# araju6/parameter-server-distributed

Measured on AMD Instinct MI355X. Metric: samples/sec (whole node) ResNet-50 async-SGD, higher is better.
Workload: dtype bf16

## Files before the change

### parameter_server_distributed_amd/csrc/bindings.cpp

```cpp
#include <torch/extension.h>

#include "async_hyper.h"
#include "async_ps.h"
#include "checkpoint.h"
#include "comm.h"
#include "kernels/launchers.h"
#include "kernels/launchers_gemm.h"
#include "ops.h"
#include "ps_core.h"
#include "registry.h"
#include "staleness.h"

namespace py = pybind11;
using namespace psd;

PYBIND11_MODULE(_C, m) {
  m.doc() = "MI355X-native parameter-server runtime: gfx950 HIP kernels, RCCL comm, PS/coordinator cores";

  m.def("fused_apply_", &fused_apply_, py::arg("master"), py::arg("grads"), py::arg("state1"), py::arg("state2"),
        py::arg("shadow"), py::arg("dyn"), py::arg("kind"), py::arg("momentum") = 0.0, py::arg("dampening") = 0.0,
        py::arg("nesterov") = false, py::arg("weight_decay") = 0.0, py::arg("beta1") = 0.9, py::arg("beta2") = 0.999,
        py::arg("eps") = 1e-8, py::arg("maximize") = false,
        py::arg("grid_cap") = 0, py::arg("scales") = ScaleList{}, py::arg("mx_scales") = MxScaleList{});
  m.def("fused_apply_lw_", &fused_apply_lw_, py::arg("master"), py::arg("grads"), py::arg("state1"),
        py::arg("state2"), py::arg("shadow"), py::arg("dyn"), py::arg("kind"), py::arg("momentum") = 0.0,
        py::arg("dampening") = 0.0, py::arg("nesterov") = false, py::arg("weight_decay") = 0.0, py::arg("beta1") = 0.9,
        py::arg("beta2") = 0.999, py::arg("eps") = 1e-8, py::arg("maximize") = false, py::arg("trust_coef") = 0.001,
        py::arg("layers") = std::vector<at::Tensor>{}, py::arg("grid_cap") = 0, py::arg("scales") = ScaleList{},
        py::arg("mx_scales") = MxScaleList{});
  m.def(
      "lw_table_build",
      [](const std::vector<int64_t>& offsets, const std::vector<int64_t>& numels, const std::vector<int64_t>& ndims,
         int64_t n, bool exclude_1d, int64_t align, const std::string& device) {
        return lw_table_build(offsets, numels, ndims, n, exclude_1d, align, at::Device(device));
      },
      py::arg("offsets"), py::arg("numels"), py::arg("ndims"), py::arg("n"), py::arg("exclude_1d"),
      py::arg("align") = 64, py::arg("device") = "cpu");
  m.def(
      "async_hyper",
      [](int kind, int workers, double momentum, double beta1, double beta2, double weight_decay) {
        const AsyncHyper h = async_hyper(kind, workers, momentum, beta1, beta2, weight_decay);
        py::dict d;
        d["lr_factor"] = h.lr_factor;
        d["grad_scale"] = h.grad_scale;
        d["momentum"] = h.momentum;
        d["beta1"] = h.beta1;
        d["beta2"] = h.beta2;
        d["weight_decay"] = h.weight_decay;
        return d;
      },
      py::arg("kind"), py::arg("workers"), py::arg("momentum"), py::arg("beta1"), py::arg("beta2"),
      py::arg("weight_decay"), "per-push optimizer hyperparameters of an apply-on-arrival PS (async_hyper.h)");
  m.def("optim_advance_", &optim_advance_, py::arg("dyn"), py::arg("beta1") = 0.9, py::arg("beta2") = 0.999);
  m.def("multi_reduce_", &multi_reduce_, py::arg("out"), py::arg("srcs"), py::arg("scale") = 1.0,
        py::arg("scales") = ScaleList{}, py::arg("mx_scales") = MxScaleList{});
  m.def("push_quant_mx_", &push_quant_mx_, py::arg("x"), py::arg("q"), py::arg("scales"),
        py::arg("blocks_per_seg") = 0, py::arg("residual") = py::none());
  m.def("grad_clip_coef_", &grad_clip_coef_, py::arg("flat"), py::arg("clip_norm"), py::arg("out"), py::arg("partials"),
        py::arg("grid_cap") = 0);
  m.def("pack_cast_", &pack_cast_, py::arg("srcs"), py::arg("dsts"));
  m.def("xfer_", &xfer_, py::arg("srcs"), py::arg("dsts"), py::arg("blocks_per_seg"), py::arg("nt_store") = false);
  m.def("amax_", &amax_);
  m.def("quant_fp8_", &quant_fp8_);
  m.def("dequant_fp8_", &dequant_fp8_);
  m.def("quant_mx_", &quant_mx_, py::arg("x"), py::arg("out"), py::arg("scales"));
  m.def("dequant_mx_", &dequant_mx_, py::arg("q"), py::arg("scales"), py::arg("out"));
  m.def("quant_mx_t_", &quant_mx_t_, py::arg("x"), py::arg("out"), py::arg("scales"));
  m.def("quant_mx_dual_", &quant_mx_dual_, py::arg("x"), py::arg("q_row"), py::arg("s_row"), py::arg("q_t"),
        py::arg("s_t"));
  m.def("quant_fp8_jit_", &quant_fp8_jit_, py::arg("x"), py::arg("out"), py::arg("scale_inv"));
  m.def("quant_fp8_delayed_", &quant_fp8_delayed_, py::arg("x"), py::arg("out"), py::arg("scale_inv"),
        py::arg("hist"), py::arg("margin") = 1.0);
  m.def("embed_bwd_", &embed_bwd_, py::arg("sorted"), py::arg("perm"), py::arg("dy"), py::arg("out"));
  m.def("xent_fwd", &xent_fwd, py::arg("x"), py::arg("labels"));
  m.def("xent_bwd", &xent_bwd, py::arg("x"), py::arg("labels"), py::arg("lse"), py::arg("scale"),
        py::arg("lse_lo") = py::none());
  m.def("bn_fwd", &bn_fwd, py::arg("x"), py::arg("gamma"), py::arg("beta"), py::arg("running_mean"),
        py::arg("running_var"), py::arg("residual"), py::arg("relu"), py::arg("training"), py::arg("momentum"),
        py::arg("eps"), py::arg("counter"), py::arg("ss_eval"), py::arg("mask_out") = false,
        py::arg("residual_ss") = py::none(), py::arg("stats_only") = false, py::arg("q8_out") = py::none(),
        py::arg("part_in") = py::none(), py::arg("part_rows") = 0, py::arg("q8_mx") = py::none());
  m.def("bn_reduce_", &bn_reduce_, py::arg("x"), py::arg("shift"));
  m.def("bn_bwd_reduce_", &bn_bwd_reduce_, py::arg("dy"), py::arg("x"), py::arg("save_mean"),
        py::arg("ss") = py::none(), py::arg("dy2") = py::none(), py::arg("mbits") = py::none());
  m.def("bn_bwd_dual", &bn_bwd_dual, py::arg("dy"), py::arg("x"), py::arg("gamma"), py::arg("save_mean"),
        py::arg("save_invstd"), py::arg("mbits"), py::arg("dy2"), py::arg("xd"), py::arg("gamma_d"), py::arg("mean_d"),
        py::arg("invstd_d"), py::arg("dgamma_out") = py::none(), py::arg("dbeta_out") = py::none(),
        py::arg("dgamma_d_out") = py::none(), py::arg("dbeta_d_out") = py::none(), py::arg("fold") = false);
  m.def("bn_bwd_coef", &bn_bwd_coef, py::arg("dy"), py::arg("x"), py::arg("gamma"), py::arg("save_mean"),
        py::arg("save_invstd"), py::arg("mbits") = py::none(), py::arg("dy2") = py::none(), py::arg("part") = py::none(),
        py::arg("rows") = 0, py::arg("dgamma_out") = py::none(), py::arg("dbeta_out") = py::none());
  m.def("bn_bwd", &bn_bwd, py::arg("dy"), py::arg("x"), py::arg("y"), py::arg("gamma"), py::arg("save_mean"),
        py::arg("save_invstd"), py::arg("relu"), py::arg("need_dr"), py::arg("dgamma_out"), py::arg("dbeta_out"),
        py::arg("dy2") = py::none(), py::arg("ss") = py::none(), py::arg("mbits") = py::none(),
        py::arg("dq") = py::none(), py::arg("dqmx") = py::none());
  m.def("gemm_", &gemm_, py::arg("A"), py::arg("B"), py::arg("a_kmajor"), py::arg("b_kmajor"), py::arg("out"),
        py::arg("bias") = py::none(), py::arg("act") = 0, py::arg("aux") = py::none(), py::arg("part") = py::none(),
        py::arg("shift") = py::none());
  m.def("gemm_stats_rows", &gemm_stats_rows_, py::arg("M"));
  m.def("gemm_set_bcontig", &gemm_set_bcontig, py::arg("on"));
  m.def("gemm_ct_", &gemm_ct_, py::arg("A"), py::arg("B"), py::arg("out"), py::arg("bias") = py::none(),
        py::arg("act") = 0, py::arg("aux") = py::none());
  m.def("gemm_gelu_bwd_", &gemm_gelu_bwd_, py::arg("A"), py::arg("B"), py::arg("a_kmajor"), py::arg("b_kmajor"),
        py::arg("pre"), py::arg("out"), py::arg("db"), py::arg("accumulate") = false);
  m.def("gemm_splitk_", &gemm_splitk_, py::arg("A"), py::arg("B"), py::arg("a_kmajor"), py::arg("b_kmajor"),
        py::arg("out"), py::arg("accumulate") = false, py::arg("scale") = 1.0, py::arg("splits") = 0);
  m.def("gemm_fp8_", &gemm_fp8_, py::arg("A"), py::arg("B"), py::arg("a_scale"), py::arg("b_scale"), py::arg("out"),
        py::arg("bias") = py::none(), py::arg("act") = 0, py::arg("aux") = py::none(), py::arg("part") = py::none(),
        py::arg("shift") = py::none());
  m.def("gemm_fp8_splitk_", &gemm_fp8_splitk_, py::arg("A"), py::arg("B"), py::arg("a_scale"), py::arg("b_scale"),
        py::arg("out"), py::arg("accumulate") = false, py::arg("scale") = 1.0, py::arg("splits") = 0);
  m.def("gemm_fp8_splits", &gemm_fp8_splits, py::arg("M"), py::arg("N"), py::arg("K"));
  m.def("convn_", &convn_, py::arg("x"), py::arg("w2"), py::arg("out"), py::arg("R"), py::arg("S"), py::arg("stride"),
        py::arg("pad"), py::arg("part") = py::none(), py::arg("shift") = py::none(), py::arg("variant") = -1,
        py::arg("x2") = py::none(), py::arg("bias") = py::none(), py::arg("no_store") = false,
        py::arg("apply_ss") = py::none(), py::arg("apply_res") = py::none(), py::arg("apply_mask") = py::none());
  m.def("convn_stats_rows", &convn_stats_rows_, py::arg("M"));
  m.def("convn_part_rows", &convn_part_rows_, py::arg("M"), py::arg("N"), py::arg("variant"), py::arg("Ho"),
        py::arg("Wo"), py::arg("R"));
  m.def("convn_variant_ok", &convn_variant_ok_, py::arg("N"), py::arg("variant"), py::arg("R"), py::arg("S"),
        py::arg("stride"), py::arg("pad"), py::arg("Wo"), py::arg("has_x2") = false);
  m.def("convn_dgrad_s2_", &convn_dgrad_s2_, py::arg("dy"), py::arg("wph"), py::arg("out"), py::arg("variant"),
        py::arg("part") = py::none(), py::arg("bx") = py::none(), py::arg("bmean") = py::none(),
        py::arg("bss") = py::none());
  m.def("convn_dgrad_s2_rows", &convn_dgrad_s2_rows, py::arg("Nb"), py::arg("Ho"), py::arg("Wo"), py::arg("Ci"),
        py::arg("variant"));
  m.def("convn_bwd_", &convn_bwd_, py::arg("dy"), py::arg("w2"), py::arg("out"), py::arg("R"), py::arg("S"),
        py::arg("stride"), py::arg("pad"), py::arg("part"), py::arg("variant"), py::arg("mode"), py::arg("bx"),
        py::arg("bmean"), py::arg("bss") = py::none(), py::arg("bdr") = py::none(), py::arg("bmbits") = py::none(),
        py::arg("x2") = py::none(), py::arg("bias") = py::none(), py::arg("bxd") = py::none(),
        py::arg("bmean_d") = py::none(), py::arg("part_d") = py::none());
  m.def("bn_bwd_pre", &bn_bwd_pre, py::arg("g"), py::arg("x"), py::arg("gamma"), py::arg("save_mean"),
        py::arg("save_invstd"), py::arg("part"), py::arg("rows"), py::arg("dgamma_out") = py::none(),
        py::arg("dbeta_out") = py::none(), py::arg("dq") = py::none(), py::arg("dqmx") = py::none());
  m.def("convn_variants", &convn_variants_, py::arg("N"));
  m.def("convn_variant_kind", &convn_variant_kind_, py::arg("N"), py::arg("variant"));
  m.def("conv_fwd_", &conv_fwd_, py::arg("x"), py::arg("w2"), py::arg("out"), py::arg("R"), py::arg("S"),
        py::arg("stride"), py::arg("pad"), py::arg("part") = py::none(), py::arg("shift") = py::none());
  m.def("conv_wgrad_", &conv_wgrad_, py::arg("dy"), py::arg("x"), py::arg("out"), py::arg("R"), py::arg("S"),
        py::arg("stride"), py::arg("pad"), py::arg("splits") = 0);
  m.def("convw_", &convw_, py::arg("dy"), py::arg("x"), py::arg("out"), py::arg("R"), py::arg("S"), py::arg("stride"),
        py::arg("pad"), py::arg("variant") = -1, py::arg("accumulate") = false, py::arg("fold") = false);
  m.def("bn_bwd_dual_pre", &bn_bwd_dual_pre, py::arg("g"), py::arg("x"), py::arg("gamma"), py::arg("save_mean"),
        py::arg("save_invstd"), py::arg("part"), py::arg("part_d"), py::arg("rows"), py::arg("xd"), py::arg("gamma_d"),
        py::arg("mean_d"), py::arg("invstd_d"), py::arg("dgamma_out") = py::none(), py::arg("dbeta_out") = py::none(),
        py::arg("dgamma_d_out") = py::none(), py::arg("dbeta_d_out") = py::none(), py::arg("fold") = false,
        py::arg("fold_d") = false, py::arg("derive_d") = false);
  m.def("bn_elemt_coef", &bn_elemt_coef, py::arg("g"), py::arg("x"), py::arg("coef"));
  m.def("convw_fold_rows", &convw_fold_rows, py::arg("Cout"), py::arg("Cin"));
  m.def("convw_gram_rows", &convw_gram_rows_, py::arg("C"));
  m.def("convw_gram_", &convw_gram_, py::arg("x"), py::arg("out"), py::arg("variant") = 0);
  m.def("bnfold_dgrad_weights", &bnfold_dgrad_weights, py::arg("w"), py::arg("coef"));
  m.def("bnfold_rowdot", &bnfold_rowdot, py::arg("P"), py::arg("w"), py::arg("row"));
  m.def("bnfold_gram_stats", &bnfold_gram_stats, py::arg("P"), py::arg("w"), py::arg("shift"), py::arg("M"),
        py::arg("row"));
  m.def("bnfold_dual_weights", &bnfold_dual_weights, py::arg("w3"), py::arg("wd"), py::arg("ss3"), py::arg("ssd"));
  m.def("bn_finalize", &bn_finalize, py::arg("part"), py::arg("rows"), py::arg("M"), py::arg("gamma"),
        py::arg("beta"), py::arg("running_mean"), py::arg("running_var"), py::arg("momentum"), py::arg("eps"),
        py::arg("counter") = py::none());
  m.def("bnfold_combine", &bnfold_combine, py::arg("P"), py::arg("w"), py::arg("coef"), py::arg("out"),
        py::arg("accumulate") = false);
  m.def("convw_variants", &convw_variants_, py::arg("Cout"), py::arg("KK"));
  m.def("conv_fwd_fp8_", &conv_fwd_fp8_, py::arg("x"), py::arg("w2"), py::arg("x_scale"), py::arg("w_scale"),
        py::arg("out"), py::arg("R"), py::arg("S"), py::arg("stride"), py::arg("pad"), py::arg("part") = py::none(),
        py::arg("shift") = py::none());
  m.def("gelu_bwd_colsum_", &gelu_bwd_colsum_, py::arg("dy"), py::arg("pre"), py::arg("dx"), py::arg("out"),
        py::arg("accumulate") = false);
  m.def("colsum_", &colsum_, py::arg("x"), py::arg("out"), py::arg("accumulate") = false);
  m.def("maxpool3s2_fwd", &maxpool3s2_fwd);
  m.def("maxpool3s2_bwd", &maxpool3s2_bwd, py::arg("dy"), py::arg("arg"), py::arg("H"), py::arg("W"),
        py::arg("dy2") = py::none());
  m.def("gap_fwd", &gap_fwd);
  m.def("bn_pool_fwd", &bn_pool_fwd, py::arg("x"), py::arg("gamma"), py::arg("beta"), py::arg("running_mean"),
        py::arg("running_var"), py::arg("momentum"), py::arg("eps"), py::arg("counter") = py::none());
  m.def("stem_fwd", &stem_fwd, py::arg("x"), py::arg("w"), py::arg("gamma"), py::arg("beta"), py::arg("running_mean"),
        py::arg("running_var"), py::arg("momentum"), py::arg("eps"), py::arg("counter") = py::none());
  m.def("stem_wgrad", &stem_wgrad);
  m.def("attn_fwd", &attn_fwd, py::arg("qkv"), py::arg("heads"), py::arg("p"), py::arg("seed"),
        py::arg("step") = py::none(), py::arg("lens") = py::none(), py::arg("grid_cap") = 0, py::arg("causal") = false,
        py::arg("doc_start") = py::none(), py::arg("window") = 0);
  m.def("attn_bwd", &attn_bwd, py::arg("dout"), py::arg("qkv"), py::arg("o"), py::arg("lse"), py::arg("heads"),
        py::arg("p"), py::arg("seed"), py::arg("step") = py::none(), py::arg("bias_out") = py::none(),
        py::arg("lens") = py::none(), py::arg("grid_cap") = 0, py::arg("causal") = false,
        py::arg("doc_start") = py::none(), py::arg("window") = 0);
  m.def("rope_", &rope_, py::arg("qkv"), py::arg("heads"), py::arg("cos"), py::arg("sin"), py::arg("lens") = py::none(),
        py::arg("doc_start") = py::none(), py::arg("inverse") = false, py::arg("blocks") = 0);
  m.def("rms_fwd", &rms_fwd, py::arg("r"), py::arg("h") = py::none(), py::arg("gamma"), py::arg("eps"), py::arg("p"),
        py::arg("seed"), py::arg("step") = py::none());
  m.def("rms_bwd", &rms_bwd, py::arg("dy"), py::arg("dr_new") = py::none(), py::arg("r_new"), py::arg("rstd"),
        py::arg("gamma"), py::arg("p"), py::arg("seed"), py::arg("step") = py::none(), py::arg("had_h"),
        py::arg("dgamma_out") = py::none());
  m.def("swiglu_fwd", &swiglu_fwd, py::arg("gu"), py::arg("blocks") = 0);
  m.def("swiglu_bwd", &swiglu_bwd, py::arg("da"), py::arg("gu"), py::arg("blocks") = 0);
  m.def("ln_fwd", &ln_fwd, py::arg("x"), py::arg("h"), py::arg("gamma"), py::arg("beta"), py::arg("eps"), py::arg("p"),
        py::arg("seed"), py::arg("step") = py::none(), py::arg("q8_out") = py::none(),
        py::arg("sc8_out") = py::none());
  m.def("ln_bwd", &ln_bwd, py::arg("dy"), py::arg("s"), py::arg("mean"), py::arg("rstd"), py::arg("gamma"), py::arg("p"),
        py::arg("seed"), py::arg("step") = py::none(), py::arg("dgamma_out") = py::none(),
        py::arg("dbeta_out") = py::none(), py::arg("dhsum_out") = py::none());
  m.def("emb_ln_fwd", &emb_ln_fwd, py::arg("ids"), py::arg("types"), py::arg("W"), py::arg("P"), py::arg("T"),
        py::arg("gamma"), py::arg("beta"), py::arg("S"), py::arg("eps"), py::arg("p"), py::arg("seed"),
        py::arg("step") = py::none(), py::arg("pos_ids") = py::none());
  m.def("emb_ln_bwd", &emb_ln_bwd, py::arg("dy"), py::arg("ids"), py::arg("types"), py::arg("W"), py::arg("P"),
        py::arg("T"), py::arg("gamma"), py::arg("mean"), py::arg("rstd"), py::arg("S"), py::arg("p"), py::arg("seed"),
        py::arg("step") = py::none(), py::arg("dgamma") = py::none(), py::arg("dbeta") = py::none(),
        py::arg("dT") = py::none(), py::arg("pos_ids") = py::none());
  m.def("bn_pool_bwd", &bn_pool_bwd, py::arg("gpool"), py::arg("gpool2"), py::arg("arg"), py::arg("x"), py::arg("gamma"),
        py::arg("save_mean"), py::arg("save_invstd"), py::arg("ss"), py::arg("dgamma_out") = py::none(),
        py::arg("dbeta_out") = py::none());
  m.def("gap_bwd", &gap_bwd);
  m.def("subsample2", &subsample2, py::arg("x"));
  m.def("wprep_table", &wprep_table, py::arg("srcs"), py::arg("dsts"), py::arg("geo"));
  m.def("wprep_run", &wprep_run, py::arg("table"), py::arg("tiles"));
  m.attr("OPT_SGD") = (int)OPT_SGD;
  m.attr("OPT_MOMENTUM") = (int)OPT_MOMENTUM;
  m.attr("OPT_ADAM") = (int)OPT_ADAM;
  m.attr("OPT_ADAMW") = (int)OPT_ADAMW;
  m.attr("OPT_LARS") = (int)OPT_LARS;
  m.attr("OPT_LAMB") = (int)OPT_LAMB;

  m.def("save_reference_ckpt", &save_reference_ckpt, py::call_guard<py::gil_scoped_release>());
  m.def("load_reference_ckpt", &load_reference_ckpt, py::call_guard<py::gil_scoped_release>());
  m.def("save_native_ckpt", &save_native_ckpt, py::call_guard<py::gil_scoped_release>());
  m.def("load_native_ckpt", &load_native_ckpt, py::call_guard<py::gil_scoped_release>());
  m.def("crc32", [](py::bytes b) {
    std::string s = b;
    return crc32(s.data(), s.size());
  });

  py::class_<WorkerEntry>(m, "WorkerEntry")
      .def_readonly("worker_id", &WorkerEntry::worker_id)
      .def_readonly("address", &WorkerEntry::address)
      .def_readonly("port", &WorkerEntry::port)
      .def_readonly("hostname", &WorkerEntry::hostname)
      .def_readonly("status", &WorkerEntry::status)
      .def_readonly("last_heartbeat", &WorkerEntry::last_heartbeat)
      .def_readonly("join_epoch", &WorkerEntry::join_epoch);
  py::class_<RegisterResult>(m, "RegisterResult")
      .def_readonly("success", &RegisterResult::success)
      .def_readonly("message", &RegisterResult::message)
      .def_readonly("ps_address", &RegisterResult::ps_address)
      .def_readonly("total_workers", &RegisterResult::total_workers)
      .def_readonly("membership_epoch", &RegisterResult::membership_epoch);
  py::class_<ShardInfo>(m, "ShardInfo")
      .def_readonly("shard_id", &ShardInfo::shard_id)
      .def_readonly("address", &ShardInfo::address)
      .def_readonly("rank", &ShardInfo::rank);
  py::class_<Registry>(m, "Registry")
      .def(py::init<std::string, int32_t>())
      .def("register_worker", &Registry::register_worker)
      .def("heartbeat", &Registry::heartbeat)
      .def("deregister", &Registry::deregister)
      .def("list_workers", &Registry::list_workers)
      .def("live_ids", &Registry::live_ids)
      .def("ps_address", &Registry::ps_address)
      .def("set_ps_address", &Registry::set_ps_address)
      .def("remove_stale", &Registry::remove_stale)
      .def("membership_epoch", &Registry::membership_epoch)
      .def("wait_epoch_change", &Registry::wait_epoch_change, py::call_guard<py::gil_scoped_release>())
      .def("set_shard", &Registry::set_shard)
      .def("shards", &Registry::shards)
      .def("kv_set", [](Registry& r, const std::string& k, py::bytes v) { r.kv_set(k, std::string(v)); })
      .def("kv_get",
           [](Registry& r, const std::string& k, double timeout) {
             std::tuple<bool, std::string> res;
             {
               py::gil_scoped_release nogil;
               res = r.kv_get(k, timeout);
             }
             return py::make_tuple(std::get<0>(res), py::bytes(std::get<1>(res)));
           })
      .def("use_manual_clock", &Registry::use_manual_clock)
      .def("advance_clock", &Registry::advance_clock)
      .def("now", &Registry::now);

  py::class_<PSConfig>(m, "PSConfig")
      .def(py::init<>())
      .def_readwrite("total_workers", &PSConfig::total_workers)
      .def_readwrite("async_mode", &PSConfig::async_mode)
      .def_readwrite("staleness_bound", &PSConfig::staleness_bound)
      .def_readwrite("window", &PSConfig::window)
      .def_readwrite("opt_kind", &PSConfig::opt_kind)
      .def_readwrite("lr", &PSConfig::lr)
      .def_readwrite("momentum", &PSConfig::momentum)
// ... 128 lines not shown
```

### parameter_server_distributed_amd/csrc/conv_ops.cpp

```cpp
#include <ATen/ATen.h>
#include <c10/core/DeviceGuard.h>

#include <algorithm>

#include "glue.h"
#include "kernels/launchers_convn.h"
#include "kernels/launchers_convw.h"
#include "kernels/launchers_gemm.h"
#include "ops.h"

namespace psd {

namespace {

struct ConvGeo {
  int64_t Nb, C, H, W, R, S, stride, pad, Ho, Wo, M, bytes;
  int logC;
  bool pow2_c() const { return (C & (C - 1)) == 0; }
};

ConvGeo conv_geo(const at::Tensor& x, int64_t R, int64_t S, int64_t stride, int64_t pad) {
  ConvGeo g{};
  g.Nb = x.size(0), g.C = x.size(1), g.H = x.size(2), g.W = x.size(3);
  g.R = R, g.S = S, g.stride = stride, g.pad = pad;
// ... 55 lines not shown
  a.Wo = (int)g.Wo;
  a.S = (int)g.S;
  a.stride = (int)g.stride;
  a.pad = (int)g.pad;
}

int64_t part_rows_bound(int64_t M, int64_t N, int64_t variant, int64_t Ho, int64_t Wo, int64_t R) {
  return std::max(convn_stats_rows((int)M), convn_part_rows_geo((int)M, (int)N, (int)std::max<int64_t>(variant, 0),
                                                                (int)Ho, (int)Wo, (int)R));
}

}

static int64_t conv_fwd_impl(const at::Tensor& x, const at::Tensor& w2, at::Tensor out, int64_t R, int64_t S,
                             int64_t stride, int64_t pad, const at::Tensor* xs, const at::Tensor* ws,
                             const c10::optional<at::Tensor>& part, const c10::optional<at::Tensor>& shift) {
  const bool f8 = xs != nullptr;
  const auto dt = f8 ? at::kFloat8_e4m3fn : at::kBFloat16;
  const bool x_e5 = f8 && x.scalar_type() == at::kFloat8_e5m2;
  const int esz = f8 ? 1 : 2;
  TORCH_CHECK(is_nhwc_dev(x, x_e5 ? at::kFloat8_e5m2 : dt), "psd conv_fwd: x must be a channels_last ",
              f8 ? "e4m3fn / e5m2" : "bf16", " device tensor");
  TORCH_CHECK(w2.is_cuda() && w2.dim() == 2 && w2.scalar_type() == dt && w2.stride(1) == 1 &&
                  (w2.stride(0) * esz) % 16 == 0 && aligned16(w2),
              "psd conv_fwd: w2 must be a 2-D device tensor like x, unit inner stride, 16-B aligned rows");
  TORCH_CHECK(out.dim() == 2 && out.stride(1) == 1 && out.scalar_type() == at::kBFloat16, "psd conv_fwd: out");
  const bool mx = f8 && xs->scalar_type() == at::kByte;
  if (mx) {
    TORCH_CHECK(ws->scalar_type() == at::kByte && xs->is_cuda() && ws->is_cuda() && xs->is_contiguous() &&
                    ws->is_contiguous() && xs->numel() == x.numel() / 32 && ws->numel() == w2.numel() / 32 &&
                    w2.stride(0) == w2.size(1),
                "psd conv_fwd_fp8: MX scales must be uint8 [pixels, C/32] / [Cout, K/32] (contiguous w2)");
  } else if (f8) {
    TORCH_CHECK(xs->scalar_type() == at::kFloat && ws->scalar_type() == at::kFloat && xs->is_cuda() && ws->is_cuda() &&
                    xs->numel() >= 1 && ws->numel() >= 1,
                "psd conv_fwd_fp8: scales must be fp32 device scalars (or MX uint8 block scales)");
  }
  const ConvGeo g = conv_geo(x, R, S, stride, pad);
  const int64_t M = g.M, Cout = w2.size(0), K = R * S * g.C;
  TORCH_CHECK(w2.size(1) == K, "psd conv_fwd: w2 must be [Cout, R*S*C]");
  TORCH_CHECK(out.size(0) == M && out.size(1) == Cout, "psd conv_fwd: out must be [Nb*Ho*Wo, Cout]");
  if (!g.pow2_c() || g.C < (f8 ? 128 : 64) || g.bytes >= ((int64_t)1 << 32) || M >= ((int64_t)1 << 31)) return 0;
  const c10::DeviceGuard dg(x.device());
  GemmArgs a{};
  a.A = x.data_ptr();
  a.B = w2.data_ptr();
  a.C = out.data_ptr();
  a.M = (int)M;
  a.N = (int)Cout;
  a.K = (int)K;
  a.lda = (int)K;
  a.ldb = (int)w2.stride(0);
  a.ldc = (int)out.stride(0);
  a.a_kmajor = a.b_kmajor = 1;
  set_geo(a, g);
  if (mx) {
    a.a_mx = xs->data_ptr<uint8_t>();
    a.b_mx = ws->data_ptr<uint8_t>();
  } else if (f8) {
    a.a_scale = xs->data_ptr<float>();
    a.b_scale = ws->data_ptr<float>();
  }
  a.f8a = x_e5 ? 1 : 0;
  int rows = 0;
  set_stats(a, part, shift, out, &rows);
  hipError_t e = f8 ? launch_conv_fwd_fp8(a, stream_of(x)) : launch_conv_fwd(a, stream_of(x));
  if (e == hipErrorNotSupported) return 0;
  check_hip(e, "psd conv_fwd");
  return a.part ? rows : 1;
}

int64_t conv_fwd_(const at::Tensor& x, const at::Tensor& w2, at::Tensor out, int64_t R, int64_t S, int64_t stride,
                  int64_t pad, c10::optional<at::Tensor> part, c10::optional<at::Tensor> shift) {
  return conv_fwd_impl(x, w2, out, R, S, stride, pad, nullptr, nullptr, part, shift);
}

int64_t conv_fwd_fp8_(const at::Tensor& x, const at::Tensor& w2, const at::Tensor& x_scale, const at::Tensor& w_scale,
                      at::Tensor out, int64_t R, int64_t S, int64_t stride, int64_t pad, c10::optional<at::Tensor> part,
                      c10::optional<at::Tensor> shift) {
  return conv_fwd_impl(x, w2, out, R, S, stride, pad, &x_scale, &w_scale, part, shift);
}

bool conv_wgrad_(const at::Tensor& dy, const at::Tensor& x, at::Tensor out, int64_t R, int64_t S, int64_t stride,
                 int64_t pad, int64_t splits) {
  TORCH_CHECK(is_nhwc_dev(dy, at::kBFloat16) && is_nhwc_dev(x, at::kBFloat16),
              "psd conv_wgrad: dy and x must be channels_last bf16 device tensors");
  const ConvGeo g = conv_geo(x, R, S, stride, pad);
  const int64_t Cout = dy.size(1);
  TORCH_CHECK(dy_matches(dy, g), "psd conv_wgrad: dy shape does not match the convolution");
  const int64_t N = R * S * g.C, K = g.M;
  TORCH_CHECK(out.dim() == 2 && out.size(0) == Cout && out.size(1) == N && out.is_contiguous() &&
                  out.scalar_type() == at::kBFloat16,
              "psd conv_wgrad: out must be a contiguous bf16 [Cout, R*S*C]");
  if (!g.pow2_c() || g.C < 8 || g.bytes >= ((int64_t)1 << 32) || K >= ((int64_t)1 << 31) || K < 128) return false;
  const c10::DeviceGuard dg(x.device());
  const int64_t tiles = ((Cout + 255) / 256) * ((N + 255) / 256);
  int64_t s = splits > 0 ? splits : std::max<int64_t>(1, 256 / tiles);
  s = std::min<int64_t>(s, std::max<int64_t>(1, K / 128));
  at::Tensor slab = at::empty({s * Cout * N}, x.options().dtype(at::kFloat));
  GemmArgs a{};
  a.A = dy.data_ptr();
  a.B = x.data_ptr();
  a.M = (int)Cout;
  a.N = (int)N;
  a.K = (int)K;
  a.lda = (int)Cout;
  a.ldb = (int)N;
  a.ldc = (int)N;
  a.a_kmajor = a.b_kmajor = 0;
  set_geo(a, g);
  hipError_t e = launch_conv_wgrad(a, slab.data_ptr<float>(), (int)s, out.data_ptr(), stream_of(x));
  if (e == hipErrorNotSupported) return false;
  check_hip(e, "psd conv_wgrad");
  return true;
}

int64_t convn_stats_rows_(int64_t M) { return convn_stats_rows((int)M); }
int64_t convn_part_rows_(int64_t M, int64_t N, int64_t v, int64_t Ho, int64_t Wo, int64_t R) {
  return convn_part_rows_geo((int)M, (int)N, (int)v, (int)Ho, (int)Wo, (int)R);
}
bool convn_variant_ok_(int64_t N, int64_t v, int64_t R, int64_t S, int64_t stride, int64_t pad, int64_t Wo,
                       bool has_x2) {
  return convn_variant_ok((int)N, (int)v, (int)R, (int)S, (int)stride, (int)pad, (int)Wo, has_x2);
}
int64_t convn_variants_(int64_t N) { return convn_variants((int)N); }
int64_t convn_variant_kind_(int64_t N, int64_t v) { return convn_variant_kind((int)N, (int)v); }

namespace {
int64_t convn_x2(ConvnArgs& a, const at::Tensor& x, c10::optional<at::Tensor> x2, c10::optional<at::Tensor> bias,
                 int64_t N) {
  if (given(bias)) {
    TORCH_CHECK(bias->scalar_type() == at::kFloat && bias->numel() == N && bias->is_contiguous() &&
                    bias->device() == x.device(),
                "psd convn: bias must be fp32 [N] on the input's device");
    a.bias = bias->data_ptr<float>();
  }
  if (!given(x2)) return 0;
  TORCH_CHECK(is_nhwc_dev(*x2, at::kBFloat16) && x2->device() == x.device() && x2->size(0) == x.size(0) &&
                  x2->size(2) == x.size(2) && x2->size(3) == x.size(3),
              "psd convn: x2 must be a channels_last bf16 tensor with the input's N, H, W");
  const int64_t C2 = x2->size(1), bytes = x2->numel() * 2;
  if (C2 < 64 || (C2 & (C2 - 1)) != 0 || bytes > 0xFFFFFF00ll) return -1;
  a.x2 = x2->data_ptr();
  a.x2bytes = (uint32_t)bytes;
  a.logC2 = log2_exact(C2);
  return C2;
}
}

int64_t convn_(const at::Tensor& x, const at::Tensor& w2, at::Tensor out, int64_t R, int64_t S, int64_t stride,
               int64_t pad, c10::optional<at::Tensor> part, c10::optional<at::Tensor> shift, int64_t variant,
               c10::optional<at::Tensor> x2, c10::optional<at::Tensor> bias, bool no_store,
               c10::optional<at::Tensor> apply_ss, c10::optional<at::Tensor> apply_res,
               c10::optional<at::Tensor> apply_mask) {
  TORCH_CHECK(is_nhwc_dev(x, at::kBFloat16), "psd convn: x must be a channels_last bf16 device tensor");
  TORCH_CHECK(w2.is_cuda() && w2.dim() == 2 && w2.scalar_type() == at::kBFloat16 && w2.is_contiguous(),
              "psd convn: w2 must be a contiguous bf16 [Cout, R*S*C] device tensor");
  TORCH_CHECK(no_store || (out.is_cuda() && out.dim() == 2 && out.stride(1) == 1 &&
                           out.scalar_type() == at::kBFloat16 && aligned16(out)),
              "psd convn: out must be a bf16 [M, Cout] device tensor, 16-B aligned");
  const bool apply = given(apply_ss);
  const ConvGeo g = conv_geo(x, R, S, stride, pad);
  const int64_t M = g.M, Cout = w2.size(0), Ho = g.Ho, Wo = g.Wo;
  ConvnArgs a{};
  const int64_t C2 = convn_x2(a, x, x2, bias, Cout);
  if (C2 < 0) return 0;
  const int64_t K = R * S * g.C + C2;
  TORCH_CHECK(w2.size(1) == K, "psd convn: w2 must be [Cout, R*S*C (+ C2)]");
  TORCH_CHECK(no_store || (out.size(0) == M && out.size(1) == Cout), "psd convn: out must be [Nb*Ho*Wo, Cout]");
  const bool stats = given(part);
  TORCH_CHECK(!no_store || (stats && !apply), "psd convn: no_store is a statistics-only pass");
  if (apply) {
    TORCH_CHECK(!stats && apply_ss->scalar_type() == at::kFloat && apply_ss->numel() == 2 * Cout &&
                    apply_ss->is_contiguous() && apply_ss->device() == x.device(),
                "psd convn: apply_ss must be fp32 [2 Cout] (no statistics in an apply pass)");
    TORCH_CHECK(!given(apply_res) ||
                    (apply_res->scalar_type() == at::kBFloat16 && apply_res->numel() == M * Cout &&
                     apply_res->device() == x.device() && nhwc_laid(*apply_res)),
                "psd convn: apply_res must be a bf16 [M, Cout] (or channels_last) residual, or None");
    TORCH_CHECK(given(apply_mask) && apply_mask->scalar_type() == at::kByte && apply_mask->numel() == M * Cout / 8 &&
                    apply_mask->is_contiguous(),
                "psd convn: apply_mask must be uint8 [M * Cout / 8]");
    TORCH_CHECK(out.stride(0) == Cout, "psd convn: the apply pass writes a dense [M, Cout] output");
  }
  if (stats) {
    TORCH_CHECK(given(shift) && shift->numel() == Cout && shift->scalar_type() == at::kFloat &&
                    shift->is_contiguous() && shift->device() == x.device(),
                "psd convn: statistics need an fp32 [Cout] shift on x's device");
    TORCH_CHECK(part->scalar_type() == at::kFloat && part->is_contiguous() && part->device() == x.device() &&
                    part->numel() >= part_rows_bound(M, Cout, variant, Ho, Wo, R) * 2 * Cout,
                "psd convn: part must be fp32 [convn_part_rows(...), 2, Cout]");
  }
  const int64_t wbytes = w2.numel() * 2;
  if (!g.pow2_c() || g.C < 64 || g.bytes > 0xFFFFFF00ll || wbytes >= ((int64_t)1 << 32) ||
      M >= ((int64_t)1 << 31) - 256 || convn_tile_n((int)Cout) == 0 || (!no_store && out.stride(0) % 8 != 0) ||
      Ho <= 0 || Wo <= 0 || variant >= convn_variants((int)Cout))
    return 0;
  const c10::DeviceGuard dg(x.device());
  a.x = x.data_ptr();
  a.w = w2.data_ptr();
  a.y = no_store ? nullptr : out.data_ptr();
  a.part = stats ? part->data_ptr<float>() : nullptr;
  a.shift = stats ? shift->data_ptr<float>() : nullptr;
  if (apply) {
    a.bwd = 8;
    a.bss = apply_ss->data_ptr<float>();
    a.ares = opt_ptr<const uint16_t>(apply_res);
    a.amask = apply_mask->data_ptr<uint8_t>();
  }
  set_geo(a, g, wbytes, Cout, K, no_store ? Cout : out.stride(0), variant);
  const hipError_t e = launch_convn(a, stream_of(x));
  if (e == hipErrorNotSupported) return 0;
  check_hip(e, "psd convn");
  return stats ? convn_part_rows_geo((int)M, (int)Cout, (int)std::max<int64_t>(variant, 0), (int)Ho, (int)Wo, (int)R)
               : 1;
}

int64_t convn_dgrad_s2_(const at::Tensor& dy, const std::vector<at::Tensor>& wph, at::Tensor out, int64_t variant,
                        c10::optional<at::Tensor> part, c10::optional<at::Tensor> bx, c10::optional<at::Tensor> bmean,
                        c10::optional<at::Tensor> bss) {
  TORCH_CHECK(is_nhwc_dev(dy, at::kBFloat16), "psd convn_dgrad_s2: dy must be a channels_last bf16 device tensor");
  TORCH_CHECK(wph.size() == 4, "psd convn_dgrad_s2: four phase weights");
  ConvGeo g = conv_geo(dy, 1, 1, 1, 0);
  const int64_t Co = g.C, Ho = g.Ho, Wo = g.Wo, M = g.M;
  const int64_t Ci = wph[0].size(0);
  for (int k = 0; k < 4; ++k) {
    const int64_t taps = (1 + (k >> 1)) * (1 + (k & 1));
    TORCH_CHECK(wph[k].is_cuda() && wph[k].dim() == 2 && wph[k].scalar_type() == at::kBFloat16 &&
                    wph[k].is_contiguous() && wph[k].size(0) == Ci && wph[k].size(1) == taps * Co &&
                    wph[k].device() == dy.device(),
                "psd convn_dgrad_s2: wph[k] must be a contiguous bf16 [Ci, taps * Co] tensor");
  }
  TORCH_CHECK(out.dim() == 2 && out.is_contiguous() && out.scalar_type() == at::kBFloat16 && out.size(0) == 4 * M &&
                  out.size(1) == Ci && out.device() == dy.device(),
              "psd convn_dgrad_s2: out must be a contiguous bf16 [Nb * 2Ho * 2Wo, Ci] tensor");
  const bool fused = given(part);
  if (fused) {
    TORCH_CHECK(given(bx) && bx->scalar_type() == at::kBFloat16 && bx->numel() == 4 * M * Ci &&
                    bx->device() == dy.device() && nhwc_laid(*bx),
                "psd convn_dgrad_s2: bx must be the BN input, bf16 like dX");
    TORCH_CHECK(given(bmean) && bmean->scalar_type() == at::kFloat && bmean->numel() == Ci && bmean->is_contiguous() &&
                    given(bss) && bss->scalar_type() == at::kFloat && bss->numel() == 2 * Ci && bss->is_contiguous(),
                "psd convn_dgrad_s2: mode 1 needs the BN's fp32 mean [Ci] and scale/shift [2 Ci]");
    TORCH_CHECK(part->scalar_type() == at::kFloat && part->is_contiguous() && part->device() == dy.device() &&
                    part->numel() >= 4 * part_rows_bound(M, Ci, variant, Ho, Wo, 2) * 2 * Ci,
                "psd convn_dgrad_s2: part must be fp32 [4 * convn_dgrad_s2_rows(...), 2, Ci]");
  }
  if (!g.pow2_c() || Co < 64 || g.bytes > 0xFFFFFF00ll || convn_tile_n((int)Ci) == 0 || Ci % 8 != 0 || variant < 0 ||
      variant >= convn_variants((int)Ci) || convn_variant_kind((int)Ci, (int)variant) != 0 || M >= (1 << 24))
    return 0;
  const c10::DeviceGuard dg(dy.device());
  const hipStream_t st = stream_of(dy);
  int64_t rows = 0;
  for (int k = 0; k < 4; ++k) {
    g.R = 1 + (k >> 1), g.S = 1 + (k & 1);
    ConvnArgs a{};
    a.x = dy.data_ptr();
    a.w = wph[k].data_ptr();
    a.y = out.data_ptr();
    set_geo(a, g, wph[k].numel() * 2, Ci, g.R * g.S * Co, Ci, variant);
    a.ophase = 1 + k;
    if (fused) {
      a.bwd = 1;
      a.part = part->data_ptr<float>() + rows * 2 * Ci;
      a.bx = reinterpret_cast<const uint16_t*>(bx->data_ptr());
      a.bmean = bmean->data_ptr<float>();
      a.bss = bss->data_ptr<float>();
    }
    const hipError_t e = launch_convn(a, st);
    if (e == hipErrorNotSupported) {
      TORCH_CHECK(k == 0, "psd convn_dgrad_s2: phase ", k, " declined after phase 0 ran");
      return 0;
    }
    check_hip(e, "psd convn_dgrad_s2");
    if (fused) rows += convn_part_rows_geo((int)M, (int)Ci, (int)variant, (int)Ho, (int)Wo, (int)g.R);
  }
  return fused ? rows : 1;
}

int64_t convn_dgrad_s2_rows(int64_t Nb, int64_t Ho, int64_t Wo, int64_t Ci, int64_t variant) {
  return 4 * part_rows_bound((int)(Nb * Ho * Wo), Ci, variant, Ho, Wo, 2);
}

int64_t convn_bwd_(const at::Tensor& dy, const at::Tensor& w2, at::Tensor out, int64_t R, int64_t S, int64_t stride,
                   int64_t pad, at::Tensor part, int64_t variant, int64_t mode, c10::optional<at::Tensor> bx,
                   const at::Tensor& bmean, c10::optional<at::Tensor> bss, c10::optional<at::Tensor> bdr,
                   c10::optional<at::Tensor> bmbits, c10::optional<at::Tensor> x2, c10::optional<at::Tensor> bias,
                   c10::optional<at::Tensor> bxd, c10::optional<at::Tensor> bmean_d, c10::optional<at::Tensor> part_d) {
  TORCH_CHECK(is_nhwc_dev(dy, at::kBFloat16), "psd convn_bwd: dy must be a channels_last bf16 device tensor");
  TORCH_CHECK(w2.is_cuda() && w2.dim() == 2 && w2.scalar_type() == at::kBFloat16 && w2.is_contiguous(),
              "psd convn_bwd: w2 must be a contiguous bf16 [N, R*S*C] tensor");
  TORCH_CHECK(out.dim() == 2 && out.is_contiguous() && out.scalar_type() == at::kBFloat16, "psd convn_bwd: out");
  TORCH_CHECK(mode == 1 || mode == 2 || mode == 3 || mode == 5,
              "psd convn_bwd: mode 1 (mask from x, ss), 2 (bit-mask + dr), 3 (2 + the dual tail's second BN) or 5 "
              "(2 with dr on the stride-2 quarter grid)");
  const ConvGeo g = conv_geo(dy, R, S, stride, pad);
  const int64_t Nb = g.Nb, Ho = g.Ho, Wo = g.Wo, M = g.M, N = w2.size(0);
  ConvnArgs a{};
  const int64_t C2 = convn_x2(a, dy, x2, bias, N);
  if (C2 < 0) return 0;
  const int64_t K = R * S * g.C + C2;
  TORCH_CHECK(w2.size(1) == K && out.size(0) == M && out.size(1) == N, "psd convn_bwd: shapes");
  auto like_out = [&](const at::Tensor& t, const char* what) {
    TORCH_CHECK(t.scalar_type() == at::kBFloat16 && t.numel() == M * N && t.device() == dy.device() && nhwc_laid(t),
                "psd convn_bwd: ", what, " must be a contiguous bf16 [M, N] (or channels_last) tensor");
  };
  const bool has_bx = given(bx);
  TORCH_CHECK(has_bx || mode == 2 || mode == 5, "psd convn_bwd: only modes 2 and 5 run without the BN input bx");
  if (has_bx) like_out(*bx, "bx");
  TORCH_CHECK(bmean.scalar_type() == at::kFloat && bmean.numel() == N && bmean.is_contiguous(), "psd convn_bwd: bmean");
  TORCH_CHECK(part.scalar_type() == at::kFloat && part.is_contiguous() &&
                  part.numel() >= part_rows_bound(M, N, variant, Ho, Wo, R) * 2 * N,
              "psd convn_bwd: part must be fp32 [convn_part_rows(...), 2, N]");
  if (mode == 1) {
    TORCH_CHECK(given(bss) && bss->numel() == 2 * N && bss->scalar_type() == at::kFloat && bss->is_contiguous(),
                "psd convn_bwd: mode 1 needs ss fp32 [2N]");
  } else {
    if (mode == 3) {
      TORCH_CHECK(given(bxd) && given(bmean_d) && given(part_d), "psd convn_bwd: mode 3 needs bxd, bmean_d and part_d");
      like_out(*bxd, "bxd");
      TORCH_CHECK(bmean_d->scalar_type() == at::kFloat && bmean_d->numel() == N && bmean_d->is_contiguous(),
                  "psd convn_bwd: bmean_d");
      TORCH_CHECK(part_d->scalar_type() == at::kFloat && part_d->is_contiguous() && part_d->numel() >= part.numel(),
                  "psd convn_bwd: part_d like part");
    }
    TORCH_CHECK(given(bdr), "psd convn_bwd: mode 2 needs dr");
    if (mode == 5) {
      TORCH_CHECK(bdr->scalar_type() == at::kBFloat16 && bdr->dim() == 4 && bdr->size(0) == Nb && bdr->size(1) == N &&
                      bdr->size(2) * 2 == Ho && bdr->size(3) * 2 == Wo &&
                      bdr->is_contiguous(at::MemoryFormat::ChannelsLast) && bdr->device() == dy.device(),
                  "psd convn_bwd: mode 5 dr must be channels_last bf16 [Nb, N, Ho/2, Wo/2]");
    } else {
      like_out(*bdr, "dr");
    }
    TORCH_CHECK(given(bmbits) && bmbits->scalar_type() == at::kByte && bmbits->numel() == M * N / 8 &&
                    bmbits->is_contiguous(),
                "psd convn_bwd: mode 2 needs the uint8 [M*N/8] bit-mask");
  }
  const int64_t wbytes = w2.numel() * 2;
  if (!g.pow2_c() || g.C < 64 || g.bytes > 0xFFFFFF00ll || wbytes >= ((int64_t)1 << 32) ||
      M >= ((int64_t)1 << 31) - 256 || convn_tile_n((int)N) == 0 || variant >= convn_variants((int)N) || N % 8 != 0)
    return 0;
  const c10::DeviceGuard dg(dy.device());
  a.x = dy.data_ptr();
  a.w = w2.data_ptr();
  a.y = out.data_ptr();
  a.part = part.data_ptr<float>();
  set_geo(a, g, wbytes, N, K, N, variant);
  a.bwd = (int)mode;
  a.bx = opt_ptr<const uint16_t>(bx);
  a.bmean = bmean.data_ptr<float>();
  a.bss = mode == 1 ? bss->data_ptr<float>() : nullptr;
  a.bdr = mode >= 2 ? reinterpret_cast<const uint16_t*>(bdr->data_ptr()) : nullptr;
  a.bmbits = mode >= 2 ? bmbits->data_ptr<uint8_t>() : nullptr;
  if (mode == 3) {
    a.bxd = reinterpret_cast<const uint16_t*>(bxd->data_ptr());
    a.bmean_d = bmean_d->data_ptr<float>();
    a.part_d = part_d->data_ptr<float>();
  }
  const hipError_t e = launch_convn(a, stream_of(dy));
  if (e == hipErrorNotSupported) return 0;
  check_hip(e, "psd convn_bwd");
  return convn_part_rows_geo((int)M, (int)N, (int)std::max<int64_t>(variant, 0), (int)Ho, (int)Wo, (int)R);
}

int64_t convw_variants_(int64_t Cout, int64_t KK) { return convw_variants((int)Cout, (int)KK); }

int64_t convw_fold_rows(int64_t Cout, int64_t Cin) {
  const int64_t rows = (Cout + Cin + 16 + 127) / 128 * 128;
  return convw_fold_ok((int)Cout, (int)Cin, (int)rows) ? rows : 0;
}

namespace {
bool run_convw(ConvwArgs& a, const at::Tensor& x, const char* op) {
  const ConvwPlan p = convw_plan(a);
  if (p.splits <= 0) return false;
  at::Tensor slab = at::empty({p.slab_floats}, x.options().dtype(at::kFloat));
  a.slab = slab.data_ptr<float>();
  const hipError_t e = launch_convw(a, stream_of(x));
  if (e == hipErrorNotSupported) return false;
  check_hip(e, op);
  return true;
}
}

bool convw_(const at::Tensor& dy, const at::Tensor& x, at::Tensor out, int64_t R, int64_t S, int64_t stride,
            int64_t pad, int64_t variant, bool accumulate, bool fold) {
  TORCH_CHECK(is_nhwc_dev(dy, at::kBFloat16) && is_nhwc_dev(x, at::kBFloat16) && dy.device() == x.device(),
              "psd convw: dy and x must be channels_last bf16 tensors on one device");
  const ConvGeo g = conv_geo(x, R, S, stride, pad);
  const int64_t Cout = dy.size(1);
  TORCH_CHECK(dy_matches(dy, g), "psd convw: dy shape does not match the convolution");
  const int64_t KK = R * S * g.C, M = g.M;
  const int64_t rows = fold ? convw_fold_rows(Cout, KK) : Cout;
  TORCH_CHECK(out.is_cuda() && out.device() == x.device() && out.dim() == 2 && out.size(0) == rows &&
                  out.size(1) == KK && out.is_contiguous() &&
                  out.scalar_type() == (fold ? at::kFloat : at::kBFloat16) && aligned16(out),
              "psd convw: out must be a contiguous [Cout, R*S*C] bf16 tensor (fold: fp32 [convw_fold_rows, C]) "
              "on x's device");
  if (fold && (R != 1 || S != 1 || stride != 1 || pad != 0 || accumulate)) return false;
  const int64_t dybytes = dy.numel() * 2;
  if (!g.pow2_c() || g.C < 64 || g.bytes > 0xFFFFFF00ll || dybytes > 0xFFFFFF00ll || M >= ((int64_t)1 << 31) ||
      (!fold && variant >= convw_variants((int)Cout, (int)KK)) || g.H >= 32768 || g.W >= 32768)
    return false;
  const c10::DeviceGuard dg(x.device());
  ConvwArgs a{};
  a.dy = dy.data_ptr();
  a.x = x.data_ptr();
  a.out = out.data_ptr();
  a.dybytes = (uint32_t)dybytes;
  set_geo(a, g);
  a.Cout = (int)Cout;
  a.KK = (int)KK;
  a.variant = (int)variant;
  a.accumulate = accumulate ? 1 : 0;
  a.fold = fold ? 1 : 0;
  a.Arows = (int)rows;
  return run_convw(a, x, "psd convw");
}

int64_t convw_gram_rows_(int64_t C) { return convw_gram_rows((int)C); }

bool convw_gram_(const at::Tensor& x, at::Tensor out, int64_t variant) {
  TORCH_CHECK(is_nhwc_dev(x, at::kBFloat16), "psd convw_gram: x must be a channels_last bf16 tensor");
  const ConvGeo g = conv_geo(x, 1, 1, 1, 0);
  const int64_t C = g.C, M = g.M;
  const int64_t rows = convw_gram_rows((int)C);
  TORCH_CHECK(out.is_cuda() && out.device() == x.device() && out.dim() == 2 && out.size(0) == rows &&
                  out.size(1) == C && out.is_contiguous() && out.scalar_type() == at::kFloat && aligned16(out),
              "psd convw_gram: out must be a contiguous fp32 [convw_gram_rows(C), C] tensor on x's device");
  if (rows == 0 || g.bytes > 0xFFFFFF00ll || M >= ((int64_t)1 << 31) || M == 0) return false;
  const c10::DeviceGuard dg(x.device());
  ConvwArgs a{};
  a.dy = x.data_ptr();
  a.x = x.data_ptr();
  a.out = out.data_ptr();
  a.dybytes = (uint32_t)g.bytes;
  set_geo(a, g);
  a.Cout = 0;
  a.KK = (int)C;
  a.fold = 2;
  a.variant = (int)variant;
  a.Arows = (int)rows;
  return run_convw(a, x, "psd convw_gram");
}

}
```

### parameter_server_distributed_amd/csrc/kernels/convn.hip

```cpp
#include "mfma_common.h"
#include "cu_count.h"
#include "launchers_convn.h"

namespace psd {

namespace {

constexpr int kBM = 128;
constexpr int kBK = 64;

__device__ __forceinline__ bf16x8 frag(const uint8_t* lds, int rb, int ks, int lane) {
  const int row = rb * 16 + (lane & 15);
  return __builtin_bit_cast(bf16x8, *reinterpret_cast<const u32x4*>(lds + kmaj_off(row, ks * 4 + (lane >> 4))));
}

template <int DPSK, int A>
__device__ __forceinline__ void wait_ahead(int ahead) {
  if constexpr (A <= 0) {
    wait_vm<0>();
  } else {
    if (ahead >= A) wait_vm<A * DPSK>();
    else wait_ahead<DPSK, A - 1>(ahead);
  }
}

template <int N>
__device__ __forceinline__ float ror_row(float x) {
  return __builtin_bit_cast(float, __builtin_amdgcn_mov_dpp(__builtin_bit_cast(int, x), 0x120 + N, 0xF, 0xF, true));
}

__device__ __forceinline__ int fdiv(int x, int d, float inv) {
  int q = (int)((float)x * inv);
  const int r = x - q * d;
  q += (r >= d ? 1 : 0) - (r < 0 ? 1 : 0);
  return q;
}

template <int BM, int BN, int WNT, int NSLOT>
struct Geo {
  static constexpr int WM = BM / 64;
  static constexpr int NWC = BN / WNT;
  static constexpr int NW = WM * NWC;
  static constexpr int NT = 64 * NW;
  static constexpr int JN = WNT / 16;
  static constexpr int APW = (BM / 8) / NW;
  static constexpr int BPW = (BN / 8) / NW;
  static constexpr int DPS = APW + BPW;
  static constexpr int AB = BM * 128;
  static constexpr int SLOT = AB + BN * 128;
  static constexpr int STG = 2048;
  static_assert((BM / 8) % NW == 0 && (BN / 8) % NW == 0 && APW >= 1 && BPW >= 1, "DMA pieces per wave");
  static_assert(DPS * (NSLOT - 2) < 64, "vmcnt is 6 bits");
  static_assert(WNT == 32 || WNT == 64, "wave tile width");
};


}

template <int JN>
struct EpiSums {
  float s1[JN], s2[JN];
  float ga[8], gb[8], gd[8];
  __device__ __forceinline__ void zero() {
#pragma unroll
    for (int j = 0; j < JN; ++j) s1[j] = s2[j] = 0.f;
#pragma unroll
    for (int e = 0; e < 8; ++e) ga[e] = gb[e] = gd[e] = 0.f;
  }
};

template <int WNT, bool STATS, int BWD>
__device__ __forceinline__ void convn_flush(const ConvnArgs& a, EpiSums<WNT / 16>& es, int64_t prow, int wc, int lane,
                                            int n0) {
  constexpr int JN = WNT / 16;
  const int cl = lane & 15;
  if constexpr (STATS) {
#pragma unroll
    for (int j = 0; j < JN; ++j) {
      float s1 = es.s1[j], s2 = es.s2[j];
      s1 += xor16(s1, lane);
      s2 += xor16(s2, lane);
      s1 += xor32(s1, lane);
      s2 += xor32(s2, lane);
      if (lane < 16) {
        float* pr = a.part + prow * 2 * a.N;
        const int col = n0 + wc * WNT + j * 16 + cl;
        pr[col] = s1;
        pr[a.N + col] = s2;
      }
    }
  }
  if constexpr (BWD >= 1 && BWD <= 5) {
    constexpr int CPR = WNT * 2 / 16;
    const int my_col = n0 + wc * WNT + (lane % CPR) * 8;
#pragma unroll
    for (int e = 0; e < 8; ++e) {
      if constexpr (CPR == 4) {
        es.ga[e] += ror_row<4>(es.ga[e]);
        es.gb[e] += ror_row<4>(es.gb[e]);
      }
      es.ga[e] += ror_row<8>(es.ga[e]);
      es.gb[e] += ror_row<8>(es.gb[e]);
      es.ga[e] += xor16(es.ga[e], lane);
      es.gb[e] += xor16(es.gb[e], lane);
      es.ga[e] += xor32(es.ga[e], lane);
      es.gb[e] += xor32(es.gb[e], lane);
      if constexpr (BWD == 3) {
        if constexpr (CPR == 4) es.gd[e] += ror_row<4>(es.gd[e]);
        es.gd[e] += ror_row<8>(es.gd[e]);
        es.gd[e] += xor16(es.gd[e], lane);
        es.gd[e] += xor32(es.gd[e], lane);
      }
    }
    if (lane < CPR) {
      float* pr = a.part + prow * 2 * a.N;
      store8_f32(pr + my_col, es.ga);
      store8_f32(pr + a.N + my_col, es.gb);
      if constexpr (BWD == 3) {
        float* pd = a.part_d + prow * 2 * a.N;
        store8_f32(pd + my_col, es.ga);
        store8_f32(pd + a.N + my_col, es.gd);
      }
    }
  }
}

template <int WNT>
struct EpiOps {
  static constexpr int CPR = WNT * 2 / 16;
  static constexpr int PASSES = 16 * CPR / 64;
  int mm[4][PASSES];
  u32x4 exr[4][PASSES], rv4[4][PASSES], dv4[4][PASSES];
  uint32_t bt[4][PASSES];
};

template <int WNT, int BWD, typename Pix>
__device__ __forceinline__ void epi_load(const ConvnArgs& a, int wr, int wc, int lane, Pix pix, int n0, EpiOps<WNT>& o) {
  constexpr bool BRED = BWD >= 1 && BWD <= 5;
  constexpr bool APPLY = BWD == 8;
  constexpr int CPR = EpiOps<WNT>::CPR, PASSES = EpiOps<WNT>::PASSES;
  const int my_col = n0 + wc * WNT + (lane % CPR) * 8;
  const bool has_bx = !BRED || a.bx != nullptr;
  const bool fast_div = a.M < (1 << 24);
  float inv_hw = 0.f, inv_wo = 0.f;
  if constexpr (BWD == 5) {
    inv_hw = 1.f / (float)(a.Ho * a.Wo);
    inv_wo = 1.f / (float)a.Wo;
  }
#pragma unroll
  for (int i = 0; i < 4; ++i)
#pragma unroll
    for (int ps = 0; ps < PASSES; ++ps) {
      const int c = ps * 64 + lane;
      const int rr = c / CPR;
      const int m = pix(wr * 64 + i * 16 + rr);
      o.mm[i][ps] = m;
      if constexpr (APPLY) {
        o.rv4[i][ps] = u32x4{0u, 0u, 0u, 0u};
        if (m >= 0 && a.ares) o.rv4[i][ps] = *reinterpret_cast<const u32x4*>(a.ares + (int64_t)m * a.N + my_col);
      }
      if constexpr (BRED) {
        o.exr[i][ps] = o.rv4[i][ps] = o.dv4[i][ps] = u32x4{0u, 0u, 0u, 0u};
        o.bt[i][ps] = 0u;
        if (m >= 0) {
          if (has_bx) o.exr[i][ps] = *reinterpret_cast<const u32x4*>(a.bx + (int64_t)m * a.N + my_col);
          if constexpr (BWD >= 2) {
            if constexpr (BWD == 5) {
              const int hw = a.Ho * a.Wo;
              const int n = fast_div ? fdiv(m, hw, inv_hw) : m / hw, rem = m - n * hw;
              const int h = fast_div ? fdiv(rem, a.Wo, inv_wo) : rem / a.Wo, w = rem - h * a.Wo;
              if (((h | w) & 1) == 0) {
                const int64_t q = ((int64_t)n * (a.Ho >> 1) + (h >> 1)) * (a.Wo >> 1) + (w >> 1);
                o.rv4[i][ps] = *reinterpret_cast<const u32x4*>(a.bdr + q * a.N + my_col);
              }
            } else {
              o.rv4[i][ps] = *reinterpret_cast<const u32x4*>(a.bdr + (int64_t)m * a.N + my_col);
            }
            o.bt[i][ps] = a.bmbits[((int64_t)m * a.N + my_col) >> 3];
          }
          if constexpr (BWD == 3) o.dv4[i][ps] = *reinterpret_cast<const u32x4*>(a.bxd + (int64_t)m * a.N + my_col);
        }
      }
    }
}

template <int BM, int BN, int WNT, bool STATS, int BWD, bool DEFER = false, bool PRE = false, typename Pix>
__device__ __forceinline__ void convn_epilogue(const ConvnArgs& a, f32x4 (&acc)[4][WNT / 16],
                                               const float (&kshift)[WNT / 16], int tm, int wr, int wc, int lane,
                                               uint8_t* stg, Pix pix, int n0, EpiSums<WNT / 16>& es,
                                               const EpiOps<WNT>* pre = nullptr) {
  constexpr int JN = WNT / 16;
  constexpr int WM = BM / 64;
  const int cl = lane & 15, rq = (lane >> 4) * 4;
  if (a.bias) {
#pragma unroll
    for (int j = 0; j < JN; ++j) {
      const float bv = a.bias[n0 + wc * WNT + j * 16 + cl];
#pragma unroll
      for (int i = 0; i < 4; ++i) acc[i][j] += f32x4{bv, bv, bv, bv};
    }
  }
  if constexpr (STATS) {
    typedef float f32x2 __attribute__((ext_vector_type(2)));
    const bool rnd = a.y != nullptr;
#pragma unroll
    for (int i = 0; i < 4; ++i) {
      const bool full = pix(wr * 64 + i * 16 + 15) >= 0;
#pragma unroll
      for (int j = 0; j < JN; ++j) {
        const f32x2 k2 = {kshift[j], kshift[j]};
        f32x2 s1 = {0.f, 0.f}, s2 = {0.f, 0.f};
#pragma unroll
        for (int r = 0; r < 4; r += 2) {
          f32x2 d;
          if (rnd) {
            const uint32_t pk = pack_bf16x2_rne(acc[i][j][r], acc[i][j][r + 1]);
            d = f32x2{__uint_as_float(pk << 16), __uint_as_float(pk & 0xFFFF0000u)} - k2;
          } else {
            d = f32x2{acc[i][j][r], acc[i][j][r + 1]} - k2;
          }
          if (!full) {
            d[0] = pix(wr * 64 + i * 16 + rq + r) >= 0 ? d[0] : 0.f;
            d[1] = pix(wr * 64 + i * 16 + rq + r + 1) >= 0 ? d[1] : 0.f;
          }
          s1 += d;
          s2 = __builtin_elementwise_fma(d, d, s2);
        }
        es.s1[j] += s1[0] + s1[1];
        es.s2[j] += s2[0] + s2[1];
      }
    }
  }
  constexpr bool BRED = BWD >= 1 && BWD <= 5;
  constexpr bool APPLY = BWD == 8;
  if constexpr (STATS && !BRED && !APPLY) {
    if (a.y == nullptr) {
      if constexpr (!DEFER) convn_flush<WNT, STATS, BWD>(a, es, (int64_t)tm * WM + wr, wc, lane, n0);
      return;
    }
  }
  if constexpr (APPLY) {
#pragma unroll
    for (int j = 0; j < JN; ++j) {
      const int col = n0 + wc * WNT + j * 16 + cl;
      const float sc = a.bss[col], sh = a.bss[a.N + col];
#pragma unroll
      for (int i = 0; i < 4; ++i)
#pragma unroll
        for (int r = 0; r < 4; ++r) acc[i][j][r] = fmaf(acc[i][j][r], sc, sh);
    }
  }
  const int L = cl & 3;
  constexpr int RB = WNT * 2;
  constexpr int CPR = RB / 16;
  constexpr int PASSES = 16 * CPR / 64;
  uint16_t* y = reinterpret_cast<uint16_t*>(a.y);
  const int my_c16 = lane % CPR;
  const int my_col = n0 + wc * WNT + my_c16 * 8;
  float bmu[8], bsc[8], bsh[8], bmd[8];
  if constexpr (BWD == 3) load8_f32(a.bmean_d + my_col, bmd);
  if constexpr (BRED) load8_f32(a.bmean + my_col, bmu);
  if constexpr (BWD == 1) {
    load8_f32(a.bss + my_col, bsc);
    load8_f32(a.bss + a.N + my_col, bsh);
  }
  EpiOps<WNT> own;
  if constexpr (!PRE) epi_load<WNT, BWD>(a, wr, wc, lane, pix, n0, own);
  const EpiOps<WNT>& ops = PRE ? *pre : own;
  const auto& mm = ops.mm;
  const auto& exr = ops.exr;
  const auto& rv4 = ops.rv4;
  const auto& dv4 = ops.dv4;
  const auto& bt = ops.bt;
#pragma unroll
  for (int i = 0; i < 4; ++i) {
    const int r = rq + L;
#pragma unroll
    for (int j = 0; j < JN; ++j) {
      float w[4];
      quad_t4(acc[i][j], L, w);
      const int c8 = (j * 16 + (cl & ~3)) >> 2;
      const int off = r * RB + ((c8 ^ ((r & 7) << 1)) & (RB / 8 - 1)) * 8;
      const uint32_t lo = pack_bf16x2_rne(w[0], w[1]), hi = pack_bf16x2_rne(w[2], w[3]);
      *reinterpret_cast<uint64_t*>(stg + off) = (uint64_t)lo | ((uint64_t)hi << 32);
    }
#pragma unroll
    for (int ps = 0; ps < PASSES; ++ps) {
      const int c = ps * 64 + lane;
      const int rr = c / CPR, c16 = c % CPR;
      const int off = rr * RB + (((2 * c16) ^ ((rr & 7) << 1)) & (RB / 8 - 1)) * 8;
      u32x4 v = *reinterpret_cast<const u32x4*>(stg + off);
      const int m = mm[i][ps];
      if (m >= 0) {
        const int64_t go = (int64_t)m * a.ldc + n0 + wc * WNT + c16 * 8;
        if constexpr (APPLY) {
          float d[8], rv[8];
          load8_bf16(reinterpret_cast<const uint16_t*>(&v), d);
          load8_bf16(reinterpret_cast<const uint16_t*>(&rv4[i][ps]), rv);
          uint32_t bits = 0;
#pragma unroll
          for (int e = 0; e < 8; ++e) {
            const float o = relu_nan(d[e] + rv[e]);
            d[e] = o;
            bits |= (o > 0.f ? 1u : 0u) << e;
          }
          uint32_t pk[4];
#pragma unroll
          for (int e = 0; e < 4; ++e) pk[e] = pack_bf16x2_rne(d[2 * e], d[2 * e + 1]);
          v = u32x4{pk[0], pk[1], pk[2], pk[3]};
          a.amask[((int64_t)m * a.N + my_col) >> 3] = (uint8_t)bits;
        }
        if constexpr (BRED) {
          float d[8], xv[8];
          load8_bf16(reinterpret_cast<const uint16_t*>(&v), d);
          load8_bf16(reinterpret_cast<const uint16_t*>(&exr[i][ps]), xv);
          if constexpr (BWD >= 2) {
            float rv[8];
            load8_bf16(reinterpret_cast<const uint16_t*>(&rv4[i][ps]), rv);
            const uint32_t bits = bt[i][ps];
#pragma unroll
            for (int e = 0; e < 8; ++e) d[e] = ((bits >> e) & 1u) ? d[e] + rv[e] : 0.f;
          } else {
#pragma unroll
            for (int e = 0; e < 8; ++e) d[e] = fmaf(xv[e], bsc[e], bsh[e]) > 0.f ? d[e] : 0.f;
          }
          uint32_t pk[4];
#pragma unroll
          for (int e = 0; e < 4; ++e) pk[e] = pack_bf16x2_rne(d[2 * e], d[2 * e + 1]);
          v = u32x4{pk[0], pk[1], pk[2], pk[3]};
          float gq[8];
          load8_bf16(reinterpret_cast<const uint16_t*>(&v), gq);
#pragma unroll
          for (int e = 0; e < 8; ++e) {
            es.ga[e] += gq[e];
            es.gb[e] = fmaf(gq[e], xv[e] - bmu[e], es.gb[e]);
          }
          if constexpr (BWD == 3) {
            float dv[8];
            load8_bf16(reinterpret_cast<const uint16_t*>(&dv4[i][ps]), dv);
#pragma unroll
            for (int e = 0; e < 8; ++e) es.gd[e] = fmaf(gq[e], dv[e] - bmd[e], es.gd[e]);
          }
        }
        *reinterpret_cast<u32x4*>(y + go) = v;
      }
    }
  }
  if constexpr (!DEFER) convn_flush<WNT, STATS, BWD>(a, es, (int64_t)tm * WM + wr, wc, lane, n0);
}

template <int BM, int BN, int WNT, int NSLOT, bool STATS, int BWD = 0>
__global__ __launch_bounds__(512) void convn_kernel(ConvnArgs a) {
  using G = Geo<BM, BN, WNT, NSLOT>;
  extern __shared__ __attribute__((aligned(16))) uint8_t smem[];
  const int tiles_m = gridDim.x;
  const int tm = xcd_remap(blockIdx.x, tiles_m);
  const int m0 = tm * BM, n0 = blockIdx.y * BN;
  constexpr int SLOTB = G::SLOT;
  const int oph = (a.ophase - 1) >> 1, opw = (a.ophase - 1) & 1;
  const float inv_ohw = 1.f / (float)(a.Ho * a.Wo), inv_owo = 1.f / (float)a.Wo;
  auto pix = [&](int p) -> int {
    const int m = m0 + p;
    if (m >= a.M) return -1;
    if (a.ophase == 0) return m;
    const int hw = a.Ho * a.Wo;
    const int n = fdiv(m, hw, inv_ohw), rem = m - n * hw;
    const int i = fdiv(rem, a.Wo, inv_owo), j = rem - i * a.Wo;
    return ((n * 2 * a.Ho + 2 * i + oph) * 2 * a.Wo) + 2 * j + opw;
  };
  const int lane = threadIdx.x & 63;
  const int wid = __builtin_amdgcn_readfirstlane(threadIdx.x >> 6);
  const int wr = wid / G::NWC, wc = wid % G::NWC;
  const int cl = lane & 15, rq = (lane >> 4) * 4;

  float kshift[G::JN];
#pragma unroll
  for (int j = 0; j < G::JN; ++j) kshift[j] = 0.f;
  if constexpr (STATS) {
#pragma unroll
    for (int j = 0; j < G::JN; ++j) kshift[j] = a.shift[n0 + wc * WNT + j * 16 + cl];
  }

  int p0[G::APW], hw[G::APW];
  {
    const int howo = a.Ho * a.Wo;
#pragma unroll
    for (int i = 0; i < G::APW; ++i) {
      const int row = (i * G::NW + wid) * 8 + (lane >> 3);
      const int m = m0 + row;
      const int n = m / howo, rem = m - n * howo;
      const int ho = rem / a.Wo, wo = rem - ho * a.Wo;
      const int h0 = ho * a.stride - a.pad, w0 = wo * a.stride - a.pad;
      p0[i] = (n * a.H + h0) * a.W + w0;
      hw[i] = m < a.M ? (int)(((uint32_t)h0 << 16) | ((uint32_t)w0 & 0xffffu)) : (int)0x80000000u;
    }
  }
  const rsrc_t xr = make_rsrc(a.x, a.xbytes);
  const rsrc_t x2r = make_rsrc(a.x2 ? a.x2 : a.x, a.x2 ? a.x2bytes : 0u);
  const rsrc_t wrs = make_rsrc(a.w, a.wbytes);
  const int cmask = (1 << a.logC) - 1;
  const int nslot = a.nslot;

  auto stage = [&](int t) {
    uint8_t* slot = smem + (t % nslot) * SLOTB;
    const int k0 = t * kBK;
    if (k0 >= a.K1) {
      const int c0 = k0 - a.K1;
#pragma unroll
      for (int i = 0; i < G::APW; ++i) {
        const int piece = i * G::NW + wid;
        const int row = piece * 8 + (lane >> 3);
        const int kc = (lane & 7) ^ ((row >> 1) & 7);
        const bool ok = hw[i] != (int)0x80000000u;
        const uint32_t off = ok ? ((((uint32_t)p0[i]) << a.logC2) + (uint32_t)(c0 + kc * 8)) * 2u : kOOB;
        __builtin_amdgcn_raw_ptr_buffer_load_lds(x2r, (__attribute__((address_space(3))) void*)(slot + piece * 1024),
                                                 16, off, 0, 0, 0);
      }
    } else {
    const int rs = k0 >> a.logC, ci0 = k0 & cmask;
    const int r = rs / a.S, s = rs - r * a.S;
#pragma unroll
    for (int i = 0; i < G::APW; ++i) {
      const int piece = i * G::NW + wid;
      const int row = piece * 8 + (lane >> 3);
      const int kc = (lane & 7) ^ ((row >> 1) & 7);
      const int hh = (hw[i] >> 16) + r, ww = ((int)((uint32_t)hw[i] << 16) >> 16) + s;
      const bool ok = (unsigned)hh < (unsigned)a.H && (unsigned)ww < (unsigned)a.W;
      const uint32_t off = ok ? ((((uint32_t)(p0[i] + r * a.W + s)) << a.logC) + (uint32_t)(ci0 + kc * 8)) * 2u : kOOB;
      __builtin_amdgcn_raw_ptr_buffer_load_lds(xr, (__attribute__((address_space(3))) void*)(slot + piece * 1024), 16,
                                               off, 0, 0, 0);
    }
    }
#pragma unroll
    for (int i = 0; i < G::BPW; ++i) {
      const int piece = i * G::NW + wid;
      const int row = piece * 8 + (lane >> 3);
      const int kc = (lane & 7) ^ ((row >> 1) & 7);
      const uint32_t off = ((uint32_t)(n0 + row) * (uint32_t)a.K + (uint32_t)(k0 + kc * 8)) * 2u;
      __builtin_amdgcn_raw_ptr_buffer_load_lds(wrs,
                                               (__attribute__((address_space(3))) void*)(slot + (SLOTB - BN * 128) +
                                                                                        piece * 1024),
                                               16, off, 0, 0, 0);
    }
  };

  f32x4 acc[4][G::JN];
#pragma unroll
  for (int i = 0; i < 4; ++i)
#pragma unroll
    for (int j = 0; j < G::JN; ++j) acc[i][j] = f32x4{0.f, 0.f, 0.f, 0.f};

  const int nt = a.K / kBK;
  const int D = nslot - 1 > 0 ? nslot - 1 : 1;
  for (int p = 0; p < D && p < nt; ++p) stage(p);
  constexpr int DPSK = G::DPS;
  for (int t = 0; t < nt; ++t) {
    wait_ahead<DPSK, NSLOT - 2>(min(nt - 1 - t, D - 1));
    __builtin_amdgcn_s_barrier();
    __builtin_amdgcn_sched_barrier(0);
    if (t + D < nt) stage(t + D);
    const uint8_t* As = smem + (t % nslot) * SLOTB;
    const uint8_t* Bs = As + (SLOTB - BN * 128);
    bf16x8 af[2][4], bf[2][G::JN];
#pragma unroll
    for (int ks = 0; ks < 2; ++ks) {
#pragma unroll
      for (int j = 0; j < G::JN; ++j) bf[ks][j] = frag(Bs, wc * G::JN + j, ks, lane);
#pragma unroll
      for (int i = 0; i < 4; ++i) af[ks][i] = frag(As, wr * 4 + i, ks, lane);
    }
#pragma unroll
    for (int ks = 0; ks < 2; ++ks)
#pragma unroll
      for (int i = 0; i < 4; ++i)
#pragma unroll
        for (int j = 0; j < G::JN; ++j)
          acc[i][j] = __builtin_amdgcn_mfma_f32_16x16x32_bf16(af[ks][i], bf[ks][j], acc[i][j], 0, 0, 0);
    __builtin_amdgcn_sched_barrier(0);
  }

  EpiSums<G::JN> es;
  es.zero();
  convn_epilogue<BM, BN, WNT, STATS, BWD>(a, acc, kshift, tm, wr, wc, lane,
                                          smem + a.nslot * SLOTB + wid * G::STG, pix,
                                          n0, es);
}


template <int BN, int WNT, int NSLOT, bool STATS, int BWD>
__global__ __launch_bounds__(512) void convp_kernel(ConvnArgs a, int tiles_m) {
  constexpr int BM = 128;
  using G = Geo<BM, BN, WNT, NSLOT>;
  constexpr int SLOTB = G::SLOT;
  extern __shared__ __attribute__((aligned(16))) uint8_t smem[];
  const int n0 = blockIdx.y * BN;
  const int gx = gridDim.x;
  const int bq = xcd_remap(blockIdx.x, gx);
  const int t_begin = (int)(((int64_t)bq * tiles_m) / gx);
  const int t_end = (int)(((int64_t)(bq + 1) * tiles_m) / gx);
  const int lane = threadIdx.x & 63;
  const int wid = __builtin_amdgcn_readfirstlane(threadIdx.x >> 6);
  const int wr = wid / G::NWC, wc = wid % G::NWC;
  const int cl = lane & 15;
  float kshift[G::JN];
#pragma unroll
  for (int j = 0; j < G::JN; ++j) kshift[j] = 0.f;
  if constexpr (STATS) {
#pragma unroll
    for (int j = 0; j < G::JN; ++j) kshift[j] = a.shift[n0 + wc * WNT + j * 16 + cl];
  }
  const rsrc_t xr = make_rsrc(a.x, a.xbytes);
  const rsrc_t x2r = make_rsrc(a.x2 ? a.x2 : a.x, a.x2 ? a.x2bytes : 0u);
  const rsrc_t wrs = make_rsrc(a.w, a.wbytes);
  const int nslot = a.nslot;
  const int nt = a.K / kBK;
  const int total = (t_end - t_begin) * nt;
  auto stage = [&](int T) {
    uint8_t* slot = smem + (T % nslot) * SLOTB;
    const int tile = t_begin + T / nt;
    const int k0 = (T % nt) * kBK;
    const int m0 = tile * BM;
    const bool second = k0 >= a.K1;
    const int c0 = second ? k0 - a.K1 : k0;
    const int lc = second ? a.logC2 : a.logC;
#pragma unroll
    for (int i = 0; i < G::APW; ++i) {
      const int piece = i * G::NW + wid;
      const int row = piece * 8 + (lane >> 3);
      const int kc = (lane & 7) ^ ((row >> 1) & 7);
      const int m = m0 + row;
      const uint32_t off = m < a.M ? ((((uint32_t)m) << lc) + (uint32_t)(c0 + kc * 8)) * 2u : kOOB;
      __builtin_amdgcn_raw_ptr_buffer_load_lds(second ? x2r : xr,
                                               (__attribute__((address_space(3))) void*)(slot + piece * 1024), 16, off,
                                               0, 0, 0);
    }
#pragma unroll
    for (int i = 0; i < G::BPW; ++i) {
      const int piece = i * G::NW + wid;
      const int row = piece * 8 + (lane >> 3);
      const int kc = (lane & 7) ^ ((row >> 1) & 7);
      const uint32_t off = ((uint32_t)(n0 + row) * (uint32_t)a.K + (uint32_t)(k0 + kc * 8)) * 2u;
      __builtin_amdgcn_raw_ptr_buffer_load_lds(
          wrs, (__attribute__((address_space(3))) void*)(slot + (SLOTB - BN * 128) + piece * 1024), 16, off, 0, 0, 0);
    }
  };
  f32x4 acc[4][G::JN];
#pragma unroll
  for (int i = 0; i < 4; ++i)
#pragma unroll
    for (int j = 0; j < G::JN; ++j) acc[i][j] = f32x4{0.f, 0.f, 0.f, 0.f};
  EpiSums<G::JN> es;
  es.zero();
  uint8_t* stg = smem + nslot * SLOTB + wid * G::STG;
  const int D = nslot - 1;
  for (int p = 0; p < D && p < total; ++p) stage(p);
  for (int T = 0; T < total; ++T) {
    wait_ahead<G::DPS, NSLOT - 2>(min(total - 1 - T, D - 1));
    __builtin_amdgcn_s_barrier();
    __builtin_amdgcn_sched_barrier(0);
    if (T + D < total) stage(T + D);
    const uint8_t* As = smem + (T % nslot) * SLOTB;
    const uint8_t* Bs = As + (SLOTB - BN * 128);
    bf16x8 af[2][4], bf[2][G::JN];
#pragma unroll
    for (int ks = 0; ks < 2; ++ks) {
#pragma unroll
      for (int j = 0; j < G::JN; ++j) bf[ks][j] = frag(Bs, wc * G::JN + j, ks, lane);
#pragma unroll
      for (int i = 0; i < 4; ++i) af[ks][i] = frag(As, wr * 4 + i, ks, lane);
    }
#pragma unroll
    for (int ks = 0; ks < 2; ++ks)
#pragma unroll
      for (int i = 0; i < 4; ++i)
#pragma unroll
        for (int j = 0; j < G::JN; ++j)
          acc[i][j] = __builtin_amdgcn_mfma_f32_16x16x32_bf16(af[ks][i], bf[ks][j], acc[i][j], 0, 0, 0);
    __builtin_amdgcn_sched_barrier(0);
    if (T % nt == nt - 1) {
      const int tile = t_begin + T / nt;
      const int m0 = tile * BM;
      auto pix = [&](int p) -> int { return m0 + p < a.M ? m0 + p : -1; };
      convn_epilogue<BM, BN, WNT, STATS, BWD, true>(a, acc, kshift, tile, wr, wc, lane, stg, pix, n0, es);
#pragma unroll
      for (int i = 0; i < 4; ++i)
#pragma unroll
        for (int j = 0; j < G::JN; ++j) acc[i][j] = f32x4{0.f, 0.f, 0.f, 0.f};
    }
  }
  convn_flush<WNT, STATS, BWD>(a, es, (int64_t)blockIdx.x * G::WM + wr, wc, lane, n0);
}

constexpr int kPrMaxSlots = 6;
template <int BN, int WNT, bool STATS, int BWD>
__global__ __launch_bounds__(512) void convpr_kernel(ConvnArgs a, int tiles_m) {
  constexpr int BM = 128;
  using G = Geo<BM, BN, WNT, 3>;
  constexpr int AB = BM * 128;
  extern __shared__ __attribute__((aligned(16))) uint8_t smem[];
  const int n0 = blockIdx.y * BN;
  const int gx = gridDim.x;
  const int bq = xcd_remap(blockIdx.x, gx);
  const int t_begin = (int)(((int64_t)bq * tiles_m) / gx);
  const int t_end = (int)(((int64_t)(bq + 1) * tiles_m) / gx);
  const int lane = threadIdx.x & 63;
  const int wid = __builtin_amdgcn_readfirstlane(threadIdx.x >> 6);
  const int wr = wid / G::NWC, wc = wid % G::NWC;
  const int cl = lane & 15;
  float kshift[G::JN];
#pragma unroll
  for (int j = 0; j < G::JN; ++j) kshift[j] = 0.f;
  if constexpr (STATS) {
#pragma unroll
    for (int j = 0; j < G::JN; ++j) kshift[j] = a.shift[n0 + wc * WNT + j * 16 + cl];
  }
  const rsrc_t xr = make_rsrc(a.x, a.xbytes);
  const rsrc_t x2r = make_rsrc(a.x2 ? a.x2 : a.x, a.x2 ? a.x2bytes : 0u);
  const rsrc_t wrs = make_rsrc(a.w, a.wbytes);
  const int nslot = a.nslot;
  const int nt = a.K / kBK;
  uint8_t* bres = smem;
  uint8_t* ring = smem + nt * BN * 128;
  uint8_t* stg = ring + nslot * AB + wid * G::STG;
  for (int pc = wid; pc < nt * (BN / 8); pc += G::NW) {
    const int kt = pc / (BN / 8), rp = pc - kt * (BN / 8);
    const int row = rp * 8 + (lane >> 3);
    const int kc = (lane & 7) ^ ((row >> 1) & 7);
    const uint32_t off = ((uint32_t)(n0 + row) * (uint32_t)a.K + (uint32_t)(kt * kBK + kc * 8)) * 2u;
    __builtin_amdgcn_raw_ptr_buffer_load_lds(wrs, (__attribute__((address_space(3))) void*)(bres + pc * 1024), 16, off, 0,
                                             0, 0);
  }
  wait_vm<0>();
  const int total = (t_end - t_begin) * nt;
  auto stage = [&](int T) {
    uint8_t* slot = ring + (T % nslot) * AB;
    const int tile = t_begin + T / nt;
    const int k0 = (T % nt) * kBK;
    const int m0 = tile * BM;
    const bool second = k0 >= a.K1;
    const int c0 = second ? k0 - a.K1 : k0;
    const int lc = second ? a.logC2 : a.logC;
#pragma unroll
    for (int i = 0; i < G::APW; ++i) {
      const int piece = i * G::NW + wid;
      const int row = piece * 8 + (lane >> 3);
      const int kc = (lane & 7) ^ ((row >> 1) & 7);
      const int m = m0 + row;
      const uint32_t off = m < a.M ? ((((uint32_t)m) << lc) + (uint32_t)(c0 + kc * 8)) * 2u : kOOB;
      __builtin_amdgcn_raw_ptr_buffer_load_lds(second ? x2r : xr,
                                               (__attribute__((address_space(3))) void*)(slot + piece * 1024), 16, off,
                                               0, 0, 0);
    }
  };
  f32x4 acc[4][G::JN];
#pragma unroll
  for (int i = 0; i < 4; ++i)
#pragma unroll
    for (int j = 0; j < G::JN; ++j) acc[i][j] = f32x4{0.f, 0.f, 0.f, 0.f};
  EpiSums<G::JN> es;
  es.zero();
  const int D = nslot - 1;
  for (int p = 0; p < D && p < total; ++p) stage(p);
  for (int T = 0; T < total; ++T) {
    wait_ahead<G::APW, kPrMaxSlots - 2>(min(total - 1 - T, D - 1));
    __builtin_amdgcn_s_barrier();
    __builtin_amdgcn_sched_barrier(0);
    if (T + D < total) stage(T + D);
    const uint8_t* As = ring + (T % nslot) * AB;
    const uint8_t* Bs = bres + (T % nt) * BN * 128;
    bf16x8 af[2][4], bf[2][G::JN];
#pragma unroll
    for (int ks = 0; ks < 2; ++ks) {
#pragma unroll
      for (int j = 0; j < G::JN; ++j) bf[ks][j] = frag(Bs, wc * G::JN + j, ks, lane);
#pragma unroll
      for (int i = 0; i < 4; ++i) af[ks][i] = frag(As, wr * 4 + i, ks, lane);
    }
#pragma unroll
    for (int ks = 0; ks < 2; ++ks)
#pragma unroll
      for (int i = 0; i < 4; ++i)
#pragma unroll
        for (int j = 0; j < G::JN; ++j)
          acc[i][j] = __builtin_amdgcn_mfma_f32_16x16x32_bf16(af[ks][i], bf[ks][j], acc[i][j], 0, 0, 0);
    __builtin_amdgcn_sched_barrier(0);
    if (T % nt == nt - 1) {
      const int tile = t_begin + T / nt;
      const int m0 = tile * BM;
      auto pix = [&](int p) -> int { return m0 + p < a.M ? m0 + p : -1; };
      convn_epilogue<BM, BN, WNT, STATS, BWD, true>(a, acc, kshift, tile, wr, wc, lane, stg, pix, n0, es);
#pragma unroll
      for (int i = 0; i < 4; ++i)
#pragma unroll
        for (int j = 0; j < G::JN; ++j) acc[i][j] = f32x4{0.f, 0.f, 0.f, 0.f};
    }
  }
  convn_flush<WNT, STATS, BWD>(a, es, (int64_t)blockIdx.x * G::WM + wr, wc, lane, n0);
}

__device__ __forceinline__ int hx_swz(int row) { return ((row >> 1) & 3) << 1; }
__device__ __forceinline__ int hx_off(int row, int kc) { return row * 128 + ((kc ^ hx_swz(row)) << 4); }

constexpr int kHxWin = 4 * 64 * 128;
constexpr int kHxW = 9 * 64 * 128;
constexpr int kHxLds = kHxW + 2 * kHxWin + 4 * 2048 + 512;

template <bool STATS, int BWD>
__global__ __launch_bounds__(256) void convh_kernel(ConvnArgs a, int ntiles) {
  extern __shared__ __attribute__((aligned(16))) uint8_t smem[];
  uint8_t* wlds = smem;
  auto winb = [&](int b) { return smem + kHxW + b * kHxWin; };
  const int lane = threadIdx.x & 63;
  const int wid = __builtin_amdgcn_readfirstlane(threadIdx.x >> 6);
  const int wr = wid >> 1, wc = wid & 1;
  const int cl = lane & 15;
  const int tpi = (a.Ho + 1) >> 1;
  const int t_begin = (int)(((int64_t)blockIdx.x * ntiles) / gridDim.x);
  const int t_end = (int)(((int64_t)(blockIdx.x + 1) * ntiles) / gridDim.x);
  if (t_begin >= t_end) return;
  float kshift[2] = {0.f, 0.f};
  if constexpr (STATS) {
#pragma unroll
    for (int j = 0; j < 2; ++j) kshift[j] = a.shift[wc * 32 + j * 16 + cl];
  }
  const rsrc_t xr = make_rsrc(a.x, a.xbytes);
  const rsrc_t wrs = make_rsrc(a.w, a.wbytes);
  for (int pc = wid; pc < 72; pc += 4) {
    const int t = pc >> 3, row = (pc & 7) * 8 + (lane >> 3);
    const int kc = (lane & 7) ^ hx_swz(row);
    const uint32_t off = ((uint32_t)row * (uint32_t)a.K + (uint32_t)(t * 64 + kc * 8)) * 2u;
    __builtin_amdgcn_raw_ptr_buffer_load_lds(wrs, (__attribute__((address_space(3))) void*)(wlds + pc * 1024), 16, off,
                                             0, 0, 0);
  }
  auto stage = [&](int tile, int b) {
    const int n = tile / tpi, ho0 = (tile - n * tpi) * 2;
#pragma unroll
    for (int i = 0; i < 8; ++i) {
      const int pc = i * 4 + wid;
      const int row = pc * 8 + (lane >> 3);
      const int jj = row >> 6, ws = row & 63;
      const int hi = ho0 - 1 + jj, wi = ws - 1;
      const int kc = (lane & 7) ^ hx_swz(row);
      const bool ok = (unsigned)hi < (unsigned)a.H && (unsigned)wi < (unsigned)a.W;
      const uint32_t off = ok ? ((((uint32_t)((n * a.H + hi) * a.W + wi)) << 6) + (uint32_t)(kc * 8)) * 2u : kOOB;
      __builtin_amdgcn_raw_ptr_buffer_load_lds(xr, (__attribute__((address_space(3))) void*)(winb(b) + pc * 1024), 16,
                                               off, 0, 0, 0);
    }
  };
  stage(t_begin, 0);
  wait_vm<0>();
  __syncthreads();
  uint8_t* stg = smem + kHxW + 2 * kHxWin + wid * 2048;
  EpiSums<2> es;
  es.zero();
  auto pix_of = [&](int tl) {
    const int n = tl / tpi, ho0 = (tl - n * tpi) * 2;
    return [=](int p) -> int {
      const int j = p >> 6, wo = p & 63;
      return ((wo < a.Wo) & (ho0 + j < a.Ho)) ? (n * a.Ho + ho0 + j) * a.Wo + wo : -1;
    };
  };
  for (int tile = t_begin, it = 0; tile < t_end; ++tile, ++it) {
    const int b = it & 1;
    if (tile + 1 < t_end) stage(tile + 1, b ^ 1);
    const uint8_t* win = winb(b);
    f32x4 acc[4][2];
#pragma unroll
    for (int i = 0; i < 4; ++i)
#pragma unroll
      for (int j = 0; j < 2; ++j) acc[i][j] = f32x4{0.f, 0.f, 0.f, 0.f};
    auto load_tap = [&](int tap, bf16x8 (&af)[2][4], bf16x8 (&bf)[2][2]) {
      const int tr = tap / 3, ts = tap - tr * 3;
      const uint8_t* Bs = wlds + tap * 8192;
#pragma unroll
      for (int ks = 0; ks < 2; ++ks) {
#pragma unroll
        for (int j = 0; j < 2; ++j)
          bf[ks][j] = __builtin_bit_cast(
              bf16x8, *reinterpret_cast<const u32x4*>(Bs + hx_off((wc * 2 + j) * 16 + (lane & 15), ks * 4 + (lane >> 4))));
#pragma unroll
        for (int i = 0; i < 4; ++i) {
          const int row = (wr + tr) * 64 + i * 16 + (lane & 15) + ts;
          af[ks][i] = __builtin_bit_cast(bf16x8, *reinterpret_cast<const u32x4*>(win + hx_off(row, ks * 4 + (lane >> 4))));
        }
      }
    };
    bf16x8 fa[2][2][4], fb[2][2][2];
    load_tap(0, fa[0], fb[0]);
#pragma unroll
    for (int tap = 0; tap < 9; ++tap) {
      const int cb = tap & 1;
      if (tap + 1 < 9) load_tap(tap + 1, fa[cb ^ 1], fb[cb ^ 1]);
      __builtin_amdgcn_sched_barrier(0);
#pragma unroll
      for (int ks = 0; ks < 2; ++ks)
#pragma unroll
        for (int i = 0; i < 4; ++i)
#pragma unroll
          for (int j = 0; j < 2; ++j)
            acc[i][j] = __builtin_amdgcn_mfma_f32_16x16x32_bf16(fa[cb][ks][i], fb[cb][ks][j], acc[i][j], 0, 0, 0);
      __builtin_amdgcn_sched_barrier(0);
    }
    wait_vm<0>();
    convn_epilogue<128, 64, 32, STATS, BWD, true>(a, acc, kshift, tile, wr, wc, lane, stg, pix_of(tile), 0, es);
    __syncthreads();
  }
  convn_flush<32, STATS, BWD>(a, es, (int64_t)blockIdx.x * 2 + wr, wc, lane, 0);
}

static bool convh_ok(const ConvnArgs& a) {
  return a.N == 64 && a.logC == 6 && a.R == 3 && a.S == 3 && a.stride == 1 && a.pad == 1 && a.H == a.Ho &&
         a.W == a.Wo && a.Wo + 2 <= 64 && !a.x2 && a.K == 576 && a.ldc == 64;
}

static int convh_grid(int ntiles) { return ntiles < cu_count() ? ntiles : cu_count(); }

template <bool STATS, int BWD>
static hipError_t convh_launch_t(const ConvnArgs& a, hipStream_t st) {
  static bool attr = false;
  if (!attr) {
    const hipError_t e =
        hipFuncSetAttribute((const void*)convh_kernel<STATS, BWD>, hipFuncAttributeMaxDynamicSharedMemorySize, kHxLds);
    if (e != hipSuccess) return e;
    attr = true;
  }
  const int ntiles = (a.M / (a.Ho * a.Wo)) * ((a.Ho + 1) / 2);
  hipLaunchKernelGGL((convh_kernel<STATS, BWD>), dim3(convh_grid(ntiles)), dim3(256), kHxLds, st, a, ntiles);
  return hipGetLastError();
}

static hipError_t convh_launch(const ConvnArgs& a, hipStream_t st) {
  if (a.bwd == 1) return convh_launch_t<false, 1>(a, st);
  if (a.bwd == 2) return convh_launch_t<false, 2>(a, st);
  if (a.bwd == 3) return convh_launch_t<false, 3>(a, st);
  if (a.bwd == 5) return convh_launch_t<false, 5>(a, st);
  return a.part ? convh_launch_t<true, 0>(a, st) : convh_launch_t<false, 0>(a, st);
}

template <int BN>
struct P1Cfg;
template <>
struct P1Cfg<256> {
  static constexpr int WNT = 64;
};
template <>
struct P1Cfg<128> {
  static constexpr int WNT = 32;
};
template <>
struct P1Cfg<64> {
  static constexpr int WNT = 32;
};
constexpr int kP1Slots = 3;
template <int BN>
constexpr int p1_lds() {
  using G = Geo<128, BN, P1Cfg<BN>::WNT, kP1Slots>;
  return kP1Slots * G::SLOT + G::NW * G::STG;
}

static int convp_grid_x(int tiles_m, int tiles_n) {
  int g = cu_count() / (tiles_n > 0 ? tiles_n : 1);
  if (g < 1) g = 1;
  return g < tiles_m ? g : tiles_m;
}

template <int BN, bool STATS, int BWD>
static hipError_t convp_launch_t(const ConvnArgs& a0, hipStream_t st, int grid_mul = 1) {
  constexpr int WNT = P1Cfg<BN>::WNT;
  using G = Geo<128, BN, WNT, kP1Slots>;
  constexpr int LDS = p1_lds<BN>();
  static_assert(LDS <= 160 * 1024, "LDS");
  static bool attr = false;
  if (!attr) {
    const hipError_t e = hipFuncSetAttribute((const void*)convp_kernel<BN, WNT, kP1Slots, STATS, BWD>,
                                             hipFuncAttributeMaxDynamicSharedMemorySize, LDS);
    if (e != hipSuccess) return e;
    attr = true;
  }
  ConvnArgs a = a0;
  a.nslot = kP1Slots;
  const int tiles_m = (a.M + 127) / 128, tiles_n = a.N / BN;
  int gx = convp_grid_x(tiles_m, tiles_n) * grid_mul;
  if (gx > tiles_m) gx = tiles_m;
  hipLaunchKernelGGL((convp_kernel<BN, WNT, kP1Slots, STATS, BWD>), dim3(gx, tiles_n), dim3(G::NT), LDS, st, a,
                     tiles_m);
  return hipGetLastError();
}

template <int BN>
static int pr_slots(int K) {
  using G = Geo<128, BN, P1Cfg<BN>::WNT, 3>;
  const int fixed = (K / kBK) * BN * 128 + G::NW * G::STG;
  int ns = (160 * 1024 - fixed) / (128 * 128);
  if (ns > kPrMaxSlots) ns = kPrMaxSlots;
  return ns >= 3 ? ns : 0;
}

template <int BN, bool STATS, int BWD>
static hipError_t convpr_launch_t(const ConvnArgs& a0, int ns, hipStream_t st, int grid_mul = 1) {
  constexpr int WNT = P1Cfg<BN>::WNT;
  using G = Geo<128, BN, WNT, 3>;
  static bool attr = false;
  if (!attr) {
    const hipError_t e = hipFuncSetAttribute((const void*)convpr_kernel<BN, WNT, STATS, BWD>,
                                             hipFuncAttributeMaxDynamicSharedMemorySize, 160 * 1024);
    if (e != hipSuccess) return e;
    attr = true;
  }
  ConvnArgs a = a0;
  a.nslot = ns;
  const int lds = (a.K / kBK) * BN * 128 + ns * 128 * 128 + G::NW * G::STG;
  const int tiles_m = (a.M + 127) / 128, tiles_n = a.N / BN;
  int gx = convp_grid_x(tiles_m, tiles_n) * grid_mul;
  if (gx > tiles_m) gx = tiles_m;
  hipLaunchKernelGGL((convpr_kernel<BN, WNT, STATS, BWD>), dim3(gx, tiles_n), dim3(G::NT), lds, st, a, tiles_m);
  return hipGetLastError();
}

template <int BN>
static hipError_t convpr_launch_s(const ConvnArgs& a, int ns, hipStream_t st, int gm = 1) {
  if (a.bwd == 1) return convpr_launch_t<BN, false, 1>(a, ns, st, gm);
  if (a.bwd == 2) return convpr_launch_t<BN, false, 2>(a, ns, st, gm);
  if (a.bwd == 3) return convpr_launch_t<BN, false, 3>(a, ns, st, gm);
  if (a.bwd == 5) return convpr_launch_t<BN, false, 5>(a, ns, st, gm);
  if (a.bwd == 8) return convpr_launch_t<BN, false, 8>(a, ns, st, gm);
  return a.part ? convpr_launch_t<BN, true, 0>(a, ns, st, gm) : convpr_launch_t<BN, false, 0>(a, ns, st, gm);
}

template <int BN>
static hipError_t convp_launch_s(const ConvnArgs& a, hipStream_t st, int gm = 1) {
  if (const int ns = pr_slots<BN>(a.K)) return convpr_launch_s<BN>(a, ns, st, gm);
  if (a.bwd == 1) return convp_launch_t<BN, false, 1>(a, st, gm);
  if (a.bwd == 2) return convp_launch_t<BN, false, 2>(a, st, gm);
  if (a.bwd == 3) return convp_launch_t<BN, false, 3>(a, st, gm);
  if (a.bwd == 5) return convp_launch_t<BN, false, 5>(a, st, gm);
  if (a.bwd == 8) return convp_launch_t<BN, false, 8>(a, st, gm);
  return a.part ? convp_launch_t<BN, true, 0>(a, st, gm) : convp_launch_t<BN, false, 0>(a, st, gm);
}

template <int BN>
static hipError_t convp2_launch_s(const ConvnArgs& a, hipStream_t st) {
  using G = Geo<128, BN, P1Cfg<BN>::WNT, 3>;
  const int lds2 = (a.K / kBK) * BN * 128 + 2 * 128 * 128 + G::NW * G::STG;
  if (lds2 <= 80 * 1024) return convpr_launch_s<BN>(a, 2, st, 2);
  return convp_launch_s<BN>(a, st, 2);
}

static hipError_t convp2_launch(const ConvnArgs& a, int bn, hipStream_t st) {
  if (a.R != 1 || a.S != 1 || a.stride != 1 || a.pad != 0 || a.Ho != a.H || a.Wo != a.W) return hipErrorNotSupported;
  if (bn == 256) return convp2_launch_s<256>(a, st);
  if (bn == 128) return convp2_launch_s<128>(a, st);
  return convp2_launch_s<64>(a, st);
}

static hipError_t convp_launch(const ConvnArgs& a, int bn, hipStream_t st) {
  if (a.R != 1 || a.S != 1 || a.stride != 1 || a.pad != 0 || a.Ho != a.H || a.Wo != a.W) return hipErrorNotSupported;
  if (bn == 256) return convp_launch_s<256>(a, st);
  if (bn == 128) return convp_launch_s<128>(a, st);
  return convp_launch_s<64>(a, st);
}

template <int BM, int BN, int WNT, int NSLOT, bool STATS, int BWD>
static hipError_t convn_launch_t(const ConvnArgs& a0, hipStream_t st) {
  using G = Geo<BM, BN, WNT, NSLOT>;
  constexpr int LDS_MAX = NSLOT * G::SLOT + G::NW * G::STG;
  static_assert(LDS_MAX <= 160 * 1024, "LDS");
  static bool attr = false;
  if (!attr) {
    const hipError_t e = hipFuncSetAttribute((const void*)convn_kernel<BM, BN, WNT, NSLOT, STATS, BWD>,
                                             hipFuncAttributeMaxDynamicSharedMemorySize, LDS_MAX);
    if (e != hipSuccess) return e;
    attr = true;
  }
  ConvnArgs a = a0;
  const int nt = a.K / kBK;
  a.nslot = nt < NSLOT ? (nt < 2 ? 1 : nt) : NSLOT;
  const int lds = a.nslot * G::SLOT + G::NW * G::STG;
  const int tiles_m = (a.M + BM - 1) / BM;
  hipLaunchKernelGGL((convn_kernel<BM, BN, WNT, NSLOT, STATS, BWD>), dim3(tiles_m, a.N / BN), dim3(G::NT), lds, st, a);
  return hipGetLastError();
}

template <int BM, int BN, int WNT, int NSLOT>
static hipError_t convn_launch_s(const ConvnArgs& a, hipStream_t st) {
  if (a.bwd == 1) return convn_launch_t<BM, BN, WNT, NSLOT, false, 1>(a, st);
  if (a.bwd == 2) return convn_launch_t<BM, BN, WNT, NSLOT, false, 2>(a, st);
  if (a.bwd == 3) return convn_launch_t<BM, BN, WNT, NSLOT, false, 3>(a, st);
  if (a.bwd == 5) return convn_launch_t<BM, BN, WNT, NSLOT, false, 5>(a, st);
  if (a.bwd == 8) return convn_launch_t<BM, BN, WNT, NSLOT, false, 8>(a, st);
  return a.part ? convn_launch_t<BM, BN, WNT, NSLOT, true, 0>(a, st)
                : convn_launch_t<BM, BN, WNT, NSLOT, false, 0>(a, st);
}

int convn_tile_n(int N) {
  if (N == 64) return 64;
  if (N == 128) return 128;
  if (N % 256 == 0) return 256;
  return 0;
}

static int plain_count(int bn) { return bn == 256 ? 3 : 4; }
static int persist_count(int bn) { return bn == 64 ? 1 : 0; }
static int p1_count(int bn) { return bn ? 2 : 0; }
static int convn_variant_count(int bn) { return plain_count(bn) + persist_count(bn) + p1_count(bn); }
static bool is_persist(int bn, int v) { return v >= plain_count(bn) && v < plain_count(bn) + persist_count(bn); }
static bool is_p1(int bn, int v) { return v == plain_count(bn) + persist_count(bn); }
static bool is_p2(int bn, int v) { return v == plain_count(bn) + persist_count(bn) + 1; }

int convn_variant_kind(int N, int v) {
  const int bn = convn_tile_n(N);
  if (!bn || v < 0 || v >= convn_variant_count(bn)) return -1;
  return v < plain_count(bn) ? 0 : is_persist(bn, v) ? 2 : is_p1(bn, v) ? 3 : 4;
}

int convn_variants(int N) {
  const int bn = convn_tile_n(N);
  return bn ? convn_variant_count(bn) : 0;
}

static int default_variant(const ConvnArgs& a, int bn) {
  (void)a;
  (void)bn;
  return 0;
}

static int variant_bm(int bn, int v) {
  if (is_persist(bn, v) || is_p1(bn, v) || is_p2(bn, v)) return 128;
  if (bn == 64) return (v == 2 || v == 3) ? 256 : 128;
  if (bn == 128) return v == 2 ? 256 : 128;
  return 128;
}

bool convn_variant_ok(int N, int v, int R, int S, int stride, int pad, int Wo, bool has_x2) {
  const int bn = convn_tile_n(N);
  if (!bn || v < 0 || v >= convn_variant_count(bn)) return false;
  if (v < plain_count(bn)) return true;
  if (is_p1(bn, v) || is_p2(bn, v)) return R == 1 && S == 1 && stride == 1 && pad == 0;
  return !has_x2 && N == 64 && R == 3 && S == 3 && stride == 1 && pad == 1 && Wo + 2 <= 64;
}

int convn_stats_rows(int M) { return 4 * ((M + 255) / 256) + 4; }

int convn_part_rows_geo(int M, int N, int variant, int Ho, int Wo, int R) {
  const int bn = convn_tile_n(N);
  if (!bn) return 0;
  const int bm = variant_bm(bn, variant);
  if (is_persist(bn, variant)) {
    if (Ho <= 0 || Wo <= 0) return 0;
    return 2 * convh_grid((M / (Ho * Wo)) * ((Ho + 1) / 2));
  }
  if (is_p1(bn, variant)) return 2 * convp_grid_x((M + 127) / 128, N / bn);
  if (is_p2(bn, variant)) {
    const int t = (M + 127) / 128, g = 2 * convp_grid_x(t, N / bn);
    return 2 * (g < t ? g : t);
  }
  return (bm / 64) * ((M + bm - 1) / bm);
}

int convn_part_rows(int M, int N, int variant) { return convn_part_rows_geo(M, N, variant, 0, 0, 1); }

hipError_t launch_convn(const ConvnArgs& a_in, hipStream_t st) {
  if (a_in.M <= 0) return hipSuccess;
  ConvnArgs a = a_in;
  if (!a.x2) a.K1 = a.K;
  const int bn = convn_tile_n(a.N);
  const int C = 1 << a.logC;
  const bool two = a.x2 != nullptr;
  const int K1 = two ? a.K1 : a.K;
  const bool ok = bn > 0 && a.logC >= 6 && a.K % kBK == 0 && K1 == a.R * a.S * C && a.ldc % 8 == 0 &&
                  (!two || (a.R == 1 && a.S == 1 && a.stride == 1 && a.pad == 0 && a.logC2 >= 6 && K1 % kBK == 0 &&
                            a.K == K1 + (1 << a.logC2) && a.x2bytes > 0 && a.x2bytes <= 0xFFFFFF00u)) &&
                  a.ldc >= a.N && a.H < 32768 && a.W < 32768 && a.xbytes > 0 && a.xbytes <= 0xFFFFFF00u &&
                  a.wbytes > 0 && a.variant < convn_variant_count(bn) &&
                  (a.y || (a.bwd == 0 && a.part)) &&
                  (a.bwd == 0 ? (!a.part || a.shift)
                   : a.bwd == 8 ? (!a.part && a.bss && a.amask && a.ldc == a.N && a.N % 8 == 0)
                              : (a.part && (a.bx || a.bwd >= 2) && a.bmean && a.ldc == a.N &&
                                 (a.bwd == 1 ? a.bss != nullptr
                                             : ((a.bwd == 2 || a.bwd == 3 || a.bwd == 5) && a.bdr && a.bmbits &&
                                                (a.bwd != 3 || (a.bxd && a.bmean_d && a.part_d)) &&
                                                (a.bwd != 5 || (a.Ho % 2 == 0 && a.Wo % 2 == 0))))));
  if (!ok) return hipErrorNotSupported;
  if (a.ophase != 0 &&
      (a.ophase > 4 || a.variant < 0 || a.variant >= plain_count(bn) || two || a.stride != 1 || a.pad != 0 ||
// ... 30 lines not shown
```

### parameter_server_distributed_amd/csrc/kernels/launchers_convn.h

```cpp
#pragma once
#include <hip/hip_runtime_api.h>
#include <cstdint>

namespace psd {

struct ConvnArgs {
  const void* x;
  const void* w;
  void* y;
  float* part;
  const float* shift;
  uint32_t xbytes;
  uint32_t wbytes;
  int M, N, K;
  int H, W, logC, Ho, Wo, R, S, stride, pad;
  int ldc;
  int variant;
  int nslot;
  int bwd;
  const uint16_t* bx;
  const float* bmean;
  const float* bss;
  const uint16_t* bdr;
  const uint8_t* bmbits;
  const uint16_t* bxd;
  const float* bmean_d;
  float* part_d;
  const void* x2;
  uint32_t x2bytes;
  int K1, logC2;
  const float* bias;
  const uint16_t* ares;
  uint8_t* amask;
  int ophase;
};

int convn_tile_n(int N);
int convn_stats_rows(int M);
int convn_part_rows(int M, int N, int variant);
int convn_part_rows_geo(int M, int N, int variant, int Ho, int Wo, int R);
bool convn_variant_ok(int N, int v, int R, int S, int stride, int pad, int Wo, bool has_x2);
int convn_variants(int N);
int convn_variant_kind(int N, int v);
hipError_t launch_convn(const ConvnArgs& a, hipStream_t stream);

}
```

### parameter_server_distributed_amd/csrc/ops.h

```cpp
#pragma once
#include <ATen/ATen.h>
#include <tuple>
#include <vector>

namespace psd {

using ScaleList = std::vector<c10::optional<at::Tensor>>;
using MxScaleList = std::vector<at::Tensor>;

void fused_apply_(at::Tensor master, const std::vector<at::Tensor>& grads, c10::optional<at::Tensor> state1,
                  c10::optional<at::Tensor> state2, c10::optional<at::Tensor> shadow, at::Tensor dyn, int64_t kind,
                  double momentum, double dampening, bool nesterov, double weight_decay, double beta1, double beta2,
                  double eps, bool maximize, int64_t grid_cap = 0, const ScaleList& scales = {},
                  const MxScaleList& mx_scales = {});
std::vector<at::Tensor> lw_table_build(const std::vector<int64_t>& offsets, const std::vector<int64_t>& numels,
                                       const std::vector<int64_t>& ndims, int64_t n, bool exclude_1d, int64_t align,
                                       const at::Device& device);
void fused_apply_lw_(at::Tensor master, const std::vector<at::Tensor>& grads, c10::optional<at::Tensor> state1,
                     c10::optional<at::Tensor> state2, c10::optional<at::Tensor> shadow, at::Tensor dyn, int64_t kind,
                     double momentum, double dampening, bool nesterov, double weight_decay, double beta1, double beta2,
                     double eps, bool maximize, double trust_coef, const std::vector<at::Tensor>& layers,
                     int64_t grid_cap = 0, const ScaleList& scales = {}, const MxScaleList& mx_scales = {});
void optim_advance_(at::Tensor dyn, double beta1, double beta2);
void multi_reduce_(at::Tensor out, const std::vector<at::Tensor>& srcs, double scale, const ScaleList& scales = {},
                   const MxScaleList& mx_scales = {});
void push_quant_mx_(const at::Tensor& x, at::Tensor q, at::Tensor scales, int64_t blocks_per_seg = 0,
                    c10::optional<at::Tensor> residual = c10::nullopt);
void grad_clip_coef_(const at::Tensor& flat, double clip_norm, at::Tensor out, at::Tensor partials,
                     int64_t grid_cap = 0);
void pack_cast_(const std::vector<at::Tensor>& srcs, const std::vector<at::Tensor>& dsts);
void xfer_(const std::vector<at::Tensor>& srcs, const std::vector<at::Tensor>& dsts, int64_t blocks_per_seg,
           bool nt_store);
void amax_(const at::Tensor& x, at::Tensor amax_out);
void quant_fp8_(const at::Tensor& x, const at::Tensor& amax, double fp8_max, at::Tensor out, at::Tensor scale_inv);
void quant_fp8_jit_(const at::Tensor& x, at::Tensor out, at::Tensor scale_inv);
void quant_fp8_delayed_(const at::Tensor& x, at::Tensor out, at::Tensor scale_inv, at::Tensor hist, double margin);
void dequant_fp8_(const at::Tensor& x, const at::Tensor& scale_inv, at::Tensor out);
void quant_mx_(const at::Tensor& x, at::Tensor out, at::Tensor scales);
void dequant_mx_(const at::Tensor& q, const at::Tensor& scales, at::Tensor out);
void quant_mx_t_(const at::Tensor& x, at::Tensor out, at::Tensor scales);
void quant_mx_dual_(const at::Tensor& x, at::Tensor q_row, at::Tensor s_row, at::Tensor q_t, at::Tensor s_t);

std::vector<at::Tensor> bn_fwd(const at::Tensor& x, c10::optional<at::Tensor> gamma, c10::optional<at::Tensor> beta,
                               c10::optional<at::Tensor> running_mean, c10::optional<at::Tensor> running_var,
                               c10::optional<at::Tensor> residual, bool relu, bool training, double momentum, double eps,
                               c10::optional<at::Tensor> counter, c10::optional<at::Tensor> ss_eval,
                               bool mask_out, c10::optional<at::Tensor> residual_ss, bool stats_only,
                               c10::optional<at::Tensor> q8_out, c10::optional<at::Tensor> part_in,
                               int64_t part_rows, c10::optional<at::Tensor> q8_mx);
at::Tensor bn_reduce_(const at::Tensor& x, const at::Tensor& shift);
at::Tensor bn_bwd_reduce_(const at::Tensor& dy, const at::Tensor& x, const at::Tensor& save_mean,
                          c10::optional<at::Tensor> ss, c10::optional<at::Tensor> dy2,
                          c10::optional<at::Tensor> mbits);
std::vector<at::Tensor> bn_bwd_dual(const at::Tensor& dy, const at::Tensor& x, const at::Tensor& gamma,
                                    const at::Tensor& save_mean, const at::Tensor& save_invstd, const at::Tensor& mbits,
                                    c10::optional<at::Tensor> dy2, const at::Tensor& xd, const at::Tensor& gamma_d,
                                    const at::Tensor& mean_d, const at::Tensor& invstd_d,
                                    c10::optional<at::Tensor> dgamma_out, c10::optional<at::Tensor> dbeta_out,
                                    c10::optional<at::Tensor> dgamma_d_out, c10::optional<at::Tensor> dbeta_d_out, bool fold);
at::Tensor bn_elemt_coef(const at::Tensor& g, const at::Tensor& x, const at::Tensor& coef);
std::vector<at::Tensor> bn_bwd_dual_pre(const at::Tensor& g, const at::Tensor& x, const at::Tensor& gamma,
                                        const at::Tensor& save_mean, const at::Tensor& save_invstd,
                                        const at::Tensor& part, const at::Tensor& part_d, int64_t rows,
                                        const at::Tensor& xd, const at::Tensor& gamma_d, const at::Tensor& mean_d,
                                        const at::Tensor& invstd_d, c10::optional<at::Tensor> dgamma_out,
                                        c10::optional<at::Tensor> dbeta_out, c10::optional<at::Tensor> dgamma_d_out,
                                        c10::optional<at::Tensor> dbeta_d_out, bool fold, bool fold_d, bool derive_d);
std::vector<at::Tensor> bnfold_dgrad_weights(const at::Tensor& w, const at::Tensor& coef);
void bnfold_combine(const at::Tensor& P, const at::Tensor& w, const at::Tensor& coef, at::Tensor out, bool accumulate);
void bnfold_rowdot(const at::Tensor& P, const at::Tensor& w, at::Tensor row);
void bnfold_gram_stats(const at::Tensor& P, const at::Tensor& w, const at::Tensor& shift, int64_t M, at::Tensor row);
std::vector<at::Tensor> bnfold_dual_weights(const at::Tensor& w3, const at::Tensor& wd, const at::Tensor& ss3,
                                            const at::Tensor& ssd);
std::vector<at::Tensor> bn_finalize(const at::Tensor& part, int64_t rows, int64_t M, const at::Tensor& gamma,
                                    const at::Tensor& beta, at::Tensor running_mean, at::Tensor running_var,
                                    double momentum, double eps, c10::optional<at::Tensor> counter);
std::vector<at::Tensor> bn_bwd_coef(const at::Tensor& dy, const at::Tensor& x, const at::Tensor& gamma,
                                    const at::Tensor& save_mean, const at::Tensor& save_invstd,
                                    c10::optional<at::Tensor> mbits, c10::optional<at::Tensor> dy2,
                                    c10::optional<at::Tensor> part, int64_t rows, c10::optional<at::Tensor> dgamma_out,
                                    c10::optional<at::Tensor> dbeta_out);
std::vector<at::Tensor> bn_bwd(const at::Tensor& dy, const at::Tensor& x, c10::optional<at::Tensor> y,
                               c10::optional<at::Tensor> gamma, const at::Tensor& save_mean,
                               const at::Tensor& save_invstd, bool relu, bool need_dr,
                               c10::optional<at::Tensor> dgamma_out, c10::optional<at::Tensor> dbeta_out,
                               c10::optional<at::Tensor> dy2, c10::optional<at::Tensor> ss,
                               c10::optional<at::Tensor> mbits, c10::optional<at::Tensor> dq, c10::optional<at::Tensor> dqmx);

int64_t gemm_(const at::Tensor& A, const at::Tensor& B, bool a_kmajor, bool b_kmajor, at::Tensor out,
              c10::optional<at::Tensor> bias, int64_t act, c10::optional<at::Tensor> aux,
              c10::optional<at::Tensor> part, c10::optional<at::Tensor> shift);
int64_t gemm_stats_rows_(int64_t M);
struct GemmArgs;
void set_stats(GemmArgs& a, const c10::optional<at::Tensor>& part, const c10::optional<at::Tensor>& shift,
               const at::Tensor& out, int* rows);
bool gemm_ct_(const at::Tensor& A, const at::Tensor& B, at::Tensor out, c10::optional<at::Tensor> bias, int64_t act,
              c10::optional<at::Tensor> aux);
bool gemm_gelu_bwd_(const at::Tensor& A, const at::Tensor& B, bool a_kmajor, bool b_kmajor, const at::Tensor& pre,
                    at::Tensor out, at::Tensor db, bool accumulate);
void gemm_splitk_(const at::Tensor& A, const at::Tensor& B, bool a_kmajor, bool b_kmajor, at::Tensor out,
                  bool accumulate, double scale, int64_t splits);
void colsum_(const at::Tensor& x, at::Tensor out, bool accumulate);
void gelu_bwd_colsum_(const at::Tensor& dy, const at::Tensor& pre, at::Tensor dx, at::Tensor out, bool accumulate);
int64_t convn_part_rows_(int64_t M, int64_t N, int64_t v, int64_t Ho, int64_t Wo, int64_t R);
bool convn_variant_ok_(int64_t N, int64_t v, int64_t R, int64_t S, int64_t stride, int64_t pad, int64_t Wo, bool has_x2);
int64_t convn_(const at::Tensor& x, const at::Tensor& w2, at::Tensor out, int64_t R, int64_t S, int64_t stride,
               int64_t pad, c10::optional<at::Tensor> part, c10::optional<at::Tensor> shift, int64_t variant,
               c10::optional<at::Tensor> x2, c10::optional<at::Tensor> bias, bool no_store,
               c10::optional<at::Tensor> apply_ss, c10::optional<at::Tensor> apply_res,
               c10::optional<at::Tensor> apply_mask);
int64_t convn_stats_rows_(int64_t M);
int64_t convn_dgrad_s2_(const at::Tensor& dy, const std::vector<at::Tensor>& wph, at::Tensor out, int64_t variant,
                        c10::optional<at::Tensor> part, c10::optional<at::Tensor> bx, c10::optional<at::Tensor> bmean,
                        c10::optional<at::Tensor> bss);
int64_t convn_dgrad_s2_rows(int64_t Nb, int64_t Ho, int64_t Wo, int64_t Ci, int64_t variant);
int64_t convn_bwd_(const at::Tensor& dy, const at::Tensor& w2, at::Tensor out, int64_t R, int64_t S, int64_t stride,
                   int64_t pad, at::Tensor part, int64_t variant, int64_t mode, c10::optional<at::Tensor> bx,
                   const at::Tensor& bmean, c10::optional<at::Tensor> bss, c10::optional<at::Tensor> bdr,
                   c10::optional<at::Tensor> bmbits, c10::optional<at::Tensor> x2,
                   c10::optional<at::Tensor> bias, c10::optional<at::Tensor> bxd, c10::optional<at::Tensor> bmean_d,
                   c10::optional<at::Tensor> part_d);
std::vector<at::Tensor> bn_bwd_pre(const at::Tensor& g, const at::Tensor& x, c10::optional<at::Tensor> gamma,
                                   const at::Tensor& save_mean, const at::Tensor& save_invstd, const at::Tensor& part,
                                   int64_t rows, c10::optional<at::Tensor> dgamma_out,
                                   c10::optional<at::Tensor> dbeta_out, c10::optional<at::Tensor> dq,
                                   c10::optional<at::Tensor> dqmx);
int64_t convn_variants_(int64_t N);
int64_t convn_variant_kind_(int64_t N, int64_t v);
int64_t conv_fwd_(const at::Tensor& x, const at::Tensor& w2, at::Tensor out, int64_t R, int64_t S, int64_t stride,
                  int64_t pad, c10::optional<at::Tensor> part, c10::optional<at::Tensor> shift);
bool conv_wgrad_(const at::Tensor& dy, const at::Tensor& x, at::Tensor out, int64_t R, int64_t S, int64_t stride,
                 int64_t pad, int64_t splits);
bool convw_(const at::Tensor& dy, const at::Tensor& x, at::Tensor out, int64_t R, int64_t S, int64_t stride,
            int64_t pad, int64_t variant, bool accumulate, bool fold);
int64_t convw_fold_rows(int64_t Cout, int64_t Cin);
int64_t convw_gram_rows_(int64_t C);
bool convw_gram_(const at::Tensor& x, at::Tensor out, int64_t variant);
int64_t convw_variants_(int64_t Cout, int64_t KK);
int64_t conv_fwd_fp8_(const at::Tensor& x, const at::Tensor& w2, const at::Tensor& x_scale, const at::Tensor& w_scale,
                      at::Tensor out, int64_t R, int64_t S, int64_t stride, int64_t pad, c10::optional<at::Tensor> part,
                      c10::optional<at::Tensor> shift);
int64_t gemm_fp8_(const at::Tensor& A, const at::Tensor& B, const at::Tensor& a_scale, const at::Tensor& b_scale,
                  at::Tensor out, c10::optional<at::Tensor> bias, int64_t act, c10::optional<at::Tensor> aux,
                  c10::optional<at::Tensor> part, c10::optional<at::Tensor> shift);
void gemm_fp8_splitk_(const at::Tensor& A, const at::Tensor& B, const at::Tensor& a_scale, const at::Tensor& b_scale,
                      at::Tensor out, bool accumulate, double scale, int64_t splits);
std::vector<at::Tensor> maxpool3s2_fwd(const at::Tensor& x);
at::Tensor maxpool3s2_bwd(const at::Tensor& dy, const at::Tensor& arg, int64_t H, int64_t W,
                          const c10::optional<at::Tensor>& dy2);
at::Tensor gap_fwd(const at::Tensor& x);
std::vector<at::Tensor> bn_pool_fwd(const at::Tensor& x, const at::Tensor& gamma, const at::Tensor& beta,
                                    const at::Tensor& running_mean, const at::Tensor& running_var, double momentum,
                                    double eps, c10::optional<at::Tensor> counter);
std::vector<at::Tensor> stem_fwd(const at::Tensor& x, const at::Tensor& w, const at::Tensor& gamma, const at::Tensor& beta,
                                 const at::Tensor& running_mean, const at::Tensor& running_var, double momentum,
                                 double eps, c10::optional<at::Tensor> counter);
at::Tensor stem_wgrad(const at::Tensor& x, const at::Tensor& dy);
std::vector<at::Tensor> attn_fwd(const at::Tensor& qkv, int64_t heads, double p, int64_t seed,
                                 c10::optional<at::Tensor> step, c10::optional<at::Tensor> lens, int64_t grid_cap,
                                 bool causal, c10::optional<at::Tensor> doc_start = c10::nullopt, int64_t window = 0);
at::Tensor attn_bwd(const at::Tensor& dout, const at::Tensor& qkv, const at::Tensor& o, const at::Tensor& lse,
                    int64_t heads, double p, int64_t seed, c10::optional<at::Tensor> step,
                    c10::optional<at::Tensor> bias_out, c10::optional<at::Tensor> lens, int64_t grid_cap,
                    bool causal, c10::optional<at::Tensor> doc_start = c10::nullopt, int64_t window = 0);
at::Tensor rope_(at::Tensor qkv, int64_t heads, const at::Tensor& cos, const at::Tensor& sin,
                 c10::optional<at::Tensor> lens, c10::optional<at::Tensor> doc_start, bool inverse, int64_t blocks);
std::vector<at::Tensor> rms_fwd(const at::Tensor& r, c10::optional<at::Tensor> h, const at::Tensor& gamma, double eps,
                                double p, int64_t seed, c10::optional<at::Tensor> step);
std::vector<at::Tensor> rms_bwd(const at::Tensor& dy, c10::optional<at::Tensor> dr_new, const at::Tensor& r_new,
                                const at::Tensor& rstd, const at::Tensor& gamma, double p, int64_t seed,
                                c10::optional<at::Tensor> step, bool had_h, c10::optional<at::Tensor> dgamma_out);
at::Tensor swiglu_fwd(const at::Tensor& gu, int64_t blocks);
at::Tensor swiglu_bwd(const at::Tensor& da, const at::Tensor& gu, int64_t blocks);
std::vector<at::Tensor> ln_fwd(const at::Tensor& x, const at::Tensor& h, const at::Tensor& gamma, const at::Tensor& beta,
                               double eps, double p, int64_t seed, c10::optional<at::Tensor> step,
                               c10::optional<at::Tensor> q8_out = c10::nullopt,
                               c10::optional<at::Tensor> sc8_out = c10::nullopt);
std::vector<at::Tensor> ln_bwd(const at::Tensor& dy, const at::Tensor& s, const at::Tensor& mean, const at::Tensor& rstd,
                               const at::Tensor& gamma, double p, int64_t seed, c10::optional<at::Tensor> step,
                               c10::optional<at::Tensor> dgamma_out, c10::optional<at::Tensor> dbeta_out,
                               c10::optional<at::Tensor> dhsum_out);
std::vector<at::Tensor> emb_ln_fwd(const at::Tensor& ids, const at::Tensor& types, const at::Tensor& W,
                                   const at::Tensor& P, const at::Tensor& T, const at::Tensor& gamma,
                                   const at::Tensor& beta, int64_t S, double eps, double p, int64_t seed,
                                   c10::optional<at::Tensor> step, c10::optional<at::Tensor> pos_ids = c10::nullopt);
std::vector<at::Tensor> emb_ln_bwd(const at::Tensor& dy, const at::Tensor& ids, const at::Tensor& types,
                                   const at::Tensor& W, const at::Tensor& P, const at::Tensor& T,
                                   const at::Tensor& gamma, const at::Tensor& mean, const at::Tensor& rstd, int64_t S,
                                   double p, int64_t seed, c10::optional<at::Tensor> step,
                                   c10::optional<at::Tensor> dgamma_out, c10::optional<at::Tensor> dbeta_out,
                                   c10::optional<at::Tensor> dT_out, c10::optional<at::Tensor> pos_ids = c10::nullopt);
std::vector<at::Tensor> bn_pool_bwd(const at::Tensor& gpool, c10::optional<at::Tensor> gpool2, const at::Tensor& arg,
                                    const at::Tensor& x, const at::Tensor& gamma, const at::Tensor& save_mean,
                                    const at::Tensor& save_invstd, const at::Tensor& ss,
                                    c10::optional<at::Tensor> dgamma_out, c10::optional<at::Tensor> dbeta_out);
at::Tensor gap_bwd(const at::Tensor& dy, int64_t H, int64_t W);
at::Tensor subsample2(const at::Tensor& x);

std::tuple<at::Tensor, int64_t> wprep_table(const std::vector<at::Tensor>& srcs, const std::vector<at::Tensor>& dsts,
                                            const std::vector<int64_t>& geo);
void wprep_run(const at::Tensor& table, int64_t tiles);

void embed_bwd_(const at::Tensor& sorted, const at::Tensor& perm, const at::Tensor& dy, at::Tensor out);
std::vector<at::Tensor> xent_fwd(const at::Tensor& x, const at::Tensor& labels);
at::Tensor xent_bwd(const at::Tensor& x, const at::Tensor& labels, const at::Tensor& lse, const at::Tensor& scale,
                    c10::optional<at::Tensor> lse_lo);

}
```

### parameter_server_distributed_amd/ops/conv.py

```python
from __future__ import annotations


import functools

import torch
import torch.nn as nn
import torch.nn.functional as F

from ..utils.config import feature as _feat
from . import wprep as _wprep
from . import autotune as _at
from .handover import (BwdPre, StatsPending, StridedDr, bn_momentum, fold_v as _fold_v, pop_dr, same, sinks, take,
                       take_dr)


def _enabled() -> bool:
    return _feat("conv1x1")


def _choose(key: tuple, candidates: dict) -> str:
    return _at.choose(("conv1x1",) + key, candidates, "miopen")


def decisions() -> dict:
# ... 53 lines not shown
def _q_weight(mod, w2: torch.Tensor):
    if _mx_on():
        return mx_weight(mod, w2)
    return _q8(w2)


def _take_dq8(mod, dy: torch.Tensor):
    return take(mod, "_psd_dq8_pending", dy, strides=True)


def _take_q8(mod, x: torch.Tensor):
    return take(mod, "_psd_q8_pending", x, strides=True)




def _psdn_ok(cin: int, cout: int) -> bool:
    return cin >= 64 and (cin & (cin - 1)) == 0 and (cout in (64, 128) or cout % 256 == 0) and \
        _feat("convn")


def _bn_consumer(mod):
    bn = getattr(mod, "_psd_bn", None) if mod is not None else None
    if bn is None or not bn.training or bn.running_mean is None or not _feat("convn_stats"):
        return None
    return bn


class _Lazy:
    __slots__ = ("fn", "t", "shape")

    def __init__(self, fn, shape):
        self.fn, self.t, self.shape = fn, None, tuple(shape)

    def __call__(self) -> torch.Tensor:
        if self.t is None:
            self.t = self.fn()
        return self.t


def _wt(w2: torch.Tensor, mod=None, weight=None) -> _Lazy:
    def make():
        t = _wprep.get(mod, weight, "t") if weight is not None else None
        return t if t is not None else w2.t().contiguous()
    return _Lazy(make, (w2.shape[1], w2.shape[0]))


def _wflip(mod, weight: torch.Tensor) -> torch.Tensor:
    t = _wprep.get(mod, weight, "f")
    if t is not None:
        return t
    cout, cin, k, _ = weight.shape
    return weight.flip(2, 3).permute(1, 2, 3, 0).reshape(cin, k * k * cout).contiguous()


def _get(w):
    return w() if isinstance(w, _Lazy) else w


def _out_hw(h: int, w: int, k: int, stride: int, pad: int) -> tuple:
    return (h + 2 * pad - k) // stride + 1, (w + 2 * pad - k) // stride + 1


def _convn_variants(x, w2, k: int, stride: int, pad: int, bn=None) -> dict:
    C = _native()
    n, _, h, w = x.shape
    cout = w2.shape[0]
    ho, wo = _out_hw(h, w, k, stride, pad)
    M = n * ho * wo

    def make(v, stats):
        def fn():
            out = torch.empty(M, cout, device=x.device, dtype=x.dtype)
            part = None
            if stats:
                part = torch.empty(_part_rows(M, cout, v, ho, wo, k), 2, cout, device=x.device, dtype=torch.float32)
            rows = C.convn_(x, _get(w2), out, k, k, stride, pad, part=part,
                            shift=bn.running_mean if stats else None, variant=v)
            if rows == 0:
                raise RuntimeError("convn_ declined a shape _psdn_ok accepted")
            y = _from_2d(out, n, ho, wo)
            if stats:
                bn._psd_stats_pending = StatsPending(y, part, rows)
            return y
        return fn

    ok = [v for v in range(C.convn_variants(cout)) if _variant_ok(cout, v, k, stride, pad, wo, x.shape[1], h)]
    cands = {f"psdn{v}": make(v, bn is not None) for v in ok}
    if bn is not None:
        cands.update({f"psdu{v}": make(v, False) for v in ok})
    return cands


def _variant_ok(cout: int, v: int, k: int, stride: int, pad: int, wo: int, cin: int | None = None,
                h: int | None = None) -> bool:
    C = _native()
    if not C.convn_variant_ok(cout, v, k, k, stride, pad, wo):
        return False
    kind = C.convn_variant_kind(cout, v)
    if kind == 2:
        return _feat("convn_persist") and cin == 64 and (h is None or h == wo)
    if kind == 3:
        return _feat("convn_p1")
    if kind == 4:
        return _feat("convn_p1") and _feat("convn_p2")
    return kind == 0


def _part_rows(M: int, N: int, v: int, ho: int, wo: int, k: int) -> int:
    C = _native()
    return max(C.convn_stats_rows(M), C.convn_part_rows(M, N, v, ho, wo, k))


def _fwd_records(ctx, mod) -> None:
    ctx.bn_in = getattr(mod, "_psd_bn_in", None) if mod is not None else None
    ctx.strided_to = getattr(mod, "_psd_strided_to", None) if mod is not None else None


def _bn_bwd_fusion(bn, x: torch.Tensor):
    st = getattr(bn, "_psd_fwd", None) if bn is not None else None
    if st is None or not _feat("convn_bwd"):
        return None
    y, bx, mean, ss, mbits, xd, mean_d = st
    if not same(y, x, strides=True):
        return None
    if mbits is not None:
        if not bn._psd_pending_dr:
            return None
        if isinstance(bn._psd_pending_dr[-1], StridedDr):
            if xd is not None or x.shape[2] % 2 or x.shape[3] % 2 or not _feat("convn_bwd5"):
                return None
            return dict(mode=5, bn=bn, bx=bx, mean=mean, mbits=mbits)
        if xd is not None:
            if not _feat("convn_bwd3"):
                return None
            return dict(mode=3, bn=bn, bx=bx, mean=mean, mbits=mbits, bxd=xd, mean_d=mean_d)
        return dict(mode=2, bn=bn, bx=bx, mean=mean, mbits=mbits)
    return dict(mode=1, bn=bn, bx=bx, mean=mean, ss=ss)


def _take_dr_for(fu) -> None:
    if fu is not None:
        fu["dr"] = fu["bn"]._psd_pending_dr.pop() if fu["mode"] >= 2 else None


def _convn_bwd_launch(dy, w2, cout: int, k: int, pad: int, v: int, fu: dict, prows: int, declined: str,
                      x2=None, bias=None) -> torch.Tensor:
    n, _, h, w = dy.shape
    out = torch.empty(n * h * w, cout, device=dy.device, dtype=dy.dtype)
    part = torch.empty(prows, 2, cout, device=dy.device, dtype=torch.float32)
    part_d = torch.empty_like(part) if fu["mode"] == 3 else None
    rows = _native().convn_bwd_(dy, w2, out, k, k, 1, pad, part, v, fu["mode"], fu["bx"], fu["mean"],
                                bss=fu.get("ss"), bdr=_dr_arg(fu.get("dr")), bmbits=fu.get("mbits"), x2=x2,
                                bias=bias, bxd=fu.get("bxd"), bmean_d=fu.get("mean_d"), part_d=part_d)
    if rows == 0:
        raise RuntimeError(declined)
    g = _from_2d(out, n, h, w)
    fu["bn"]._psd_bwd_pre = BwdPre(g, part, rows, part_d)
    return g


def _convn_bwd_variants(dy, w2, k: int, pad: int, fu: dict) -> dict:
    C = _native()
    n, _, h, w = dy.shape
    cout = w2.shape[0]

    def make(v):
        return lambda: _convn_bwd_launch(dy, _get(w2), cout, k, pad, v, fu, _part_rows(n * h * w, cout, v, h, w, k) + 1,
                                         "convn_bwd_ declined a shape _psdn_ok accepted")

    return {f"psdnb{v}": make(v) for v in range(C.convn_variants(cout))
            if _variant_ok(cout, v, k, 1, pad, w, dy.shape[1], h)}


def _s2_phase_weights(weight: torch.Tensor) -> list:
    cin = weight.shape[1]
    sel = (lambda t, d: t.narrow(d, 1, 1), lambda t, d: t[(slice(None),) * d + (slice(None, None, 2),)].flip(d))
    out = []
    for ph in (0, 1):
        for pw in (0, 1):
            wsel = sel[pw](sel[ph](weight, 2), 3)
            out.append(wsel.permute(1, 2, 3, 0).reshape(cin, -1).contiguous())
    return out


def _dgrad_s2_phases(dy, weight, x, fu, mod=None) -> dict:
    C = _native()
    n, cin, h, w = x.shape
    ho, wo = dy.shape[2], dy.shape[3]
    def phases():
        got = _wprep.get(mod, weight, "p")
        return got if got is not None else _s2_phase_weights(weight)

    wph = _Lazy(phases, (4,))

    def make(v, fused):
        def fn():
            out = torch.empty(n * h * w, cin, device=dy.device, dtype=dy.dtype)
            if fused:
                part = torch.empty(C.convn_dgrad_s2_rows(n, ho, wo, cin, v) + 1, 2, cin, device=dy.device,
                                   dtype=torch.float32)
                rows = C.convn_dgrad_s2_(dy, wph(), out, v, part=part, bx=fu["bx"], bmean=fu["mean"], bss=fu["ss"])
            else:
                rows = C.convn_dgrad_s2_(dy, wph(), out, v)
            if rows == 0:
                raise RuntimeError("convn_dgrad_s2_ declined a shape it was offered for")
            g = _from_2d(out, n, h, w)
            if fused:
                fu["bn"]._psd_bwd_pre = BwdPre(g, part, rows)
            return g
        return fn

    cands = {}
    for v in range(C.convn_variants(cin)):
        if C.convn_variant_kind(cin, v) != 0 or not C.convn_variant_ok(cin, v, 2, 2, 1, 0, wo, False):
            continue
        cands[f"psdns{v}"] = make(v, False)
        if fu is not None:
            cands[f"psdnbs{v}"] = make(v, True)
    return cands


def _dgrad_route(key: tuple, cands: dict, default: str, fu, dy_like, timed=None, defer=None):
    timed = cands if timed is None else timed
    if fu is None:
        how = _at.choose(key, timed, default)
        return cands[how]() if how != defer else None
    if fu.get("bx") is None:
        cands = {name: fn for name, fn in cands.items() if name.startswith("psdnb")}
        if not cands:
            raise RuntimeError("psd: a BN without its stored input needs the fused bwd-data epilogue")
        key, default = key + ("nobx",), next(iter(cands))
    timed = {n: (timed[n] if n.startswith("psdnb") else _with_bn_bwd_reduce(timed[n], fu)) for n in cands}
    how = _at.choose(key + ("bnbwd",), timed, default, group=lambda n: n.startswith("psdnb"))
    out = cands[how]() if how != defer else None
    if not how.startswith("psdnb"):
        fu["bn"]._psd_bwd_pre = None
        if fu.get("dr") is not None:
            fu["bn"]._psd_pending_dr.append(fu["dr"])
    return out


def _with_bn_reduce(fn, bn):
    def g():
        y = fn()
        _native().bn_reduce_(y, bn.running_mean)
        return y
    return g


def _with_bn_bwd_reduce(fn, fu):
    def g():
        dx = fn()
        _native().bn_bwd_reduce_(dx, fu["bx"], fu["mean"], ss=fu.get("ss"), dy2=take_dr(fu.get("dr")),
                                 mbits=fu.get("mbits"))
        return dx
    return g


def _stats_part(bn, M: int, cout: int, device):
    if bn is None or not _feat("gemm_stats"):
        return None
    return torch.empty(_native().gemm_stats_rows(M), 2, cout, device=device, dtype=torch.float32)


def _hand_stats(bn, y, part, rows: int):
    if part is not None and rows > 0:
        bn._psd_stats_pending = StatsPending(y, part, rows)


def _dr_arg(dr):
    return dr.t4 if isinstance(dr, StridedDr) else dr


def _route(key: tuple, cands: dict, default: str, bn=None) -> str:
    if bn is None:
        return _at.choose(key, cands, default)
    timed = {name: (fn if name.startswith(("psdn", "psds")) else _with_bn_reduce(fn, bn))
             for name, fn in cands.items()}
    how = _at.choose(key + ("bnstats",), timed, default)
    bn._psd_stats_pending = None
    return how


def _convw_cands(dy, x, k: int, stride: int, pad: int) -> dict:
    if not _feat("convw"):
        return {}
    C = _native()
    cout, cin = dy.shape[1], x.shape[1]
    kk = k * k * cin
    if cin < 64 or (cin & (cin - 1)) or not (cout in (64, 128) or cout % 256 == 0):
        return {}

    def make(v):
        def fn(into=None):
            o = into if into is not None else torch.empty(cout, kk, device=dy.device, dtype=dy.dtype)
            if not C.convw_(dy, x, o, k, k, stride, pad, variant=v):
                raise _at.Declined(f"convw_ variant {v}")
            return o.view(cout, k, k, cin).permute(0, 3, 1, 2)
        return fn

    nv = C.convw_variants(cout, kk)
    persist = 1 if (cout == 64 and kk == 576) else 0
    shapes = (nv - persist) // 2
    vs = [v for v in range(nv) if (v < shapes or _feat("convw_twostage")) and (v < 2 * shapes or _feat("convw_persist"))]
    return {f"psdw{v}": make(v) for v in vs}

# ... 606 lines not shown
```

### parameter_server_distributed_amd/ops/tail.py

```python
from __future__ import annotations

import types

import torch

from ..utils.config import feature as _feat
from . import autotune as _at
from .conv import (Conv1x1, ConvNHWC, _fold_backward, _fold_v, _from_2d, _fwd_records, _native, _part_rows, _sink_view,
                   _write_dw, fold_ok)
from .bn import FusedBatchNorm2d
from .handover import (BnFwd, FoldPending, StridedDr, bn_momentum, dual_from_fold, pop_dr, route_res_grad, sinks,
                       take)

__all__ = ["tail_ok", "conv_bn_tail", "dual_tail_ok", "conv_bn_dual_tail", "TAIL_CALLS"]

TAIL_CALLS = {"fwd": 0, "bwd_fused": 0, "bwd_recompute": 0, "dual_fwd": 0, "dual_bwd_fused": 0,
              "dual_bwd_recompute": 0}


def tail_ok(conv, bn, a2: torch.Tensor, idt: torch.Tensor) -> bool:
    if not (_feat("tail_recompute") and _feat("convn")) or not isinstance(conv, Conv1x1):
        return False
    tail8 = conv.fp8 and _feat("tail_fp8") and getattr(bn, "_psd_fold_conv", None) is conv
    if conv.fp8 and not tail8:
        return False
    if not isinstance(bn, FusedBatchNorm2d) or not bn.relu or not bn.training or bn.weight is None:
        return False
    if not (a2.is_cuda and a2.dtype == torch.bfloat16 and idt.dtype == torch.bfloat16 and torch.is_grad_enabled()):
        return False
    if conv.weight.dtype != torch.bfloat16 or (getattr(bn, "_psd_q8_consumer", None) is not None and not tail8):
        return False
    cin, cout = conv.in_channels, conv.out_channels
    if idt.shape != (a2.shape[0], cout, a2.shape[2], a2.shape[3]):
        return False
    if not (a2.is_contiguous(memory_format=torch.channels_last) and idt.is_contiguous(memory_format=torch.channels_last)):
        return False
    C = _native()
    return fold_ok(cin, cout) and C.convn_variants(cout) > 0 and (a2.shape[0] * a2.shape[2] * a2.shape[3]) % 8 == 0


def _kind_ok(kind: int) -> bool:
    return kind in (0, 3) or (kind == 4 and _feat("convn_p2"))


def _variant(a2, w2, M: int, cin: int, cout: int, h: int, w: int, shift) -> int:
    C = _native()
    dev = a2.device
    scratch = []

    def make(v):
        def fn():
            if not scratch:
                scratch.extend((torch.zeros(M, cout, device=dev, dtype=torch.bfloat16),
                                torch.zeros(2 * cout, device=dev, dtype=torch.float32)))
            res, ss = scratch
            out = torch.empty(M, cout, device=dev, dtype=torch.bfloat16)
            mb = torch.empty(M * cout // 8, device=dev, dtype=torch.uint8)
            if C.convn_(a2, w2, out, 1, 1, 1, 0, variant=v, apply_ss=ss, apply_res=res, apply_mask=mb) == 0:
                raise _at.Declined("convn apply pass")
            return out
        return fn

    cands = {f"psdn{v}": make(v) for v in range(C.convn_variants(cout))
             if _kind_ok(C.convn_variant_kind(cout, v)) and C.convn_variant_ok(cout, v, 1, 1, 1, 0, w)}
    how = _at.choose(("tail", "apply", M, cin, cout), cands, next(iter(cands)))
    return int(how[4:])


def _stats_route(a2, w2, M: int, cin: int, cout: int, v: int, h: int, w: int, shift) -> str:
    C = _native()
    if not _feat("tail_gram") or C.convw_gram_rows(cin) <= 0 or cout % 4:
        return "pass"
    dev = a2.device

    def gram():
        P = torch.empty(C.convw_gram_rows(cin), cin, device=dev, dtype=torch.float32)
        if not C.convw_gram_(a2, P, variant=_fold_v()):
            raise _at.Declined("convw Gram launch")
        row = torch.empty(2, cout, device=dev, dtype=torch.float32)
        C.bnfold_gram_stats(P, w2, shift, M, row)
        return row

    def pas():
        part = torch.empty(_part_rows(M, cout, v, h, w, 1), 2, cout, device=dev, dtype=torch.float32)
        rows = C.convn_(a2, w2, part, 1, 1, 1, 0, part=part, shift=shift, variant=v, no_store=True)
        if rows == 0:
            raise _at.Declined("convn statistics-only pass")
        return part[:rows].sum(0)

    return _at.choose(("tail", "stats", M, cin, cout), {"gram": gram, "pass": pas}, "pass")


def _conv1x1_bwd(dy, x, weight, need_x: bool, need_w: bool):
    return torch.ops.aten.convolution_backward(dy, x, weight, None, [1, 1], [0, 0], [1, 1], False, [0, 0], 1,
                                               [need_x, need_w, False])


class _TailFn(torch.autograd.Function):
    @staticmethod
    def forward(ctx, a2, weight, gamma, beta, idt, conv, bn, resid_to):
        C = _native()
        n, cin, h, w = a2.shape
        cout = weight.shape[0]
        M = n * h * w
        w2 = weight.reshape(cout, cin)
        if not w2.is_contiguous():
            w2 = w2.contiguous()
        v = _variant(a2, w2, M, cin, cout, h, w, bn.running_mean)
        if _stats_route(a2, w2, M, cin, cout, v, h, w, bn.running_mean) == "gram":
            P = torch.empty(C.convw_gram_rows(cin), cin, device=a2.device, dtype=torch.float32)
            if not C.convw_gram_(a2, P, variant=_fold_v()):
                raise RuntimeError("psd tail: convw declined the Gram launch")
            part = torch.empty(1, 2, cout, device=a2.device, dtype=torch.float32)
            C.bnfold_gram_stats(P, w2, bn.running_mean, M, part[0])
            rows = 1
        else:
            part = torch.empty(_part_rows(M, cout, v, h, w, 1), 2, cout, device=a2.device, dtype=torch.float32)
            rows = C.convn_(a2, w2, part, 1, 1, 1, 0, part=part, shift=bn.running_mean, variant=v, no_store=True)
            if rows == 0:
                raise RuntimeError("psd tail: convn declined the statistics-only pass")
        mean, invstd, ss = C.bn_finalize(part, rows, M, gamma, beta, bn.running_mean, bn.running_var,
                                         bn_momentum(bn), bn.eps, bn.num_batches_tracked)
        out = torch.empty(M, cout, device=a2.device, dtype=torch.bfloat16)
        mbits = torch.empty(M * cout // 8, device=a2.device, dtype=torch.uint8)
        if C.convn_(a2, w2, out, 1, 1, 1, 0, variant=v, apply_ss=ss, apply_res=idt, apply_mask=mbits) == 0:
            raise RuntimeError("psd tail: convn declined the apply pass")
        y = _from_2d(out, n, h, w)
        bn._psd_fwd = BnFwd(y, None, mean, ss, mbits)
        ctx.mod = conv
        _fwd_records(ctx, conv)
        ctx.bn, ctx.resid_to, ctx.v = bn, resid_to, v
        ctx.save_for_backward(a2, weight, gamma, mean, invstd, mbits)
        TAIL_CALLS["fwd"] += 1
        return y

    @staticmethod
    def backward(ctx, dy):
        a2, weight, gamma, mean, invstd, mbits = ctx.saved_tensors
        C = _native()
        bn = ctx.bn
        bn._psd_fwd = None
        n, cin, h, w = a2.shape
        cout = weight.shape[0]
        M = n * h * w
        dgo, dbo = sinks(bn)
        pre = take(bn, "_psd_bwd_pre", dy, strides=False)
        need_x, need_w = ctx.needs_input_grad[0], ctx.needs_input_grad[1]
        if pre is not None and pre.part_d is None:
            g, part, rows = pre[:3]
            if part.shape[0] <= rows:
                raise RuntimeError("psd tail: the partials buffer has no row for sum g y")
            P = torch.empty(C.convw_fold_rows(cout, cin), cin, device=dy.device, dtype=torch.float32)
            if not C.convw_(g, a2, P, 1, 1, 1, 0, variant=_fold_v(), fold=True):
                raise RuntimeError("psd tail: convw_ declined the fold wgrad")
            C.bnfold_rowdot(P, weight, part[rows])
            g, coef, dg, db = C.bn_bwd_coef(g, g, gamma, mean, invstd, part=part, rows=rows + 1, dgamma_out=dgo,
                                            dbeta_out=dbo)
            y = None
            TAIL_CALLS["bwd_fused"] += 1
        else:
            P = None
            w2 = weight.reshape(cout, cin).contiguous()
            out = torch.empty(M, cout, device=dy.device, dtype=torch.bfloat16)
            if C.convn_(a2, w2, out, 1, 1, 1, 0, variant=ctx.v) == 0:
                raise RuntimeError("psd tail: convn declined the recompute")
            y = _from_2d(out, n, h, w)
            g, coef, dg, db = C.bn_bwd_coef(dy, y, gamma, mean, invstd, mbits=mbits, dy2=pop_dr(bn), dgamma_out=dgo,
                                            dbeta_out=dbo)
            TAIL_CALLS["bwd_recompute"] += 1
        res_grad = route_res_grad(ctx.resid_to, g)
        dx, dw, dyu = _fold_backward(ctx, FoldPending(g, coef, y, P), a2, weight, need_x, need_w)
        if dyu is not None:
            dx, dw, _ = _conv1x1_bwd(dyu, a2, weight, need_x, need_w)
            dw = _write_dw(_sink_view(ctx.mod, weight), lambda: dw, None)
        return dx, dw, dg, db, res_grad, None, None, None


def conv_bn_tail(conv, bn, a2: torch.Tensor, idt: torch.Tensor, resid_to=None) -> torch.Tensor:
    return _TailFn.apply(a2, conv.weight, bn.weight, bn.bias, idt, conv, bn, resid_to)




def dual_tail_ok(conv3, bn3, a2: torch.Tensor, convd, bnd, xin: torch.Tensor) -> bool:
    if not (_feat("tail_recompute") and _feat("dual_recompute") and _feat("convn") and _feat("bn_fold")):
        return False
    if not isinstance(conv3, Conv1x1) or conv3.fp8 or getattr(convd, "fp8", False):
        return False
    strided = _ds_stride(convd)
    if strided is None:
        return False
    if not (isinstance(bn3, FusedBatchNorm2d) and isinstance(bnd, FusedBatchNorm2d) and bn3.relu and not bnd.relu
            and bn3.training and bnd.training and bn3.weight is not None and bnd.weight is not None):
        return False
    if getattr(bn3, "_psd_q8_consumer", None) is not None or not torch.is_grad_enabled():
        return False
    for t in (a2, xin):
        if not (t.is_cuda and t.dtype == torch.bfloat16 and t.dim() == 4
                and t.is_contiguous(memory_format=torch.channels_last)):
            return False
    if a2.shape[0] != xin.shape[0] or a2.shape[2] * strided != xin.shape[2] or a2.shape[3] * strided != xin.shape[3]:
        return False
    if conv3.weight.dtype != torch.bfloat16 or convd.weight.dtype != torch.bfloat16:
        return False
    c3, cd, cout = conv3.in_channels, convd.in_channels, conv3.out_channels
    if convd.out_channels != cout or a2.shape[1] != c3 or xin.shape[1] != cd or cout % 4:
        return False
    C = _native()
    if not (fold_ok(c3, cout) and fold_ok(cd, cout) and C.convw_gram_rows(c3) > 0 and C.convw_gram_rows(cd) > 0):
        return False
    n, _, h, w = a2.shape
    return (n * h * w) % 8 == 0 and any(_dual_variants(cout, w))


def _ds_stride(convd):
    if isinstance(convd, Conv1x1):
        return 1
    if isinstance(convd, ConvNHWC) and convd.kernel_size == (1, 1) and convd.stride == (2, 2) \
            and convd.padding == (0, 0) and convd.groups == 1:
        return 2
    return None


def _dual_variants(cout: int, w: int) -> list:
    C = _native()
    return [v for v in range(C.convn_variants(cout))
            if _kind_ok(C.convn_variant_kind(cout, v)) and C.convn_variant_ok(cout, v, 1, 1, 1, 0, w, True)]


def _gram_moments(x, w2, shift, M: int) -> torch.Tensor:
    C = _native()
    cin = x.shape[1]
    P = torch.empty(C.convw_gram_rows(cin), cin, device=x.device, dtype=torch.float32)
    if not C.convw_gram_(x, P, variant=_fold_v()):
        raise RuntimeError("psd dual tail: convw declined the Gram launch")
    part = torch.empty(1, 2, w2.shape[0], device=x.device, dtype=torch.float32)
    C.bnfold_gram_stats(P, w2, shift, M, part[0])
    return part


def _finalize(bn, part, M: int):
    return _native().bn_finalize(part, 1, M, bn.weight, bn.bias, bn.running_mean, bn.running_var, bn_momentum(bn),
                                 bn.eps, bn.num_batches_tracked)


def dual_weights_reference(w3_2, wd_2, ss3, ss_d):
    cout = w3_2.shape[0]
    s3, sd = ss3[:cout], ss_d[:cout]
    big3 = s3.abs() >= sd.abs()
    sbig = torch.where(big3, s3, sd)
    safe = torch.where(sbig == 0, torch.ones_like(sbig), sbig)
    r3 = torch.where(big3, torch.ones_like(s3), s3 / safe)
    rd = torch.where(big3, sd / safe, torch.ones_like(sd))
    r3 = torch.where(sbig == 0, torch.zeros_like(r3), r3)
    rd = torch.where(sbig == 0, torch.zeros_like(rd), rd)
    wcat = torch.cat([w3_2.float() * r3[:, None], wd_2.float() * rd[:, None]], 1).to(torch.bfloat16)
    return wcat, torch.cat([sbig, ss3[cout:] + ss_d[cout:]])


class _DualTailFn(torch.autograd.Function):
    @staticmethod
    def forward(ctx, a2, w3, g3, b3, xfull, wd, gd, bd, conv3, bn3, convd, bnd):
        C = _native()
        ctx.full_hw = tuple(xfull.shape[2:])
        ctx.stride = _ds_stride(convd)
        xin = xfull if ctx.stride == 1 else C.subsample2(xfull)
        n, c3, h, w = a2.shape
        cd, cout = xin.shape[1], w3.shape[0]
        M = n * h * w
        w3_2, wd_2 = w3.reshape(cout, c3).contiguous(), wd.reshape(cout, cd).contiguous()
        mean3, invstd3, ss3 = _finalize(bn3, _gram_moments(a2, w3_2, bn3.running_mean, M), M)
        mean_d, invstd_d, ss_d = _finalize(bnd, _gram_moments(xin, wd_2, bnd.running_mean, M), M)
        wcat, ssc = C.bnfold_dual_weights(w3_2, wd_2, ss3, ss_d)
        out = torch.empty(M, cout, device=a2.device, dtype=torch.bfloat16)
        mbits = torch.empty(M * cout // 8, device=a2.device, dtype=torch.uint8)

        def make(v):
            def fn():
                o = torch.empty(M, cout, device=a2.device, dtype=torch.bfloat16)
                mb = torch.empty(M * cout // 8, device=a2.device, dtype=torch.uint8)
                if C.convn_(a2, wcat, o, 1, 1, 1, 0, variant=v, x2=xin, apply_ss=ssc, apply_mask=mb) == 0:
                    raise _at.Declined("convn dual apply pass")
                return o
            return fn

        cands = {f"psdn{v}": make(v) for v in _dual_variants(cout, w)}
        v = int(_at.choose(("tail", "dual_apply", M, c3, cd, cout), cands, next(iter(cands)))[4:])
        if C.convn_(a2, wcat, out, 1, 1, 1, 0, variant=v, x2=xin, apply_ss=ssc, apply_mask=mbits) == 0:
            raise RuntimeError("psd dual tail: convn declined the apply pass")
        y = _from_2d(out, n, h, w)
        bn3._psd_fwd = BnFwd(y, None, mean3, None, mbits)
        ctx.r3, ctx.rd = types.SimpleNamespace(mod=conv3), types.SimpleNamespace(mod=convd)
        _fwd_records(ctx.r3, conv3)
        _fwd_records(ctx.rd, convd)
        ctx.bn3, ctx.bnd, ctx.v = bn3, bnd, v
        ctx.save_for_backward(a2, w3, g3, mean3, invstd3, xin, wd, gd, mean_d, invstd_d, mbits)
        TAIL_CALLS["dual_fwd"] += 1
        return y

    @staticmethod
    def backward(ctx, dy):
        a2, w3, g3, mean3, invstd3, xin, wd, gd, mean_d, invstd_d, mbits = ctx.saved_tensors
        C = _native()
        bn3, bnd = ctx.bn3, ctx.bnd
        bn3._psd_fwd = None
        (dg3o, db3o), (dgdo, dbdo) = sinks(bn3), sinks(bnd)
        n, c3, h, w = a2.shape
        cd, cout = xin.shape[1], w3.shape[0]
        M = n * h * w
        pre = take(bn3, "_psd_bwd_pre", dy, strides=False)
        need = ctx.needs_input_grad
        if pre is not None and pre.part_d is None:
            g = pre.g
            Ps, dg3, db3, dgd, dbd, coef, coef_d = dual_from_fold(
                pre, w3, a2, wd, xin, g, g3, mean3, invstd3, g, gd, mean_d, invstd_d, (dg3o, db3o), (dgdo, dbdo))
            dxa, dw3, _ = _fold_backward(ctx.r3, FoldPending(g, coef, None, Ps[0]), a2, w3, need[0], need[1])
            dxi, dwd, _ = _fold_backward(ctx.rd, FoldPending(g, coef_d, None, Ps[1]), xin, wd, need[4], need[5])
            TAIL_CALLS["dual_bwd_fused"] += 1
            return dxa, dw3, dg3, db3, _DualTailFn._input_grad(ctx, dxi), dwd, dgd, dbd, None, None, None, None
        ys = []
        for inp, wt, cin in ((a2, w3, c3), (xin, wd, cd)):
            o = torch.empty(M, cout, device=dy.device, dtype=torch.bfloat16)
            if C.convn_(inp, wt.reshape(cout, cin).contiguous(), o, 1, 1, 1, 0, variant=0) == 0:
                raise RuntimeError("psd dual tail: convn declined the recompute")
            ys.append(_from_2d(o, n, h, w))
        dx3, dxd, dg3, db3, dgd, dbd = C.bn_bwd_dual(dy, ys[0], g3, mean3, invstd3, mbits, pop_dr(bn3), ys[1], gd,
                                                     mean_d, invstd_d, dg3o, db3o, dgdo, dbdo)
        dxa, dw3, _ = _conv1x1_bwd(dx3, a2, w3, need[0], need[1])
        dxi, dwd, _ = _conv1x1_bwd(dxd, xin, wd, need[4], need[5])
        dw3 = _write_dw(_sink_view(ctx.r3.mod, w3), lambda: dw3, None)
        dwd = _write_dw(_sink_view(ctx.rd.mod, wd), lambda: dwd, None)
        TAIL_CALLS["dual_bwd_recompute"] += 1
        return dxa, dw3, dg3, db3, _DualTailFn._input_grad(ctx, dxi), dwd, dgd, dbd, None, None, None, None

    @staticmethod
    def _input_grad(ctx, dxi):
        if dxi is None or ctx.stride == 1:
            return dxi
        H, W = ctx.full_hw
        dr = StridedDr(dxi if dxi.is_contiguous(memory_format=torch.channels_last)
                       else dxi.contiguous(memory_format=torch.channels_last), H, W)
        to = ctx.rd.strided_to
        if isinstance(to, FusedBatchNorm2d):
            to._psd_pending_dr.append(dr)
            n, c = dxi.shape[:2]
            return torch.zeros((), device=dxi.device, dtype=dxi.dtype).expand(n, c, H, W)
        return dr.full()


def conv_bn_dual_tail(conv3, bn3, a2: torch.Tensor, convd, bnd, xin: torch.Tensor) -> torch.Tensor:
    return _DualTailFn.apply(a2, conv3.weight, bn3.weight, bn3.bias, xin, convd.weight, bnd.weight, bnd.bias,
                             conv3, bn3, convd, bnd)
```

### parameter_server_distributed_amd/utils/config.py

```python
from __future__ import annotations

import argparse
import json
import os


def load_config(path: str) -> dict:
    with open(path) as f:
        text = f.read()
    if path.endswith(".json"):
        cfg = json.loads(text)
    else:
        import yaml

        cfg = yaml.safe_load(text) or {}
    if not isinstance(cfg, dict):
        raise ValueError(f"{path}: a run config must be a mapping of option -> value")
    return {str(k).replace("-", "_"): v for k, v in cfg.items()}


def apply_config(ap: argparse.ArgumentParser, argv: list[str] | None = None) -> None:
    pre = argparse.ArgumentParser(add_help=False)
    pre.add_argument("--config", default=os.environ.get("PSD_CONFIG", ""))
    known, _ = pre.parse_known_args(argv)
    if not any(a.dest == "config" for a in ap._actions):
        ap.add_argument("--config", default="", help="YAML/JSON run config (flags override it)")
    if not known.config:
        return
    cfg = load_config(known.config)
    dests = {a.dest for a in ap._actions}
    unknown = sorted(set(cfg) - dests)
    if unknown:
        raise SystemExit(f"{known.config}: unknown option(s) {unknown}")
    ap.set_defaults(**cfg)


FEATURES: dict[str, tuple[bool, str]] = {
    "conv1x1": (True, "per-shape routing of 1x1 convolutions (MIOpen / hipBLASLt / MFMA); off: MIOpen only"),
    "conv1x1_mfma": (True, "the 8-phase MFMA GEMM as a 1x1-convolution candidate"),
    "conv_igemm": (True, "implicit-GEMM MFMA convolution (gemm.hip) as a forward / bwd-data candidate"),
    "conv_wgrad": (True, "implicit-GEMM MFMA weight gradient as a candidate"),
    "convn": (True, "narrow implicit-GEMM convolution kernels (convn.hip) as candidates"),
    "convn_stats": (True, "consumer-BN statistics in the narrow convolution's epilogue"),
    "convn_persist": (True, "persistent layer-1 3x3 kernel (convh)"),
    "convn_p1": (True, "persistent 1x1 kernels (convp / convpr)"),
    "convn_p2": (True, "the persistent 1x1 kernel at two workgroups per CU (two-slot ring) as a candidate"),
    "convn_bwd": (True, "producing BN's backward reduction in the bwd-data epilogue (modes 1/2)"),
    "convn_bwd3": (True, "the dual-BN tail's reduction in the bwd-data epilogue (mode 3)"),
    "convn_bwd5": (True, "stride-2 downsample gradient added on the quarter grid (mode 5)"),
    "dgrad_s2_phase": (True, "stride-2 3x3 bwd-data as four output-parity phase launches of the narrow kernel "
                              "(with the producing BN's backward reduction in the epilogue) vs MIOpen"),
    "convw": (True, "narrow weight-gradient kernel (convw.hip) as a candidate"),
    "convw_persist": (True, "persistent layer-1 3x3 weight gradient (convhw)"),
    "convw_twostage": (True, "narrow weight-gradient tiles also on a two-stage ring at two workgroups per CU"),
    "convw_fold2": (True, "the BN-fold and Gram weight-gradient launches on the two-stage ring (two workgroups per CU)"),
    "gemm_stats": (True, "consumer-BN statistics in the 8-phase GEMM epilogue"),
    "library_candidates": (False, "convolutions: autotune also times MIOpen / hipBLASLt candidates wherever one of "
                                  "our kernels takes the shape; off (default): our kernels only there, the library "
                                  "only as the fallback -- same-box ResNet-50 15,681 / 15,695 vs 15,557 / 15,591 "
                                  "img/s with them (profiles/r6/ab_library_candidates.md)"),
    "library_linear": (True, "Linear layers: hipBLASLt stays an autotune candidate (BERT-base same-box 9,576 / 9,505 "
                             "vs 9,297 / 9,362 seq/s without it: it wins the QKV forward, the attention-output "
                             "bwd-data and the MLM-head weight gradient in the step, profiles/r6/ab_library_candidates.md)"),
    "prefer_own": (True, "autotune: our kernel takes a pick a library candidate wins by < 2 % (ops/autotune.py OWN_MARGIN)"),
    "wprep": (True, "every convolution's bwd-data weight operand (transpose / tap flip / stride-2 phases) in one batched launch per step (ops/wprep.py)"),
    "bn_fold": (True, "bn3's backward folded into conv3's bwd-data / weight-gradient GEMMs"),
    "bn_fold_ds": (True, "the stride-1 downsample BN folded into its convolution's backward"),
    "dual_nobx": (True, "downsample blocks' dual tail without the BN inputs in the consumer epilogue"),
    "tail_recompute": (True, "identity blocks' conv3 output recomputed instead of stored"),
    "tail_gram": (True, "the recomputing tail's statistics from the Gram matrix of conv3's input"),
    "dual_recompute": (True, "stride-1 downsample blocks: neither conv3's nor the downsample conv's output stored"),
    "fp8_compute": (True, "fp8 convolutions / Linear layers where the model asks for them"),
    "fp8_mx": (True, "MX block scales for every fp8 operand; off: per-tensor scales"),
    "fp8_mx_handover": (True, "BN passes write the consumer's MX e4m3 input / producer's MX e5m2 dY"),
    "fp8_delayed": (True, "per-tensor fp8: delayed (previous-call amax) scaling"),
    "fp8_dgrad": (True, "fp8 e5m2-dY bwd-data of the fp8 convolutions and fp8 Linear layers"),
    "fp8_wgrad": (False, "fp8 e4m3 x e4m3 split-K weight gradient of the fp8 Linear layers (tokens % 128 == 0); off: bf16"),
    "fp8_ln_handover": (True, "the fused LayerNorm writes the MX e4m3 input of the fp8 Linear that consumes it"),
    "async_cached_local": (True, "async PS at world 1: inbox / publish buffers in plain (cached) device memory "
                                 "instead of uncached IPC memory (AsyncPS hands it to the native engine)"),
    "async_apply_background": (True, "async PS with SSP bound >= 1: the owner's apply on a normal-priority stream "
                                     "with at most 512 workgroups, beside the compute stream (AsyncPS hands it to "
                                     "the native engine); off: high priority, full grid (the S = 0 setting)"),
    "async_direct_pull": (True, "async PS at world 1: each step pulls straight into the model's working weights "
                                "on the compute stream (one local copy) instead of prefetching into a second "
                                "buffer and copying that into the working weights"),
    "tail_fp8": (False, "fp8 models' identity blocks: conv3 + bn3 as the bf16 recomputing tail (bn3 folded "
                       "into conv3's bf16 backward, conv3's output never stored); read at model build. Off: same-box "
                       "WRN-101-2 4,136 vs 4,170 img/s (profiles/r6/ab_tail_fp8.md)"),
    "linear_tune": (True, "per-shape MFMA / hipBLASLt choice for Linear layers; off: MFMA only"),
    "gelu_fuse": (True, "GELU backward in the consumer Linear's bwd-data GEMM epilogue"),
    "attn_bias": (True, "QKV bias gradient handed over by the attention backward"),
    "attn_long": (True, "streaming fused attention kernels for S = 192 .. 512 (multiples of 64); off: SDPA on "
                        "transposed views there, as for every other S > 128"),
    "attn_xlong": (True, "the streaming fused attention kernels also at S = 576 .. 4096 (multiples of 64; needs "
                         "attn_long); off: S > 512 goes back to SDPA on transposed views"),
    "rope": (True, "in-place rotary position embedding kernel on the packed QKV (ops/rope.py RotaryQK); off: the "
                   "out-of-place torch composite rope_ref"),
    "rmsnorm": (True, "fused residual add + dropout + RMSNorm kernels (ops/rmsnorm.py FusedAddRMSNorm); off: the "
                      "torch composite add_rmsnorm_ref"),
    "swiglu": (True, "gated SiLU kernels on the packed gate/up tensor (ops/swiglu.py SwiGLU); off: the torch "
                     "composite swiglu_ref"),
}

_FEAT_ENV: str | None = None
_FEAT_OVR: dict[str, bool] = {}
_FEAT_SET: dict[str, bool] = {}


def _feature_env() -> dict[str, bool]:
    global _FEAT_ENV, _FEAT_OVR
    raw = os.environ.get("PSD_FEATURES", "")
    if raw != _FEAT_ENV:
        ovr = {}
        for item in filter(None, (t.strip() for t in raw.split(","))):
            name, _, val = item.partition("=")
            name = name.strip()
            if name not in FEATURES:
                raise ValueError(f"PSD_FEATURES: unknown feature {name!r} (known: {sorted(FEATURES)})")
            ovr[name] = val.strip() not in ("0", "false", "off", "no")
        _FEAT_ENV, _FEAT_OVR = raw, ovr
    return _FEAT_OVR


def feature(name: str) -> bool:
    if name in _FEAT_SET:
        return _FEAT_SET[name]
    ovr = _feature_env()
    if name in ovr:
        return ovr[name]
    return FEATURES[name][0]


def set_feature(name: str, on: bool | None) -> None:
    if name not in FEATURES:
        raise ValueError(f"unknown feature {name!r}")
    if on is None:
        _FEAT_SET.pop(name, None)
    else:
        _FEAT_SET[name] = bool(on)


def features() -> dict[str, bool]:
    return {n: feature(n) for n in FEATURES}


FAULTS: dict[str, tuple[int, str]] = {
    "stop_heartbeat_after": (-1, "worker: stop sending coordinator heartbeats after n of them"),
    "push_delay_ms": (0, "worker: sleep this long before every gradient push"),
    "exit_after_push": (-1, "worker: exit the process right after its k-th push"),
    "selftest_fail_rank": (-1, "async PS: this rank reports a failed start-up self-test"),
    "selftest_fail_kernel": (-1, "async PS: this rank fails the kernel-transport self-test attempt only"),
}


def fault(name: str) -> int:
    if name not in FAULTS:
        raise ValueError(f"unknown fault key {name!r}")
    for item in filter(None, (t.strip() for t in os.environ.get("PSD_FAULT", "").split(","))):
        k, _, v = item.partition("=")
        if k.strip() == name:
            return int(v)
    return FAULTS[name][0]
```

Before: 16340.

## Prefetch persistent 1x1 conv epilogue operands one tile ahead

In the persistent 1x1 convolution kernels (convp/convpr) with 256-wide tiles and epilogue modes 2, 5 and 8, the epilogue's global operands (residual/dr, mask bytes, BN input) are issued as buffer loads one tile ahead, interleaved into the current tile's epilogue. Per-column constants (bias, scale/shift, means) are hoisted out of the tile loop. This hides the epilogue's load latency behind the next tile's main loop, at the cost of more registers, extra vmcnt bookkeeping in the wait logic and a dummy stage past the last tile. It is controlled by a new feature flag that is on by default.

```diff
diff --git a/parameter_server_distributed_amd/csrc/bindings.cpp b/parameter_server_distributed_amd/csrc/bindings.cpp
--- a/parameter_server_distributed_amd/csrc/bindings.cpp
+++ b/parameter_server_distributed_amd/csrc/bindings.cpp
@@ -114,7 +114,8 @@
   m.def("convn_", &convn_, py::arg("x"), py::arg("w2"), py::arg("out"), py::arg("R"), py::arg("S"), py::arg("stride"),
         py::arg("pad"), py::arg("part") = py::none(), py::arg("shift") = py::none(), py::arg("variant") = -1,
         py::arg("x2") = py::none(), py::arg("bias") = py::none(), py::arg("no_store") = false,
-        py::arg("apply_ss") = py::none(), py::arg("apply_res") = py::none(), py::arg("apply_mask") = py::none());
+        py::arg("apply_ss") = py::none(), py::arg("apply_res") = py::none(), py::arg("apply_mask") = py::none(),
+        py::arg("epi_prefetch") = true);
   m.def("convn_stats_rows", &convn_stats_rows_, py::arg("M"));
   m.def("convn_part_rows", &convn_part_rows_, py::arg("M"), py::arg("N"), py::arg("variant"), py::arg("Ho"),
         py::arg("Wo"), py::arg("R"));
@@ -129,7 +130,7 @@
         py::arg("stride"), py::arg("pad"), py::arg("part"), py::arg("variant"), py::arg("mode"), py::arg("bx"),
         py::arg("bmean"), py::arg("bss") = py::none(), py::arg("bdr") = py::none(), py::arg("bmbits") = py::none(),
         py::arg("x2") = py::none(), py::arg("bias") = py::none(), py::arg("bxd") = py::none(),
-        py::arg("bmean_d") = py::none(), py::arg("part_d") = py::none());
+        py::arg("bmean_d") = py::none(), py::arg("part_d") = py::none(), py::arg("epi_prefetch") = true);
   m.def("bn_bwd_pre", &bn_bwd_pre, py::arg("g"), py::arg("x"), py::arg("gamma"), py::arg("save_mean"),
         py::arg("save_invstd"), py::arg("part"), py::arg("rows"), py::arg("dgamma_out") = py::none(),
         py::arg("dbeta_out") = py::none(), py::arg("dq") = py::none(), py::arg("dqmx") = py::none());
diff --git a/parameter_server_distributed_amd/csrc/conv_ops.cpp b/parameter_server_distributed_amd/csrc/conv_ops.cpp
--- a/parameter_server_distributed_amd/csrc/conv_ops.cpp
+++ b/parameter_server_distributed_amd/csrc/conv_ops.cpp
@@ -231,7 +231,7 @@
                int64_t pad, c10::optional<at::Tensor> part, c10::optional<at::Tensor> shift, int64_t variant,
                c10::optional<at::Tensor> x2, c10::optional<at::Tensor> bias, bool no_store,
                c10::optional<at::Tensor> apply_ss, c10::optional<at::Tensor> apply_res,
-               c10::optional<at::Tensor> apply_mask) {
+               c10::optional<at::Tensor> apply_mask, bool epi_prefetch) {
   TORCH_CHECK(is_nhwc_dev(x, at::kBFloat16), "psd convn: x must be a channels_last bf16 device tensor");
   TORCH_CHECK(w2.is_cuda() && w2.dim() == 2 && w2.scalar_type() == at::kBFloat16 && w2.is_contiguous(),
               "psd convn: w2 must be a contiguous bf16 [Cout, R*S*C] device tensor");
@@ -287,6 +287,7 @@
     a.ares = opt_ptr<const uint16_t>(apply_res);
     a.amask = apply_mask->data_ptr<uint8_t>();
   }
+  a.epi_prefetch = epi_prefetch ? 1 : 0;
   set_geo(a, g, wbytes, Cout, K, no_store ? Cout : out.stride(0), variant);
   const hipError_t e = launch_convn(a, stream_of(x));
   if (e == hipErrorNotSupported) return 0;
@@ -365,7 +366,8 @@
                    int64_t pad, at::Tensor part, int64_t variant, int64_t mode, c10::optional<at::Tensor> bx,
                    const at::Tensor& bmean, c10::optional<at::Tensor> bss, c10::optional<at::Tensor> bdr,
                    c10::optional<at::Tensor> bmbits, c10::optional<at::Tensor> x2, c10::optional<at::Tensor> bias,
-                   c10::optional<at::Tensor> bxd, c10::optional<at::Tensor> bmean_d, c10::optional<at::Tensor> part_d) {
+                   c10::optional<at::Tensor> bxd, c10::optional<at::Tensor> bmean_d, c10::optional<at::Tensor> part_d,
+                   bool epi_prefetch) {
   TORCH_CHECK(is_nhwc_dev(dy, at::kBFloat16), "psd convn_bwd: dy must be a channels_last bf16 device tensor");
   TORCH_CHECK(w2.is_cuda() && w2.dim() == 2 && w2.scalar_type() == at::kBFloat16 && w2.is_contiguous(),
               "psd convn_bwd: w2 must be a contiguous bf16 [N, R*S*C] tensor");
@@ -426,6 +428,7 @@
   a.y = out.data_ptr();
   a.part = part.data_ptr<float>();
   set_geo(a, g, wbytes, N, K, N, variant);
+  a.epi_prefetch = epi_prefetch ? 1 : 0;
   a.bwd = (int)mode;
   a.bx = opt_ptr<const uint16_t>(bx);
   a.bmean = bmean.data_ptr<float>();
diff --git a/parameter_server_distributed_amd/csrc/kernels/convn.hip b/parameter_server_distributed_amd/csrc/kernels/convn.hip
--- a/parameter_server_distributed_amd/csrc/kernels/convn.hip
+++ b/parameter_server_distributed_amd/csrc/kernels/convn.hip
@@ -14,13 +14,13 @@
   return __builtin_bit_cast(bf16x8, *reinterpret_cast<const u32x4*>(lds + kmaj_off(row, ks * 4 + (lane >> 4))));
 }
 
-template <int DPSK, int A>
+template <int DPSK, int A, int OFF = 0>
 __device__ __forceinline__ void wait_ahead(int ahead) {
   if constexpr (A <= 0) {
-    wait_vm<0>();
+    wait_vm<OFF>();
   } else {
-    if (ahead >= A) wait_vm<A * DPSK>();
-    else wait_ahead<DPSK, A - 1>(ahead);
+    if (ahead >= A) wait_vm<A * DPSK + OFF>();
+    else wait_ahead<DPSK, A - 1, OFF>(ahead);
   }
 }
 
@@ -132,6 +132,7 @@
   int mm[4][PASSES];
   u32x4 exr[4][PASSES], rv4[4][PASSES], dv4[4][PASSES];
   uint32_t bt[4][PASSES];
+  uint8_t bt8[4][PASSES];
 };
 
 template <int WNT, int BWD, typename Pix>
@@ -184,18 +185,102 @@
     }
 }
 
-template <int BM, int BN, int WNT, bool STATS, int BWD, bool DEFER = false, bool PRE = false, typename Pix>
+struct EpiSrc {
+  rsrc_t bx, dr, mb, xd;
+};
+__device__ __forceinline__ EpiSrc epi_src(const ConvnArgs& a) {
+  const uint32_t mn2 = (uint32_t)a.M * (uint32_t)a.N * 2u;
+  EpiSrc s;
+  s.bx = make_rsrc(a.bx ? (const void*)a.bx : a.x, a.bx ? mn2 : 0u);
+  if (a.bwd == 8) {
+    s.dr = make_rsrc(a.ares ? (const void*)a.ares : a.x, a.ares ? mn2 : 0u);
+  } else {
+    s.dr = make_rsrc(a.bdr, a.bwd == 5 ? mn2 >> 2 : mn2);
+  }
+  s.mb = make_rsrc(a.bmbits ? (const void*)a.bmbits : a.x, a.bmbits ? mn2 >> 4 : 0u);
+  s.xd = make_rsrc(a.bxd ? (const void*)a.bxd : a.x, a.bxd ? mn2 : 0u);
+  return s;
+}
+
+template <int WNT>
+struct EpiK {
+  float bmu[8], bmd[8];
+  float sc[WNT / 16], sh[WNT / 16], bias[WNT / 16];
+};
+template <int WNT, int BWD>
+__device__ __forceinline__ void epi_consts(const ConvnArgs& a, int wc, int lane, int n0, EpiK<WNT>& k) {
+  constexpr int CPR = EpiOps<WNT>::CPR;
+  const int my_col = n0 + wc * WNT + (lane % CPR) * 8;
+  if constexpr (BWD == 3) load8_f32(a.bmean_d + my_col, k.bmd);
+  if constexpr (BWD >= 1 && BWD <= 5) load8_f32(a.bmean + my_col, k.bmu);
+#pragma unroll
+  for (int j = 0; j < WNT / 16; ++j) {
+    const int col = n0 + wc * WNT + j * 16 + (lane & 15);
+    k.bias[j] = a.bias ? a.bias[col] : 0.f;
+    if constexpr (BWD == 8) {
+      k.sc[j] = a.bss[col];
+      k.sh[j] = a.bss[a.N + col];
+    }
+  }
+}
+
+template <int WNT, int BWD, bool HASBX>
+struct EpiPf {
+  static constexpr int PER = BWD == 8 ? 1 : (HASBX ? 1 : 0) + 2 + (BWD == 3 ? 1 : 0);
+  static constexpr int LOADS = 4 * EpiOps<WNT>::PASSES * PER;
+};
+
+template <int WNT, int BWD, bool HASBX>
+__device__ __forceinline__ void epi_prefetch(const ConvnArgs& a, const EpiSrc& s, int i, int wr, int wc, int lane,
+                                             int m0, int mlim, int n0, EpiOps<WNT>& o) {
+  constexpr int CPR = EpiOps<WNT>::CPR, PASSES = EpiOps<WNT>::PASSES;
+  const int my_col = n0 + wc * WNT + (lane % CPR) * 8;
+#pragma unroll
+  for (int ps = 0; ps < PASSES; ++ps) {
+    const int rr = (ps * 64 + lane) / CPR;
+    const int row = m0 + wr * 64 + i * 16 + rr;
+    const bool ok = row < mlim;
+    o.mm[i][ps] = ok ? row : -1;
+    const uint32_t off = ok ? ((uint32_t)row * (uint32_t)a.N + (uint32_t)my_col) * 2u : kOOB;
+    if constexpr (BWD == 8) {
+      o.rv4[i][ps] = __builtin_amdgcn_raw_buffer_load_b128(s.dr, off, 0, 0);
+    } else {
+      if constexpr (HASBX) o.exr[i][ps] = __builtin_amdgcn_raw_buffer_load_b128(s.bx, off, 0, 0);
+      uint32_t roff = off;
+      if constexpr (BWD == 5) {
+        const int hw = a.Ho * a.Wo;
+        const int n = fdiv(row, hw, 1.f / (float)hw), rem = row - n * hw;
+        const int h = fdiv(rem, a.Wo, 1.f / (float)a.Wo), w = rem - h * a.Wo;
+        const uint32_t q = (uint32_t)((n * (a.Ho >> 1) + (h >> 1)) * (a.Wo >> 1) + (w >> 1));
+        roff = (ok && ((h | w) & 1) == 0) ? (q * (uint32_t)a.N + (uint32_t)my_col) * 2u : kOOB;
+      }
+      o.rv4[i][ps] = __builtin_amdgcn_raw_buffer_load_b128(s.dr, roff, 0, 0);
+      o.bt8[i][ps] = __builtin_amdgcn_raw_buffer_load_b8(s.mb, ok ? off >> 4 : kOOB, 0, 0);
+      if constexpr (BWD == 3) o.dv4[i][ps] = __builtin_amdgcn_raw_buffer_load_b128(s.xd, off, 0, 0);
+    }
+  }
+}
+
+struct NoNext {
+  __device__ __forceinline__ void operator()(int) const {}
+};
+
+template <int BM, int BN, int WNT, bool STATS, int BWD, bool DEFER = false, bool PRE = false, bool HASBX = true,
+          typename Pix, typename Nxt = NoNext>
 __device__ __forceinline__ void convn_epilogue(const ConvnArgs& a, f32x4 (&acc)[4][WNT / 16],
                                                const float (&kshift)[WNT / 16], int tm, int wr, int wc, int lane,
                                                uint8_t* stg, Pix pix, int n0, EpiSums<WNT / 16>& es,
-                                               const EpiOps<WNT>* pre = nullptr) {
+                                               const EpiOps<WNT>* pre = nullptr, const EpiK<WNT>* kc = nullptr,
+                                               Nxt next = Nxt{}) {
   constexpr int JN = WNT / 16;
   constexpr int WM = BM / 64;
   const int cl = lane & 15, rq = (lane >> 4) * 4;
   if (a.bias) {
 #pragma unroll
     for (int j = 0; j < JN; ++j) {
-      const float bv = a.bias[n0 + wc * WNT + j * 16 + cl];
+      float bv;
+      if constexpr (PRE) bv = kc->bias[j];
+      else bv = a.bias[n0 + wc * WNT + j * 16 + cl];
 #pragma unroll
       for (int i = 0; i < 4; ++i) acc[i][j] += f32x4{bv, bv, bv, bv};
     }
@@ -243,7 +328,12 @@
 #pragma unroll
     for (int j = 0; j < JN; ++j) {
       const int col = n0 + wc * WNT + j * 16 + cl;
-      const float sc = a.bss[col], sh = a.bss[a.N + col];
+      float sc, sh;
+      if constexpr (PRE) {
+        sc = kc->sc[j], sh = kc->sh[j];
+      } else {
+        sc = a.bss[col], sh = a.bss[a.N + col];
+      }
 #pragma unroll
       for (int i = 0; i < 4; ++i)
 #pragma unroll
@@ -258,8 +348,16 @@
   const int my_c16 = lane % CPR;
   const int my_col = n0 + wc * WNT + my_c16 * 8;
   float bmu[8], bsc[8], bsh[8], bmd[8];
-  if constexpr (BWD == 3) load8_f32(a.bmean_d + my_col, bmd);
-  if constexpr (BRED) load8_f32(a.bmean + my_col, bmu);
+  if constexpr (PRE) {
+#pragma unroll
+    for (int e = 0; e < 8; ++e) {
+      if constexpr (BRED) bmu[e] = kc->bmu[e];
+      if constexpr (BWD == 3) bmd[e] = kc->bmd[e];
+    }
+  } else {
+    if constexpr (BWD == 3) load8_f32(a.bmean_d + my_col, bmd);
+    if constexpr (BRED) load8_f32(a.bmean + my_col, bmu);
+  }
   if constexpr (BWD == 1) {
     load8_f32(a.bss + my_col, bsc);
     load8_f32(a.bss + a.N + my_col, bsh);
@@ -313,11 +411,18 @@
         if constexpr (BRED) {
           float d[8], xv[8];
           load8_bf16(reinterpret_cast<const uint16_t*>(&v), d);
-          load8_bf16(reinterpret_cast<const uint16_t*>(&exr[i][ps]), xv);
+          if constexpr (HASBX) {
+            load8_bf16(reinterpret_cast<const uint16_t*>(&exr[i][ps]), xv);
+          } else {
+#pragma unroll
+            for (int e = 0; e < 8; ++e) xv[e] = 0.f;
+          }
           if constexpr (BWD >= 2) {
             float rv[8];
             load8_bf16(reinterpret_cast<const uint16_t*>(&rv4[i][ps]), rv);
-            const uint32_t bits = bt[i][ps];
+            uint32_t bits;
+            if constexpr (PRE) bits = ops.bt8[i][ps];
+            else bits = bt[i][ps];
 #pragma unroll
             for (int e = 0; e < 8; ++e) d[e] = ((bits >> e) & 1u) ? d[e] + rv[e] : 0.f;
           } else {
@@ -345,6 +450,7 @@
         *reinterpret_cast<u32x4*>(y + go) = v;
       }
     }
+    if constexpr (PRE) next(i);
   }
   if constexpr (!DEFER) convn_flush<WNT, STATS, BWD>(a, es, (int64_t)tm * WM + wr, wc, lane, n0);
 }
@@ -487,7 +593,7 @@
 }
 
 
-template <int BN, int WNT, int NSLOT, bool STATS, int BWD>
+template <int BN, int WNT, int NSLOT, bool STATS, int BWD, bool PF = false, bool HASBX = true>
 __global__ __launch_bounds__(512) void convp_kernel(ConvnArgs a, int tiles_m) {
   constexpr int BM = 128;
   using G = Geo<BM, BN, WNT, NSLOT>;
@@ -523,13 +629,14 @@
     const bool second = k0 >= a.K1;
     const int c0 = second ? k0 - a.K1 : k0;
     const int lc = second ? a.logC2 : a.logC;
+    const bool live = !PF || T < total;
 #pragma unroll
     for (int i = 0; i < G::APW; ++i) {
       const int piece = i * G::NW + wid;
       const int row = piece * 8 + (lane >> 3);
       const int kc = (lane & 7) ^ ((row >> 1) & 7);
       const int m = m0 + row;
-      const uint32_t off = m < a.M ? ((((uint32_t)m) << lc) + (uint32_t)(c0 + kc * 8)) * 2u : kOOB;
+      const uint32_t off = (live && m < a.M) ? ((((uint32_t)m) << lc) + (uint32_t)(c0 + kc * 8)) * 2u : kOOB;
       __builtin_amdgcn_raw_ptr_buffer_load_lds(second ? x2r : xr,
                                                (__attribute__((address_space(3))) void*)(slot + piece * 1024), 16, off,
                                                0, 0, 0);
@@ -539,7 +646,7 @@
       const int piece = i * G::NW + wid;
       const int row = piece * 8 + (lane >> 3);
       const int kc = (lane & 7) ^ ((row >> 1) & 7);
-      const uint32_t off = ((uint32_t)(n0 + row) * (uint32_t)a.K + (uint32_t)(k0 + kc * 8)) * 2u;
+      const uint32_t off = live ? ((uint32_t)(n0 + row) * (uint32_t)a.K + (uint32_t)(k0 + kc * 8)) * 2u : kOOB;
       __builtin_amdgcn_raw_ptr_buffer_load_lds(
           wrs, (__attribute__((address_space(3))) void*)(slot + (SLOTB - BN * 128) + piece * 1024), 16, off, 0, 0, 0);
     }
@@ -553,12 +660,34 @@
   es.zero();
   uint8_t* stg = smem + nslot * SLOTB + wid * G::STG;
   const int D = nslot - 1;
-  for (int p = 0; p < D && p < total; ++p) stage(p);
+  constexpr int PFL = EpiPf<WNT, BWD, HASBX>::LOADS;
+  static_assert(!PF || G::DPS * (NSLOT - 2) + PFL < 64, "vmcnt is 6 bits");
+  EpiOps<WNT> ops;
+  EpiK<WNT> kc;
+  EpiSrc src;
+  int pf_at = -1;
+  if constexpr (PF) {
+    src = epi_src(a);
+    epi_consts<WNT, BWD>(a, wc, lane, n0, kc);
+    for (int p = 0; p < D; ++p) stage(p);
+    __builtin_amdgcn_sched_barrier(0);
+#pragma unroll
+    for (int i = 0; i < 4; ++i)
+      epi_prefetch<WNT, BWD, HASBX>(a, src, i, wr, wc, lane, t_begin * BM, total > 0 ? a.M : 0, n0, ops);
+    __builtin_amdgcn_sched_barrier(0);
+  } else {
+    for (int p = 0; p < D && p < total; ++p) stage(p);
+  }
   for (int T = 0; T < total; ++T) {
-    wait_ahead<G::DPS, NSLOT - 2>(min(total - 1 - T, D - 1));
+    if constexpr (PF) {
+      if (T - pf_at <= D) wait_ahead<G::DPS, NSLOT - 2, PFL>(D - 1);
+      else wait_ahead<G::DPS, NSLOT - 2>(D - 1);
+    } else {
+      wait_ahead<G::DPS, NSLOT - 2>(min(total - 1 - T, D - 1));
+    }
     __builtin_amdgcn_s_barrier();
     __builtin_amdgcn_sched_barrier(0);
-    if (T + D < total) stage(T + D);
+    if (PF || T + D < total) stage(T + D);
     const uint8_t* As = smem + (T % nslot) * SLOTB;
     const uint8_t* Bs = As + (SLOTB - BN * 128);
     bf16x8 af[2][4], bf[2][G::JN];
@@ -581,7 +710,18 @@
       const int tile = t_begin + T / nt;
       const int m0 = tile * BM;
       auto pix = [&](int p) -> int { return m0 + p < a.M ? m0 + p : -1; };
-      convn_epilogue<BM, BN, WNT, STATS, BWD, true>(a, acc, kshift, tile, wr, wc, lane, stg, pix, n0, es);
+      if constexpr (PF) {
+        const int nlim = tile + 1 < t_end ? a.M : 0;
+        auto next = [&](int i) {
+          epi_prefetch<WNT, BWD, HASBX>(a, src, i, wr, wc, lane, m0 + BM, nlim, n0, ops);
+        };
+        convn_epilogue<BM, BN, WNT, STATS, BWD, true, true, HASBX>(a, acc, kshift, tile, wr, wc, lane, stg, pix, n0,
+                                                                   es, &ops, &kc, next);
+        pf_at = T;
+        __builtin_amdgcn_sched_barrier(0);
+      } else {
+        convn_epilogue<BM, BN, WNT, STATS, BWD, true>(a, acc, kshift, tile, wr, wc, lane, stg, pix, n0, es);
+      }
 #pragma unroll
       for (int i = 0; i < 4; ++i)
 #pragma unroll
@@ -592,7 +732,7 @@
 }
 
 constexpr int kPrMaxSlots = 6;
-template <int BN, int WNT, bool STATS, int BWD>
+template <int BN, int WNT, bool STATS, int BWD, bool PF = false, bool HASBX = true>
 __global__ __launch_bounds__(512) void convpr_kernel(ConvnArgs a, int tiles_m) {
   constexpr int BM = 128;
   using G = Geo<BM, BN, WNT, 3>;
@@ -640,13 +780,14 @@
     const bool second = k0 >= a.K1;
     const int c0 = second ? k0 - a.K1 : k0;
     const int lc = second ? a.logC2 : a.logC;
+    const bool live = !PF || T < total;
 #pragma unroll
     for (int i = 0; i < G::APW; ++i) {
       const int piece = i * G::NW + wid;
       const int row = piece * 8 + (lane >> 3);
       const int kc = (lane & 7) ^ ((row >> 1) & 7);
       const int m = m0 + row;
-      const uint32_t off = m < a.M ? ((((uint32_t)m) << lc) + (uint32_t)(c0 + kc * 8)) * 2u : kOOB;
+      const uint32_t off = (live && m < a.M) ? ((((uint32_t)m) << lc) + (uint32_t)(c0 + kc * 8)) * 2u : kOOB;
       __builtin_amdgcn_raw_ptr_buffer_load_lds(second ? x2r : xr,
                                                (__attribute__((address_space(3))) void*)(slot + piece * 1024), 16, off,
                                                0, 0, 0);
@@ -660,12 +801,34 @@
   EpiSums<G::JN> es;
   es.zero();
   const int D = nslot - 1;
-  for (int p = 0; p < D && p < total; ++p) stage(p);
+  constexpr int PFL = EpiPf<WNT, BWD, HASBX>::LOADS;
+  static_assert(!PF || G::APW * (kPrMaxSlots - 2) + PFL < 64, "vmcnt is 6 bits");
+  EpiOps<WNT> ops;
+  EpiK<WNT> kc;
+  EpiSrc src;
+  int pf_at = -1;
+  if constexpr (PF) {
+    src = epi_src(a);
+    epi_consts<WNT, BWD>(a, wc, lane, n0, kc);
+    for (int p = 0; p < D; ++p) stage(p);
+    __builtin_amdgcn_sched_barrier(0);
+#pragma unroll
+    for (int i = 0; i < 4; ++i)
+      epi_prefetch<WNT, BWD, HASBX>(a, src, i, wr, wc, lane, t_begin * BM, total > 0 ? a.M : 0, n0, ops);
+    __builtin_amdgcn_sched_barrier(0);
+  } else {
+    for (int p = 0; p < D && p < total; ++p) stage(p);
+  }
   for (int T = 0; T < total; ++T) {
-    wait_ahead<G::APW, kPrMaxSlots - 2>(min(total - 1 - T, D - 1));
+    if constexpr (PF) {
+      if (T - pf_at <= D) wait_ahead<G::APW, kPrMaxSlots - 2, PFL>(D - 1);
+      else wait_ahead<G::APW, kPrMaxSlots - 2>(D - 1);
+    } else {
+      wait_ahead<G::APW, kPrMaxSlots - 2>(min(total - 1 - T, D - 1));
+    }
     __builtin_amdgcn_s_barrier();
     __builtin_amdgcn_sched_barrier(0);
-    if (T + D < total) stage(T + D);
+    if (PF || T + D < total) stage(T + D);
     const uint8_t* As = ring + (T % nslot) * AB;
     const uint8_t* Bs = bres + (T % nt) * BN * 128;
     bf16x8 af[2][4], bf[2][G::JN];
@@ -688,7 +851,18 @@
       const int tile = t_begin + T / nt;
       const int m0 = tile * BM;
       auto pix = [&](int p) -> int { return m0 + p < a.M ? m0 + p : -1; };
-      convn_epilogue<BM, BN, WNT, STATS, BWD, true>(a, acc, kshift, tile, wr, wc, lane, stg, pix, n0, es);
+      if constexpr (PF) {
+        const int nlim = tile + 1 < t_end ? a.M : 0;
+        auto next = [&](int i) {
+          epi_prefetch<WNT, BWD, HASBX>(a, src, i, wr, wc, lane, m0 + BM, nlim, n0, ops);
+        };
+        convn_epilogue<BM, BN, WNT, STATS, BWD, true, true, HASBX>(a, acc, kshift, tile, wr, wc, lane, stg, pix, n0,
+                                                                   es, &ops, &kc, next);
+        pf_at = T;
+        __builtin_amdgcn_sched_barrier(0);
+      } else {
+        convn_epilogue<BM, BN, WNT, STATS, BWD, true>(a, acc, kshift, tile, wr, wc, lane, stg, pix, n0, es);
+      }
 #pragma unroll
       for (int i = 0; i < 4; ++i)
 #pragma unroll
@@ -864,7 +1038,13 @@
   return g < tiles_m ? g : tiles_m;
 }
 
-template <int BN, bool STATS, int BWD>
+template <int BN>
+static bool pf_ok(const ConvnArgs& a) {
+  return BN == 256 && a.epi_prefetch && (a.bwd == 2 || a.bwd == 5 || a.bwd == 8) && a.ldc == a.N &&
+         (int64_t)a.M * a.N * 2 <= 0xFFFFFF00ll && a.M < (1 << 24);
+}
+
+template <int BN, bool STATS, int BWD, bool PF = false, bool HASBX = true>
 static hipError_t convp_launch_t(const ConvnArgs& a0, hipStream_t st, int grid_mul = 1) {
   constexpr int WNT = P1Cfg<BN>::WNT;
   using G = Geo<128, BN, WNT, kP1Slots>;
@@ -872,7 +1052,7 @@
   static_assert(LDS <= 160 * 1024, "LDS");
   static bool attr = false;
   if (!attr) {
-    const hipError_t e = hipFuncSetAttribute((const void*)convp_kernel<BN, WNT, kP1Slots, STATS, BWD>,
+    const hipError_t e = hipFuncSetAttribute((const void*)convp_kernel<BN, WNT, kP1Slots, STATS, BWD, PF, HASBX>,
                                              hipFuncAttributeMaxDynamicSharedMemorySize, LDS);
     if (e != hipSuccess) return e;
     attr = true;
@@ -882,8 +1062,8 @@
   const int tiles_m = (a.M + 127) / 128, tiles_n = a.N / BN;
   int gx = convp_grid_x(tiles_m, tiles_n) * grid_mul;
   if (gx > tiles_m) gx = tiles_m;
-  hipLaunchKernelGGL((convp_kernel<BN, WNT, kP1Slots, STATS, BWD>), dim3(gx, tiles_n), dim3(G::NT), LDS, st, a,
-                     tiles_m);
+  hipLaunchKernelGGL((convp_kernel<BN, WNT, kP1Slots, STATS, BWD, PF, HASBX>), dim3(gx, tiles_n), dim3(G::NT), LDS, st,
+                     a, tiles_m);
   return hipGetLastError();
 }
 
@@ -896,13 +1076,13 @@
   return ns >= 3 ? ns : 0;
 }
 
-template <int BN, bool STATS, int BWD>
+template <int BN, bool STATS, int BWD, bool PF = false, bool HASBX = true>
 static hipError_t convpr_launch_t(const ConvnArgs& a0, int ns, hipStream_t st, int grid_mul = 1) {
   constexpr int WNT = P1Cfg<BN>::WNT;
   using G = Geo<128, BN, WNT, 3>;
   static bool attr = false;
   if (!attr) {
-    const hipError_t e = hipFuncSetAttribute((const void*)convpr_kernel<BN, WNT, STATS, BWD>,
+    const hipError_t e = hipFuncSetAttribute((const void*)convpr_kernel<BN, WNT, STATS, BWD, PF, HASBX>,
                                              hipFuncAttributeMaxDynamicSharedMemorySize, 160 * 1024);
     if (e != hipSuccess) return e;
     attr = true;
@@ -913,12 +1093,23 @@
   const int tiles_m = (a.M + 127) / 128, tiles_n = a.N / BN;
   int gx = convp_grid_x(tiles_m, tiles_n) * grid_mul;
   if (gx > tiles_m) gx = tiles_m;
-  hipLaunchKernelGGL((convpr_kernel<BN, WNT, STATS, BWD>), dim3(gx, tiles_n), dim3(G::NT), lds, st, a, tiles_m);
+  hipLaunchKernelGGL((convpr_kernel<BN, WNT, STATS, BWD, PF, HASBX>), dim3(gx, tiles_n), dim3(G::NT), lds, st, a,
+                     tiles_m);
   return hipGetLastError();
 }
 
 template <int BN>
 static hipError_t convpr_launch_s(const ConvnArgs& a, int ns, hipStream_t st, int gm = 1) {
+  if constexpr (BN == 256) {
+    if (pf_ok<BN>(a)) {
+      const bool hb = a.bx != nullptr;
+      if (a.bwd == 2) return hb ? convpr_launch_t<BN, false, 2, true, true>(a, ns, st, gm)
+                                : convpr_launch_t<BN, false, 2, true, false>(a, ns, st, gm);
+      if (a.bwd == 5) return hb ? convpr_launch_t<BN, false, 5, true, true>(a, ns, st, gm)
+                                : convpr_launch_t<BN, false, 5, true, false>(a, ns, st, gm);
+      if (a.bwd == 8) return convpr_launch_t<BN, false, 8, true, true>(a, ns, st, gm);
+    }
+  }
   if (a.bwd == 1) return convpr_launch_t<BN, false, 1>(a, ns, st, gm);
   if (a.bwd == 2) return convpr_launch_t<BN, false, 2>(a, ns, st, gm);
   if (a.bwd == 3) return convpr_launch_t<BN, false, 3>(a, ns, st, gm);
@@ -930,6 +1121,16 @@
 template <int BN>
 static hipError_t convp_launch_s(const ConvnArgs& a, hipStream_t st, int gm = 1) {
   if (const int ns = pr_slots<BN>(a.K)) return convpr_launch_s<BN>(a, ns, st, gm);
+  if constexpr (BN == 256) {
+    if (pf_ok<BN>(a)) {
+      const bool hb = a.bx != nullptr;
+      if (a.bwd == 2) return hb ? convp_launch_t<BN, false, 2, true, true>(a, st, gm)
+                                : convp_launch_t<BN, false, 2, true, false>(a, st, gm);
+      if (a.bwd == 5) return hb ? convp_launch_t<BN, false, 5, true, true>(a, st, gm)
+                                : convp_launch_t<BN, false, 5, true, false>(a, st, gm);
+      if (a.bwd == 8) return convp_launch_t<BN, false, 8, true, true>(a, st, gm);
+    }
+  }
   if (a.bwd == 1) return convp_launch_t<BN, false, 1>(a, st, gm);
   if (a.bwd == 2) return convp_launch_t<BN, false, 2>(a, st, gm);
   if (a.bwd == 3) return convp_launch_t<BN, false, 3>(a, st, gm);
diff --git a/parameter_server_distributed_amd/csrc/kernels/launchers_convn.h b/parameter_server_distributed_amd/csrc/kernels/launchers_convn.h
--- a/parameter_server_distributed_amd/csrc/kernels/launchers_convn.h
+++ b/parameter_server_distributed_amd/csrc/kernels/launchers_convn.h
@@ -33,6 +33,7 @@
   const uint16_t* ares;
   uint8_t* amask;
   int ophase;
+  int epi_prefetch;
 };
 
 int convn_tile_n(int N);
diff --git a/parameter_server_distributed_amd/csrc/ops.h b/parameter_server_distributed_amd/csrc/ops.h
--- a/parameter_server_distributed_amd/csrc/ops.h
+++ b/parameter_server_distributed_amd/csrc/ops.h
@@ -108,7 +108,7 @@
                int64_t pad, c10::optional<at::Tensor> part, c10::optional<at::Tensor> shift, int64_t variant,
                c10::optional<at::Tensor> x2, c10::optional<at::Tensor> bias, bool no_store,
                c10::optional<at::Tensor> apply_ss, c10::optional<at::Tensor> apply_res,
-               c10::optional<at::Tensor> apply_mask);
+               c10::optional<at::Tensor> apply_mask, bool epi_prefetch);
 int64_t convn_stats_rows_(int64_t M);
 int64_t convn_dgrad_s2_(const at::Tensor& dy, const std::vector<at::Tensor>& wph, at::Tensor out, int64_t variant,
                         c10::optional<at::Tensor> part, c10::optional<at::Tensor> bx, c10::optional<at::Tensor> bmean,
@@ -119,7 +119,7 @@
                    const at::Tensor& bmean, c10::optional<at::Tensor> bss, c10::optional<at::Tensor> bdr,
                    c10::optional<at::Tensor> bmbits, c10::optional<at::Tensor> x2,
                    c10::optional<at::Tensor> bias, c10::optional<at::Tensor> bxd, c10::optional<at::Tensor> bmean_d,
-                   c10::optional<at::Tensor> part_d);
+                   c10::optional<at::Tensor> part_d, bool epi_prefetch);
 std::vector<at::Tensor> bn_bwd_pre(const at::Tensor& g, const at::Tensor& x, c10::optional<at::Tensor> gamma,
                                    const at::Tensor& save_mean, const at::Tensor& save_invstd, const at::Tensor& part,
                                    int64_t rows, c10::optional<at::Tensor> dgamma_out,
diff --git a/parameter_server_distributed_amd/ops/conv.py b/parameter_server_distributed_amd/ops/conv.py
--- a/parameter_server_distributed_amd/ops/conv.py
+++ b/parameter_server_distributed_amd/ops/conv.py
@@ -229,7 +229,8 @@
     part_d = torch.empty_like(part) if fu["mode"] == 3 else None
     rows = _native().convn_bwd_(dy, w2, out, k, k, 1, pad, part, v, fu["mode"], fu["bx"], fu["mean"],
                                 bss=fu.get("ss"), bdr=_dr_arg(fu.get("dr")), bmbits=fu.get("mbits"), x2=x2,
-                                bias=bias, bxd=fu.get("bxd"), bmean_d=fu.get("mean_d"), part_d=part_d)
+                                bias=bias, bxd=fu.get("bxd"), bmean_d=fu.get("mean_d"), part_d=part_d,
+                                epi_prefetch=_feat("convp_epi_prefetch"))
     if rows == 0:
         raise RuntimeError(declined)
     g = _from_2d(out, n, h, w)
diff --git a/parameter_server_distributed_amd/ops/tail.py b/parameter_server_distributed_amd/ops/tail.py
--- a/parameter_server_distributed_amd/ops/tail.py
+++ b/parameter_server_distributed_amd/ops/tail.py
@@ -56,7 +56,8 @@
             res, ss = scratch
             out = torch.empty(M, cout, device=dev, dtype=torch.bfloat16)
             mb = torch.empty(M * cout // 8, device=dev, dtype=torch.uint8)
-            if C.convn_(a2, w2, out, 1, 1, 1, 0, variant=v, apply_ss=ss, apply_res=res, apply_mask=mb) == 0:
+            if C.convn_(a2, w2, out, 1, 1, 1, 0, variant=v, apply_ss=ss, apply_res=res, apply_mask=mb,
+                        epi_prefetch=_feat("convp_epi_prefetch")) == 0:
                 raise _at.Declined("convn apply pass")
             return out
         return fn
@@ -123,7 +124,8 @@
                                          bn_momentum(bn), bn.eps, bn.num_batches_tracked)
         out = torch.empty(M, cout, device=a2.device, dtype=torch.bfloat16)
         mbits = torch.empty(M * cout // 8, device=a2.device, dtype=torch.uint8)
-        if C.convn_(a2, w2, out, 1, 1, 1, 0, variant=v, apply_ss=ss, apply_res=idt, apply_mask=mbits) == 0:
+        if C.convn_(a2, w2, out, 1, 1, 1, 0, variant=v, apply_ss=ss, apply_res=idt, apply_mask=mbits,
+                    epi_prefetch=_feat("convp_epi_prefetch")) == 0:
             raise RuntimeError("psd tail: convn declined the apply pass")
         y = _from_2d(out, n, h, w)
         bn._psd_fwd = BnFwd(y, None, mean, ss, mbits)
@@ -279,14 +281,16 @@
             def fn():
                 o = torch.empty(M, cout, device=a2.device, dtype=torch.bfloat16)
                 mb = torch.empty(M * cout // 8, device=a2.device, dtype=torch.uint8)
-                if C.convn_(a2, wcat, o, 1, 1, 1, 0, variant=v, x2=xin, apply_ss=ssc, apply_mask=mb) == 0:
+                if C.convn_(a2, wcat, o, 1, 1, 1, 0, variant=v, x2=xin, apply_ss=ssc, apply_mask=mb,
+                            epi_prefetch=_feat("convp_epi_prefetch")) == 0:
                     raise _at.Declined("convn dual apply pass")
                 return o
             return fn
 
         cands = {f"psdn{v}": make(v) for v in _dual_variants(cout, w)}
         v = int(_at.choose(("tail", "dual_apply", M, c3, cd, cout), cands, next(iter(cands)))[4:])
-        if C.convn_(a2, wcat, out, 1, 1, 1, 0, variant=v, x2=xin, apply_ss=ssc, apply_mask=mbits) == 0:
+        if C.convn_(a2, wcat, out, 1, 1, 1, 0, variant=v, x2=xin, apply_ss=ssc, apply_mask=mbits,
+                    epi_prefetch=_feat("convp_epi_prefetch")) == 0:
             raise RuntimeError("psd dual tail: convn declined the apply pass")
         y = _from_2d(out, n, h, w)
         bn3._psd_fwd = BnFwd(y, None, mean3, None, mbits)
diff --git a/parameter_server_distributed_amd/utils/config.py b/parameter_server_distributed_amd/utils/config.py
--- a/parameter_server_distributed_amd/utils/config.py
+++ b/parameter_server_distributed_amd/utils/config.py
@@ -45,6 +45,10 @@
     "convn_persist": (True, "persistent layer-1 3x3 kernel (convh)"),
     "convn_p1": (True, "persistent 1x1 kernels (convp / convpr)"),
     "convn_p2": (True, "the persistent 1x1 kernel at two workgroups per CU (two-slot ring) as a candidate"),
+    "convp_epi_prefetch": (True, "persistent 1x1 kernels, 256-wide tiles, epilogue modes 2 / 5 / 8: the epilogue "
+                                 "operands (dr / residual, mask bytes, BN input) loaded one tile ahead; off: loaded "
+                                 "at the top of each tile's epilogue (same results bit for bit, "
+                                 "profiles/convp_epi_prefetch.md)"),
     "convn_bwd": (True, "producing BN's backward reduction in the bwd-data epilogue (modes 1/2)"),
     "convn_bwd3": (True, "the dual-BN tail's reduction in the bwd-data epilogue (mode 3)"),
     "convn_bwd5": (True, "stride-2 downsample gradient added on the quarter grid (mode 5)"),
```

Measured after the change: 16790 (median of 6 runs). +2.7%, better.
